# genetronhealth/uvc

Measured on AMD Instinct MI355X. Metric: pileup positions scored/sec at 300x depth, higher is better.
Workload: dtype int32

## Files before the change

### uvc_amd/csrc/uvc_device.h

```cpp
#ifndef UVC_DEVICE_H
#define UVC_DEVICE_H

#include <hip/hip_runtime.h>
#include <stddef.h>
#include <stdint.h>
#include "uvcgpu.h"
#include "uvc_rules.h"
#include "uvc_planes.h"

#define SQR_QUAL_DIV 32
#define MAX_INSERT_SIZE 2000
#define MAX_STR_N_BASES 100
#define UVC_MAXEV 8
#define UVC_DIGEST_MAX_VOTES (1 << 22)

enum { C_MATCH = 0, C_INS = 1, C_DEL = 2, C_REF_SKIP = 3, C_SOFT_CLIP = 4, C_HARD_CLIP = 5, C_PAD = 6, C_EQUAL = 7, C_DIFF = 8 };

struct AlnRec {
    int32_t pos, rend, mpos, isize;
    int32_t flag, mapq, dflag, l_qseq;
    int64_t seq_off;
    int64_t qbase;
    int64_t cigar_off;
    int64_t table_off;
// ... 50 lines not shown
static_assert(sizeof(Item) == 16, "Item");

struct MisItem { int32_t rank, epos, symval; };

struct FragUnit { int32_t beg, end, fi, flags, pos0, rend0, pos1, rend1, qb0, qb1, nogap0, nogap1; };
enum { UVC_FSUM_LCNT = 0 , UVC_FSUM_LTA = 5, UVC_FSUM_LTB, UVC_FSUM_LSING, UVC_FSUM_LMQ, UVC_FSUM_BDP, UVC_FSUM_BTA, UVC_FSUM_BTB, UVC_FSUM_BMQ, UVC_FSUM_N };
struct FragFast {
    int32_t beg, end, fi, flags;
    int32_t pos0, rend0, pos1, rend1;
    int32_t qb0, qb1, nogap0, nogap1;
    int32_t sq, n_cov, n_near, pad_;
    int32_t bpos0, brend0, bqb0, sp0;
    int32_t bpos1, brend1, bqb1, sp1;
};
enum { FF_GENERIC = 1,
       FF_STRAND = 2, FF_SINGLETON = 4, FF_NALN_SHIFT = 3, FF_NALN_MASK = 0xF,
       FF_RUNS_B = 0x100,
       FF_LINK_PER_POS = 0x200,
       FF_NOT_REGISTER = FF_GENERIC | FF_RUNS_B,
       FF_FULL = FF_RUNS_B | FF_LINK_PER_POS,
       FF_NOT_IN_SUMS = FF_GENERIC | FF_FULL };
#define FF_W(field) ((int)(offsetof(FragFast, field) / 4))
static_assert(sizeof(FragFast) == 96, "k_frag fetches a fragment record as six 16-byte words per lane");
static_assert(sizeof(FragUnit) == 48 && offsetof(FragFast, sq) == sizeof(FragUnit), "FragUnit is the first 12 words of FragFast");
static_assert(FF_W(flags) == 3 && offsetof(FragUnit, flags) == offsetof(FragFast, flags) && offsetof(FragUnit, nogap1) == offsetof(FragFast, nogap1), "k_frag_sums reads flags as .w of a record's first int4");

struct AlnGap {
    int32_t epos, sym;
    int32_t len, qpos;
    int32_t weight, aln;
    int32_t mark, pad_;
};
struct GapRow { int32_t x, sym, len, ev; int64_t seq_off; int32_t cnt[8]; };
struct GapWork {
    AlnGap *ev; int32_t n_ev;
    unsigned long long *ckey, *ckey_s, *cval, *cval_s;
    unsigned long long *ikey, *ikey_s, *ival, *ival_s;
    int32_t inc_cap; int32_t *n_inc;
    GapRow *rows; int32_t *n_rows; uint8_t *seq; unsigned long long *seq_len; int64_t seq_cap;
    int32_t *maj;
    void *sort_tmp; size_t sort_tmp_bytes;
};

struct Contrib { uint8_t bsym_p1 , lmask ; uint16_t bval; uint16_t lval[8]; uint16_t pad_[2]; };
static_assert(sizeof(Contrib) == 24, "Contrib rows are zero-filled as bytes and indexed as 24-byte records");

struct HapWork { int32_t *cand, *cand_off, *cand_cap; int32_t *n_cand; unsigned long long *total; int32_t *events; };

struct DevParams { UvcParams P; };

struct RegionDev {
    int32_t beg, end; int64_t npos;
    const uint8_t *refsym;
    int32_t *rtr;
    const int64_t *baq;
    int32_t *prep32; int64_t *prep64; int32_t *thres;
    int32_t *seg32; int64_t *seg64; int32_t *vq; int32_t *bqsum;
    int32_t *frag; int32_t *fam; int32_t *faminfo32; int64_t *faminfo64; int32_t *duplex;
    int32_t *bucket;
    const uint8_t *bases; const uint8_t *quals; const uint32_t *cigars;
    const uint16_t *bq; uint32_t bq_bytes;
    AlnRec *alns; int32_t n_alns;
    int32_t n_fast;
    int32_t p2_off[5];
    FastRec *frec2; int32_t n_fast2; int32_t max_p2_span;
    const int32_t *complex_ids; int32_t n_complex;
    FragRec *frags; int32_t n_frags;
    int32_t *frag_nmut; int32_t *frag_mut;
    const int32_t *sweep_frags; int32_t n_sweep;
    int32_t *overflow_frags; int32_t *n_overflow;
    const int32_t *frag_sorted;
    const int32_t *frag_rank;
    int32_t frag_off[3];
    FragFast *ffast;
    FragUnit *ffast_u;
    int32_t *win; int32_t nwin;
    int32_t *fsum;
    FsRec *fss; int32_t n_fs;
    const int32_t *generic_fs; int32_t n_generic_fs; int64_t n_generic_work;
    const int32_t *generic_sorted; int32_t max_unit_span;
    uint8_t *p5flag;
    uint8_t *dirty; int32_t ndblk;
    uint32_t *occ;
    uint32_t *fam_digest;
    Contrib *table;
    int32_t *ir_list;
    Item *items; int32_t *item_cnt;
    MisItem *mis; int32_t *mis_cnt; int32_t mis_cap;
    unsigned long long *mis_total;
    int32_t max_frag_span;
    int32_t any_amplicon;
    int32_t frag32;
    int32_t max_frag_depth;
    int32_t *err;
    GapWork gap;
};

#define DEV __device__ __forceinline__

DEV int ff_naln(int flags) { return (flags >> FF_NALN_SHIFT) & FF_NALN_MASK; }
template <int WORDS>
DEV void load_words(const void *rec, bool valid, int (&c)[WORDS]) {
    static_assert(WORDS % 4 == 0, "whole 16-byte words");
    if (valid) {
        const int4 *q4 = (const int4 *)rec;
#pragma unroll
        for (int i = 0; i < WORDS / 4; i++) { const int4 t = q4[i]; c[4 * i] = t.x; c[4 * i + 1] = t.y; c[4 * i + 2] = t.z; c[4 * i + 3] = t.w; }
    } else {
#pragma unroll
        for (int i = 0; i < WORDS; i++) c[i] = 0;
    }
}
DEV int64_t lmin(int64_t a, int64_t b) { return a < b ? a : b; }
DEV int64_t lmax(int64_t a, int64_t b) { return a > b ? a : b; }
DEV int64_t nnminus(int64_t a, int64_t b) { return a > b ? a - b : 0; }
DEV int ibetween(int v, int a, int b) { return imin(imax(a, v), b); }
DEV bool is_ins(int s) { return s == UVC_LINK_I3P || s == UVC_LINK_I2 || s == UVC_LINK_I1; }
DEV bool is_del(int s) { return s == UVC_LINK_D3P || s == UVC_LINK_D2 || s == UVC_LINK_D1; }
DEV bool is_subst(int s) { return s <= UVC_BASE_NN; }
DEV bool symbols_mutated(int ref, int alt) {
    if (alt <= UVC_BASE_NN) return ref != alt && ref < UVC_BASE_N && alt < UVC_BASE_N;
    return alt != UVC_LINK_M && alt != UVC_LINK_NN;
}
DEV int cig_op(uint32_t c) { return (int)(c & 0xF); }
DEV int cig_len(uint32_t c) { return (int)(c >> 4); }
DEV bool cig_aligned(int op) { return op == C_MATCH || op == C_EQUAL || op == C_DIFF; }
DEV bool cig_query(int op) { return op == C_MATCH || op == C_EQUAL || op == C_DIFF || op == C_INS || op == C_SOFT_CLIP; }
DEV bool cig_ref(int op) { return op == C_MATCH || op == C_EQUAL || op == C_DIFF || op == C_DEL || op == C_REF_SKIP; }

#define P32(R, f, x) ((R).prep32[(size_t)(f) * (R).npos + (x)])
#define P64(R, f, x) ((R).prep64[(size_t)(f) * (R).npos + (x)])
#define TH(R, f, x) ((R).thres[(size_t)(f) * (R).npos + (x)])
#define S32(R, f, s, x) ((R).seg32[((size_t)(f) * NSYM + (s)) * (R).npos + (x)])
#define S64(R, f, s, x) ((R).seg64[((size_t)(f) * NSYM + (s)) * (R).npos + (x)])
#define VQP(R, f, s, x) ((R).vq[((size_t)(f) * NSYM + (s)) * (R).npos + (x)])
#define BQS(R, s, x) ((R).bqsum[(size_t)(s) * (R).npos + (x)])
#define FRP(R, st, f, s, x) ((R).frag[(((size_t)(st) * UVC_NFRAG + (f)) * NSYM + (s)) * (R).npos + (x)])
#define FAP(R, st, f, s, x) ((R).fam[(((size_t)(st) * UVC_NFAM + (f)) * NSYM + (s)) * (R).npos + (x)])
#define FIP(R, f, s, x) ((R).faminfo32[((size_t)(f) * NSYM + (s)) * (R).npos + (x)])
#define FI64P(R, f, s, x) ((R).faminfo64[((size_t)(f) * NSYM + (s)) * (R).npos + (x)])
#define DUP(R, f, s, x) ((R).duplex[((size_t)(f) * NSYM + (s)) * (R).npos + (x)])
#define BKP(R, st, s, b, x) ((R).bucket[((((size_t)(st) * NSYM + (s)) * NBUCKETS) + (b)) * (R).npos + (x)])
#define RTRP(R, f, x) ((R).rtr[(size_t)(f) * (R).npos + (x)])
#define BAQ1(R, p) ((R).baq[(p) - (R).beg])
#define BAQ2(R, p) ((R).baq[(R).npos + (p) - (R).beg])

DEV int cov_PREP32(const RegionDev &R, int plane, int64_t x) { return P32(R, plane, x); }
DEV int cov_FRAG(const RegionDev &R, int plane, int64_t x) {
    int v = 0;
#pragma unroll
    for (int sd = 0; sd < 2; sd++)
#pragma unroll
        for (int s = UVC_BASE_A; s <= UVC_BASE_NN; s++) v += FRP(R, sd, plane, s, x);
    return v;
}
DEV int cov_FAM(const RegionDev &R, int plane, int64_t x) {
    int v = 0;
#pragma unroll
    for (int sd = 0; sd < 2; sd++)
#pragma unroll
        for (int s = UVC_BASE_A; s <= UVC_BASE_NN; s++) v += FAP(R, sd, plane, s, x);
    return v;
}
DEV int cov_DUPLEX(const RegionDev &R, int plane, int64_t x) {
    int v = 0;
#pragma unroll
// ... 86 lines not shown
```

### uvc_amd/csrc/uvc_host.cpp

```cpp
#include "uvc_launch.h"
#include "uvc_host.h"
#include "uvc_alloc.h"
#include "uvc_prep.h"
#include "uvc_rtr.h"
#include "uvc_hap.h"
#include "uvc_cpus.h"

#include <algorithm>
#include <array>
#include <chrono>
#include <cmath>
#include <cstring>
#include <memory>
#include <numeric>
#include <string>
#include <thread>
#include <vector>

static thread_local std::string g_err;
static int fail(int code, const std::string &msg) { g_err = msg; return code; }
template <class F> static int guarded(const char *what, F &&f) {
    try {
        const int rc = f();
        const hipError_t stale = hipGetLastError();
        if (stale != hipSuccess && getenv("UVCGPU_DEBUG")) fprintf(stderr, "[uvcgpu] %s (rc %d) left HIP error: %s\n", what, rc, hipGetErrorString(stale));
        return rc;
    }
    catch (const std::bad_alloc &) { return fail(UVCGPU_ENOMEM, std::string(what) + ": out of host memory"); }
    catch (const std::exception &e) { return fail(UVCGPU_EDEVICE, std::string(what) + ": " + e.what()); }
}
extern "C" int uvcgpu_set_error(int code, const char *msg) { return fail(code, msg ? msg : ""); }
#define HIP_OK(call) do { hipError_t e_ = (call); if (e_ != hipSuccess) return fail(UVCGPU_EDEVICE, std::string(#call) + ": " + hipGetErrorString(e_)); } while (0)

struct uvcgpu_score_stream;
struct uvcgpu_region;
static void quiesce(const uvcgpu_region *r);
template <class T, bool HOST = false> struct Buf {
    const uvcgpu_region *r; T *p = nullptr; size_t cap = 0;
    explicit Buf(const uvcgpu_region *r_) : r(r_) {}
    Buf(const Buf &) = delete; Buf &operator=(const Buf &) = delete;
    ~Buf() { release(); }
    operator T *() const { return p; }
    static hipError_t raw_alloc(void **q, size_t bytes) { return HOST ? hipHostMalloc(q, bytes, hipHostMallocDefault) : uvc_dev_malloc(q, bytes); }
    static hipError_t raw_free(void *q) { return HOST ? hipHostFree(q) : uvc_dev_free(q); }
    void release() { if (p) { quiesce(r); (void)raw_free(p); } p = nullptr; cap = 0; }
    hipError_t fit(size_t need, size_t slack = 0, size_t keep_max = 0, size_t unit = sizeof(T), size_t *bytes = nullptr) {
        if (cap >= need && !(keep_max && cap > keep_max)) return hipSuccess;
        release();
        const size_t want = (need + slack) * unit;
        if (bytes) *bytes = want;
        const hipError_t e = raw_alloc((void **)&p, want);
        if (e != hipSuccess) { (void)hipGetLastError(); p = nullptr; return e; }
        cap = need + slack;
        return hipSuccess;
    }
};
struct Pool {
    const uvcgpu_region *r; std::vector<void *> blocks; hipError_t last = hipSuccess;
    explicit Pool(const uvcgpu_region *r_) : r(r_) {}
    Pool(const Pool &) = delete; Pool &operator=(const Pool &) = delete;
    ~Pool() { clear(); }
    void *get(size_t bytes) { void *q = nullptr; last = uvc_dev_malloc(&q, bytes); if (last != hipSuccess) return nullptr; blocks.push_back(q); return q; }
    template <class T> bool get(T **out, size_t count) { *out = (T *)get(count * sizeof(T)); return *out != nullptr; }
    void clear() { if (!blocks.empty()) quiesce(r); for (void *q : blocks) (void)uvc_dev_free(q); blocks.clear(); }
};

struct uvcgpu_region {
    UvcParams P;
    int32_t tid, beg, end;
    int64_t npos;
    std::string refstring;
    std::vector<int32_t> h_rtr; bool h_rtr_valid = false;
    UvcRtrWork rw; Buf<char> d_rtrwork{this}; bool thr_ready = false;
    Buf<char, true> h_ref{this};
    hipStream_t stream = nullptr;
    std::array<hipStream_t *, 3> streams() { return { { &stream, &side, &side3 } }; }
    std::array<hipEvent_t *, 6> events() { return { { &e_fork, &e_join, &e_fork2, &e_join3, &e_stat, &e_alleles } }; }
    hipStream_t side = nullptr, side3 = nullptr; hipEvent_t e_fork = nullptr, e_join = nullptr, e_fork2 = nullptr, e_join3 = nullptr, e_stat = nullptr, e_alleles = nullptr;
    Buf<uint8_t> d_refsym{this}; Buf<int32_t> d_rtr{this}, d_rtr0{this}, d_fsum{this}, d_win{this}; Buf<int64_t> d_baq{this};
    Buf<char> d_state{this}; SlabLayout L = {};
    Buf<int32_t> d_err{this};
    int64_t npos_cap = 0;
    bool buckets_clean = false;
    Pool owned{this};
    RegionDev R;
    int32_t *d_dup_units = nullptr; int64_t *d_dup_off = nullptr; int n_dup = 0; int64_t n_dup_work = 0;
    bool has_reads = false, accumulated = false;
    bool reads_given = false;
    Buf<uint8_t> d_dirty{this}; Buf<ZeroPlane> d_zero_planes{this}; int64_t zero_planes_npos = 0;
    int64_t dirty_npos = 0;
    bool state_released = false, state_zeroed = false;
    int64_t last_scored = 0, last_returned = 0;
    size_t zeroed_bytes = 0;
    RawReads W;
    int32_t *d_p2[4] = { nullptr, nullptr, nullptr, nullptr };
    int64_t n_bases = 0;
    UvcProf prof;
    Buf<char> d_score_scratch{this};
    Buf<int32_t> d_score_fields{this}; int64_t *d_score_count = nullptr;
    Buf<uint8_t, true> h_stage{this};
    Buf<int32_t> d_score_kept{this};
    Buf<char> d_report{this}; Buf<char, true> h_report{this};
    uvcgpu_score_stream *ss = nullptr;
    bool gap_ready = false;
    std::vector<UvcGapRow> gap_rows; std::vector<uint8_t> gap_seq;
    std::vector<UvcIndelAllele> gap_alleles; std::vector<int32_t> gap_allele_row;
    Buf<UvcIndelAllele> d_gap_alleles{this}; Buf<int32_t> d_gap_allele_row{this}; Buf<UvcGapRow> d_gap_rows{this}; Buf<uint8_t> d_gap_seq{this};
    bool hap_ready = false;
    std::vector<UvcHapLinkHost> hap[3];
};

static bool stream_is_open(const uvcgpu_region *r);
static void stream_destroy(uvcgpu_region *r);
static void quiesce(const uvcgpu_region *r) { for (hipStream_t s : { r->stream, r->side, r->side3 }) if (s) (void)hipStreamSynchronize(s); }
static int planes_guard(const uvcgpu_region *r, const char *call) {
    if (!r->accumulated) return fail(UVCGPU_ESTATE, std::string(call) + " before accumulate");
    if (r->state_released) return fail(UVCGPU_ESTATE, "the planes were released by the last score (UvcScoreRequest::release_state)");
    return 0;
}

namespace {
template <class T> int dev_alloc(uvcgpu_region *r, size_t count, T **out, bool zero = false) {
    const size_t n = std::max<size_t>(count, 1);
    if (!r->owned.get(out, n)) return fail(UVCGPU_ENOMEM, std::string("hipMalloc: ") + hipGetErrorString(r->owned.last));
    if (zero && hipMemsetAsync(*out, 0, n * sizeof(T), r->stream) != hipSuccess) return fail(UVCGPU_EDEVICE, "hipMemsetAsync");
    return 0;
}
void free_reads(uvcgpu_region *r) { r->owned.clear(); r->has_reads = false; r->reads_given = false; r->accumulated = false; }
}

extern "C" {

const char *uvcgpu_last_error(void) { return g_err.c_str(); }
const char *uvcgpu_version(void) { return "uvcgpu 0.1 (gfx950)"; }

int uvcgpu_init(int device_id) {
    int n = 0;
    if (hipGetDeviceCount(&n) != hipSuccess || n <= 0) return fail(UVCGPU_EDEVICE, "no HIP device: libuvcgpu has no CPU fallback");
    HIP_OK(hipSetDevice(device_id));
    hipDeviceProp_t prop;
    HIP_OK(hipGetDeviceProperties(&prop, device_id));
    if (std::string(prop.gcnArchName).find("gfx950") == std::string::npos) return fail(UVCGPU_EDEVICE, std::string("device is ") + prop.gcnArchName + ", this library is built for gfx950 only");
    return 0;
}

int uvcgpu_device_memory(int64_t *free_bytes, int64_t *total_bytes) {
    size_t fr = 0, tot = 0;
    HIP_OK(hipMemGetInfo(&fr, &tot));
    if (free_bytes) *free_bytes = (int64_t)fr;
    if (total_bytes) *total_bytes = (int64_t)tot;
    return 0;
}

int uvcgpu_device_count(void) { int n = 0; if (hipGetDeviceCount(&n) != hipSuccess) { (void)hipGetLastError(); return 0; } return n; }

void uvcgpu_params_default(UvcParams *p) {
    memset(p, 0, sizeof(*p));
    p->struct_size = (int32_t)sizeof(UvcParams);
#define UVC_PI(name, dflt) p->name = (int32_t)(dflt);
#define UVC_PD(name, dflt) p->name = (double)(dflt);
#include "uvc_params.def"
#undef UVC_PI
#undef UVC_PD
}

static void platform_deltas(UvcParams *p, int32_t platform) {
    auto dec = [](int32_t &a, int32_t b) { a = a - std::min(a, b); };
    if (platform == UVC_PLATFORM_IONTORRENT) {
        p->bq_phred_added_misma += 8;
        dec(p->fam_thres_highBQ_snv, 30); dec(p->fam_thres_highBQ_indel, 30); dec(p->bias_thres_PFBQ1, 30); dec(p->bias_thres_PFBQ2, 30); dec(p->bias_thres_highBQ, 13);
    } else if (platform == UVC_PLATFORM_ILLUMINA) {
        p->syserr_minABQ_pcr_snv += 200; p->syserr_minABQ_pcr_indel += 100; p->syserr_minABQ_cap_snv += 200; p->syserr_minABQ_cap_indel += 100;
    }
}

void uvcgpu_params_apply_platform(UvcParams *p, int32_t platform, int32_t central_readlen, int32_t max_mapq) {
    p->inferred_sequencing_platform = platform;
    if (0 == p->central_readlen) p->central_readlen = central_readlen;
    p->inferred_maxMQ = std::max(p->inferred_maxMQ, max_mapq);
    platform_deltas(p, platform);
}

int uvcgpu_params_apply_platform_ex(UvcParams *p, int32_t sequencing_platform, int32_t inferred, int32_t central_readlen, int32_t max_mapq) {
    if (!p || sequencing_platform < UVC_PLATFORM_AUTO || sequencing_platform > UVC_PLATFORM_OTHER) return fail(UVCGPU_EINVAL, "sequencing platform outside 0..3");
    if (sequencing_platform == UVC_PLATFORM_ILLUMINA || sequencing_platform == UVC_PLATFORM_IONTORRENT) {
        p->inferred_sequencing_platform = sequencing_platform;
        platform_deltas(p, sequencing_platform);
    } else if (sequencing_platform == UVC_PLATFORM_AUTO) {
        uvcgpu_params_apply_platform(p, inferred, central_readlen, max_mapq);
    } else {
        p->inferred_sequencing_platform = inferred;
        if (0 == p->central_readlen) p->central_readlen = central_readlen;
        p->inferred_maxMQ = std::max(p->inferred_maxMQ, max_mapq);
    }
    return 0;
}

static int configure_region(uvcgpu_region *r, int32_t tid, int32_t beg, int32_t end, const char *refseq) {
    r->tid = tid; r->beg = beg; r->end = end + 1; r->npos = (int64_t)end - beg + 1;
    r->refstring.assign(refseq, (size_t)(end - beg));
    r->accumulated = false; r->gap_ready = false; r->hap_ready = false; r->state_released = false;
    r->h_rtr_valid = false;
    r->L = slab_layout(r->npos);
    r->state_zeroed = r->state_zeroed && r->npos <= r->npos_cap && r->L.total <= r->zeroed_bytes;
    r->buckets_clean = r->state_zeroed;
    const int vmax = r->P.indel_vntr_repeatsize_max, smax = r->P.indel_str_repeatsize_max, bqm = r->P.indel_BQ_max;
    const size_t n_rtr = (size_t)UVC_NRTR * r->npos, n = (size_t)r->npos;
    if (r->npos > r->npos_cap) {
        r->npos_cap = 0; r->dirty_npos = 0; r->thr_ready = false;
        size_t scan_tmp = 0;
        const size_t work_bytes = uvc_rtr_work_bytes(r->npos, vmax, smax, bqm, &scan_tmp);
        if (r->d_refsym.fit(n + 1) != hipSuccess || r->d_rtr.fit(n_rtr) != hipSuccess || r->d_rtr0.fit(n_rtr) != hipSuccess || r->d_fsum.fit(2 * UVC_FSUM_N * n) != hipSuccess
            || r->d_win.fit(16 * (size_t)((r->npos + 63) / 64)) != hipSuccess || r->d_baq.fit(2 * n) != hipSuccess || r->d_state.fit(r->L.total) != hipSuccess || r->d_rtrwork.fit(work_bytes) != hipSuccess
            || r->d_dirty.fit((size_t)3 * NSYM * (size_t)((r->npos >> UVC_DIRTY_SHIFT) + 2)) != hipSuccess) return fail(UVCGPU_ENOMEM, "hipMalloc(region planes) failed");
        uvc_rtr_bind(&r->rw, r->d_rtrwork, r->npos, vmax, smax, bqm, scan_tmp);
        r->npos_cap = r->npos;
    }
    if (!r->thr_ready) {
        std::vector<int32_t> thr((size_t)smax * bqm);
        uvc_rtr_thresholds(&r->P, thr.data());
        HIP_OK(hipMemcpy(r->rw.thr, thr.data(), sizeof(int32_t) * thr.size(), hipMemcpyHostToDevice));
        r->thr_ready = true;
    }
    const size_t n_ref = (size_t)(end - beg);
    if (r->h_ref.fit(n_ref) != hipSuccess) return fail(UVCGPU_ENOMEM, "hipHostMalloc(reference staging) failed");
    memcpy(r->h_ref, refseq, n_ref);
    HIP_OK(hipMemcpyAsync(r->rw.refchar, r->h_ref, n_ref, hipMemcpyHostToDevice, r->stream));
    {
        const int e = uvc_launch_region_tracks(&r->rw, &r->P, r->npos, r->d_refsym, r->d_rtr0, r->d_baq, r->stream);
        if (e) return fail(UVCGPU_EDEVICE, std::string("side-array kernels: ") + hipGetErrorString((hipError_t)e));
    }
    RegionDev &R = r->R;
    memset(&R, 0, sizeof(R));
    R.beg = r->beg; R.end = r->end; R.npos = r->npos; R.refsym = r->d_refsym; R.rtr = r->d_rtr; R.baq = r->d_baq; R.fsum = r->d_fsum; R.win = r->d_win; R.nwin = (int32_t)((r->npos + 63) / 64);
    char *b = r->d_state;
#define X(g, m) R.m = (decltype(R.m))(b + r->L.off[UVC_F_##g]);
    UVC_SLAB_MEMBERS(X)
#undef X
    R.bucket = (int32_t *)(b + r->L.bucket_off); R.p5flag = (uint8_t *)(b + r->L.p5flag_off); R.occ = (uint32_t *)(b + r->L.occ_off);
    R.dirty = r->d_dirty; R.ndblk = (int32_t)((r->npos + ((int64_t)1 << UVC_DIRTY_SHIFT) - 1) >> UVC_DIRTY_SHIFT);
    R.err = r->d_err;
    HIP_OK(hipMemsetAsync(R.err, 0, 4, r->stream));
    return 0;
}

static int uvcgpu_region_create_impl(uvcgpu_region_t **out, const UvcParams *params, int32_t tid, int32_t beg, int32_t end, const char *refseq) {
    if (!out || !params || !refseq || end <= beg) return fail(UVCGPU_EINVAL, "bad argument");
    if (const int rc = uvcgpu_params_check(params)) return rc;
    uvcgpu_region *r = new uvcgpu_region();
    memset(&r->prof, 0, sizeof(r->prof));
    memset(&r->R, 0, sizeof(r->R));
    r->P = *params;
    const bool one_stream = (getenv("UVCGPU_ONE_STREAM") != nullptr);
    for (hipStream_t *s : r->streams()) {
        const bool main = (s == &r->stream);
        if (!main && one_stream) break;
        if (hipStreamCreateWithFlags(s, hipStreamNonBlocking) != hipSuccess) { uvcgpu_region_destroy(r); return fail(UVCGPU_EDEVICE, main ? "hipStreamCreate failed (no GPU?)" : "hipStreamCreate / hipEventCreate failed"); }
    }
    if (!one_stream) for (hipEvent_t *e : r->events()) if (hipEventCreateWithFlags(e, hipEventDisableTiming) != hipSuccess) { uvcgpu_region_destroy(r); return fail(UVCGPU_EDEVICE, "hipStreamCreate / hipEventCreate failed"); }
    if (r->d_err.fit(1) != hipSuccess) { uvcgpu_region_destroy(r); return fail(UVCGPU_ENOMEM, "hipMalloc failed"); }
    const int rc = configure_region(r, tid, beg, end, refseq);
    if (rc) { uvcgpu_region_destroy(r); return rc; }
    *out = r;
    return 0;
}

static int uvcgpu_region_reset_impl(uvcgpu_region_t *r, int32_t tid, int32_t beg, int32_t end, const char *refseq) {
    if (!r || !refseq || end <= beg) return fail(UVCGPU_EINVAL, "bad argument");
    if (stream_is_open(r)) return fail(UVCGPU_ESTATE, "reset while a score stream is open");
    HIP_OK(hipStreamSynchronize(r->stream));
    if (r->side) HIP_OK(hipStreamSynchronize(r->side));
    if (r->side3) HIP_OK(hipStreamSynchronize(r->side3));
    free_reads(r);
    return configure_region(r, tid, beg, end, refseq);
}

static void *prep_alloc(void *ctx, size_t bytes, int zero) {
    uvcgpu_region *r = (uvcgpu_region *)ctx;
    char *p = nullptr;
    if (dev_alloc(r, bytes, &p, zero != 0)) return nullptr;
    return p;
}
static int set_reads_on_device(uvcgpu_region_t *r, const UvcReadSoA *d, bool timing, std::chrono::steady_clock::time_point t_prev) {
    auto lap = [&](const char *what) { if (!timing) return; hipStreamSynchronize(r->stream); const auto t = std::chrono::steady_clock::now();
                                       fprintf(stderr, "[uvcgpu set_reads] %-28s %8.2f ms\n", what, std::chrono::duration<double, std::milli>(t - t_prev).count()); t_prev = t; };
    const int64_t n = d->n_reads;
    if (r->npos >= ((int64_t)1 << 29)) return fail(UVCGPU_EUNSUPPORTED, "region longer than 2^29");
    if (d->n_bases >= ((int64_t)1 << 31)) return fail(UVCGPU_EUNSUPPORTED, "more than 2^31 read bases in one region: split the region");
    if (!d->bases && !d->bases4 && d->n_bases > 0) return fail(UVCGPU_EINVAL, "neither bases nor bases4");
    UvcReadSoA dd = *d;
    int32_t *d_bad = nullptr; uint16_t *bq_done = nullptr;
    if (!d->seq_off || !d->cigar_off || !d->bases) {
        int rc0;
        int64_t *so = nullptr, *co = nullptr, *b4o = nullptr; uint8_t *ub = nullptr; char *tmp = nullptr;
        const size_t tb = uvc_prep_compact_tmp_bytes(n);
        if ((rc0 = dev_alloc(r, tb, &tmp)) || (rc0 = dev_alloc(r, 2, &d_bad, true))) return rc0;
        if (!d->seq_off && (rc0 = dev_alloc(r, (size_t)n, &so))) return rc0;
        if (!d->cigar_off && (rc0 = dev_alloc(r, (size_t)n, &co))) return rc0;
        if (!d->bases && ((rc0 = dev_alloc(r, (size_t)n, &b4o)) || (rc0 = dev_alloc(r, (size_t)std::max<int64_t>(d->n_bases, 1), &ub)) || (rc0 = dev_alloc(r, (size_t)std::max<int64_t>(d->n_bases, 1), &bq_done)))) return rc0;
        const int e = uvc_prep_compact(d->l_qseq, d->n_cigar, n, d->n_bases, d->bases ? nullptr : d->bases4, d->n_bases4_bytes, d->quals, so, d->seq_off, co, b4o, ub, bq_done, d_bad, tmp, tb, r->stream);
        if (e) return fail(UVCGPU_EDEVICE, std::string("offset scans: ") + hipGetErrorString((hipError_t)e));
        if (so) dd.seq_off = so;
        if (co) dd.cigar_off = co;
        if (ub) dd.bases = ub;
        d = &dd;
    }
    UvcPrepIn in; memset(&in, 0, sizeof(in));
    in.n_reads = n; in.n_bases = d->n_bases; in.n_cigar_ops = d->n_cigar_ops; in.n_fams = d->n_fams;
    in.pos = d->pos; in.mpos = d->mpos; in.isize = d->isize; in.nm = d->nm; in.l_qseq = d->l_qseq; in.n_cigar = d->n_cigar; in.frag_id = d->frag_id; in.fam_id = d->fam_id;
    in.flag = d->flag; in.mapq = d->mapq; in.fam_strand = d->fam_strand; in.fam_dflag = d->fam_dflag; in.seq_off = d->seq_off; in.cigar_off = d->cigar_off; in.cigars = d->cigars;
    uint16_t *bq_packed = bq_done;
    if (!bq_packed) {
        int rc1;
        if ((rc1 = dev_alloc(r, (size_t)std::max<int64_t>(d->n_bases, 1), &bq_packed))) return rc1;
        if (!d_bad && (rc1 = dev_alloc(r, 2, &d_bad, true))) return rc1;
        uvc_launch_pack_bq(d->bases, d->quals, bq_packed, d->n_bases, d_bad, r->stream);
    }
    in.quals = d->quals; in.zero_qual = d_bad + 1;
    UvcPrepOut o; char msg[256];
    int rc = uvc_prep_reads(&in, &r->P, r->beg, r->end, r->npos, prep_alloc, r, r->stream, &o, msg, (int)sizeof(msg));
    if (rc) return fail(rc, msg);
    lap("nesting + CIGAR facts (device)");
    RegionDev &R = r->R;
// ... 107 lines not shown
    const int64_t n = in->n_reads;
    if (n == 0) { r->reads_given = true; return 0; }
    if (n > INT32_MAX / 2) return fail(UVCGPU_EUNSUPPORTED, "more than 2^30 reads in one region");
    if (in->n_bases < 0 || in->n_cigar_ops < 0) return fail(UVCGPU_EINVAL, "bad reads");
    UvcReadSoA d = *in;
    int rc;
    hipStream_t small_stream = (r->side ? r->side : r->stream);
    auto up_on = [&](hipStream_t st, const void *src, size_t bytes, void **out) -> int {
        char *q = nullptr;
        int rc2 = dev_alloc(r, bytes, &q);
        if (rc2) return rc2;
        if (bytes && hipMemcpyAsync(q, src, bytes, hipMemcpyHostToDevice, st) != hipSuccess) return fail(UVCGPU_EDEVICE, "hipMemcpyAsync(H2D)");
        *out = q;
        return 0;
    };
#define UP(field, T, count) { void *q; if ((rc = up_on(small_stream, in->field, sizeof(T) * (size_t)(count), &q))) return rc; d.field = (const T *)q; }
#define UPBIG(field, T, count) { void *q; if ((rc = up_on(r->stream, in->field, sizeof(T) * (size_t)(count), &q))) return rc; d.field = (const T *)q; }
    if (in->bases) UPBIG(bases, uint8_t, in->n_bases)
    else if (in->bases4) { if (in->n_bases4_bytes < 0) return fail(UVCGPU_EINVAL, "bad reads"); UPBIG(bases4, uint8_t, in->n_bases4_bytes) }
    UPBIG(quals, uint8_t, in->n_bases)
    UP(pos, int32_t, n) UP(mpos, int32_t, n) UP(isize, int32_t, n) UP(flag, uint16_t, n) UP(mapq, uint8_t, n) UP(nm, int32_t, n) UP(l_qseq, int32_t, n)
    UP(n_cigar, int32_t, n) UP(frag_id, int32_t, n) UP(fam_id, int32_t, n) UP(fam_strand, uint8_t, n)
    if (in->seq_off) UP(seq_off, int64_t, n)
    if (in->cigar_off) UP(cigar_off, int64_t, n)
    UP(cigars, uint32_t, in->n_cigar_ops) UP(fam_dflag, uint8_t, in->n_fams)
    if (small_stream != r->stream) {
        if (hipEventRecord(r->e_fork2, small_stream) != hipSuccess || hipStreamWaitEvent(r->stream, r->e_fork2, 0) != hipSuccess) return fail(UVCGPU_EDEVICE, "hipEventRecord / hipStreamWaitEvent");
    }
#undef UPBIG
#undef UP
    if (timing) { hipStreamSynchronize(r->stream); const auto t = std::chrono::steady_clock::now(); fprintf(stderr, "[uvcgpu set_reads] %-28s %8.2f ms\n", "H2D of the columns", std::chrono::duration<double, std::milli>(t - t_prev).count()); t_prev = t; }
    return set_reads_on_device(r, &d, timing, t_prev);
}

static int uvcgpu_region_set_reads_device_impl(uvcgpu_region_t *r, const UvcReadSoA *in) {
    if (!r || !in) return fail(UVCGPU_EINVAL, "bad reads");
    if (stream_is_open(r)) return fail(UVCGPU_ESTATE, "set_reads while a score stream is open");
    if (in->struct_size != (int32_t)sizeof(UvcReadSoA)) return fail(UVCGPU_EINVAL, "UvcReadSoA::struct_size mismatch (set it to sizeof(UvcReadSoA))");
    if (in->n_reads < 0 || in->n_fams < 0 || in->n_bases < 0 || in->n_cigar_ops < 0) return fail(UVCGPU_EINVAL, "bad reads");
    const bool timing = (getenv("UVCGPU_TIMING") != nullptr);
    free_reads(r);
    if (in->n_reads == 0) { r->reads_given = true; return 0; }
    if (in->n_reads > INT32_MAX / 2) return fail(UVCGPU_EUNSUPPORTED, "more than 2^30 reads in one region");
    return set_reads_on_device(r, in, timing, std::chrono::steady_clock::now());
}

static int uvcgpu_region_correct_bq_impl(uvcgpu_region_t *r) {
    if (!r) return fail(UVCGPU_EINVAL, "null region");
    if (!r->has_reads) return fail(UVCGPU_ENOREADS, "no reads");
    uvc_launch_correct_bq(&r->R, r->P.assay_sequencing_BQ_max, r->P.assay_sequencing_BQ_inc, r->stream);
    uvc_launch_pack_bq(r->R.bases, r->R.quals, (uint16_t *)r->R.bq, r->n_bases, nullptr, r->stream);
    const int zthr = uvc_prep_zero_value_qual(&r->P);
    int32_t *d_n_joined = nullptr;
    if (zthr > 0 || (zthr == 0 && (r->P.assay_sequencing_BQ_inc < 0 || r->P.assay_sequencing_BQ_max <= 0))) {
        int rc = dev_alloc(r, 1, &d_n_joined, true);
        if (rc) return rc;
        uvc_prep_requalify(r->R.quals, r->W.seq_off, r->W.l_qseq, &r->P, r->R.n_frags, (FragRec *)r->R.frags, (int32_t *)r->R.sweep_frags, r->R.n_sweep, d_n_joined, r->stream);
    }
    HIP_OK(hipMemsetAsync(r->R.mis_total, 0, sizeof(unsigned long long), r->stream));
    uvc_launch_prelude(&r->R, &r->W, &r->P, r->stream);
    uvc_launch_build_p2list(&r->R, r->W.fast_rank, r->d_p2[0], r->d_p2[1], r->d_p2[2], r->d_p2[3], r->stream);
    HIP_OK(hipGetLastError());
    if (d_n_joined) {
        HIP_OK(hipStreamSynchronize(r->stream));
        int32_t n_joined = 0;
        HIP_OK(hipMemcpy(&n_joined, d_n_joined, sizeof(n_joined), hipMemcpyDeviceToHost));
        if (getenv("UVCGPU_TIMING")) fprintf(stderr, "[uvcgpu correct_bq] fragments looked at again: %d joined the sweep list (%d)\n", n_joined, r->R.n_sweep + n_joined);
        r->R.n_sweep += n_joined;
    } else HIP_OK(hipStreamSynchronize(r->stream));
    r->accumulated = false;
    return 0;
}

int uvcgpu_region_read_quals(uvcgpu_region_t *r, uint8_t *dst, int64_t n) {
    if (!r || !dst) return fail(UVCGPU_EINVAL, "null argument");
    if (!r->has_reads) return fail(UVCGPU_ENOREADS, "no reads");
    if (n != r->n_bases) return fail(UVCGPU_EINVAL, "n must equal UvcReadSoA::n_bases");
    HIP_OK(hipStreamSynchronize(r->stream));
    if (n > 0) HIP_OK(hipMemcpy(dst, r->R.quals, (size_t)n, hipMemcpyDeviceToHost));
    return 0;
}

static int zero_state(uvcgpu_region *r, hipStream_t s) {
    const size_t n_dirty = (size_t)3 * NSYM * (size_t)r->R.ndblk;
    const bool selective = (r->dirty_npos == r->npos && !getenv("UVCGPU_FILL_ALL"));
    r->dirty_npos = 0;
    if (selective) {
        if (r->zero_planes_npos != r->npos) {
            ZeroPlane v[UVC_N_ZERO_PLANES];
            zero_plane_rows(r->L, r->npos, v);
            r->zero_planes_npos = 0;
            const hipError_t e = r->d_zero_planes.fit(UVC_N_ZERO_PLANES);
            if (e != hipSuccess) return fail(UVCGPU_EDEVICE, std::string("hipMalloc(zero-fill table): ") + hipGetErrorString(e));
            HIP_OK(hipMemcpy(r->d_zero_planes, v, sizeof(v), hipMemcpyHostToDevice));
            r->zero_planes_npos = r->npos;
        }
        uvc_launch_zero_state(r->d_state, r->d_zero_planes, UVC_N_ZERO_PLANES, r->d_dirty, r->R.ndblk, r->npos, s);
        if (hipGetLastError() != hipSuccess) return fail(UVCGPU_EDEVICE, "zero fill of the planes failed");
        if (!r->buckets_clean) HIP_OK(hipMemsetAsync(r->d_state + r->L.bucket_off, 0, r->L.total - r->L.bucket_off, s));
    } else {
        HIP_OK(hipMemsetAsync(r->d_state, 0, r->buckets_clean ? r->L.bucket_off : r->L.total, s));
    }
    HIP_OK(hipMemsetAsync(r->d_dirty, 0, n_dirty, s));
    return 0;
}

static int uvcgpu_region_accumulate_impl(uvcgpu_region_t *r) {
    if (!r) return fail(UVCGPU_EINVAL, "null region");
    if (stream_is_open(r)) return fail(UVCGPU_ESTATE, "accumulate while a score stream is open");
    if (!r->has_reads) return fail(UVCGPU_ENOREADS, "no reads");
    if (r->state_zeroed) { r->dirty_npos = 0; HIP_OK(hipStreamWaitEvent(r->stream, r->e_join, 0)); }
    else { const int rcz = zero_state(r, r->stream); if (rcz) return rcz; }
    r->state_zeroed = false; r->state_released = false;
    r->buckets_clean = false;
    HIP_OK(hipMemcpyAsync(r->d_rtr, r->d_rtr0, (size_t)4 * UVC_NRTR * r->npos, hipMemcpyDeviceToDevice, r->stream));
    HIP_OK(hipMemsetAsync(r->R.frag_nmut, 0, sizeof(int32_t) * (size_t)r->R.n_frags, r->stream));
    HIP_OK(hipMemsetAsync(r->R.n_overflow, 0, sizeof(int32_t), r->stream));
    HIP_OK(hipMemsetAsync(r->R.mis_cnt, 0, sizeof(int32_t), r->stream));
    if (r->R.n_complex) {
    }
    const int half = (int)std::round((10.0 / std::log(10.0)) * std::log(r->P.indel_del_to_ins_err_ratio)) / 2;
    const UvcAccStreams st = { r->stream, r->side, r->side3, r->e_fork, r->e_join, r->e_fork2, r->e_join3, r->e_stat, r->e_alleles };
    uvc_launch_accumulate(&r->R, &r->P, half, r->d_dup_units, r->n_dup, r->d_dup_off, r->n_dup_work, &st, &r->prof);
    HIP_OK(hipGetLastError());
    r->buckets_clean = (r->P.inferred_is_vcf_generated != 0);
    r->dirty_npos = r->npos;
    r->accumulated = true; r->gap_ready = false; r->hap_ready = false;
    return 0;
}

int uvcgpu_region_check_presence(uvcgpu_region_t *r, int64_t *n_violations) {
    if (!r || !n_violations) return fail(UVCGPU_EINVAL, "bad argument");
    if (planes_guard(r, "check_presence")) return fail(UVCGPU_ESTATE, "check_presence needs the planes of an accumulate");
    Pool tmp(r);
    unsigned long long *d = nullptr, h = 0;
    if (!tmp.get(&d, 1)) return fail(UVCGPU_EDEVICE, std::string("hipMalloc(violation count): ") + hipGetErrorString(tmp.last));
    int rc = 0;
    if (hipMemsetAsync(d, 0, 8, r->stream) != hipSuccess) rc = fail(UVCGPU_EDEVICE, "hipMemsetAsync");
    if (!rc) { uvc_launch_check_presence(&r->R, d, r->stream); uvc_launch_check_dirty(&r->R, d, r->stream); if (hipMemcpyAsync(&h, d, 8, hipMemcpyDeviceToHost, r->stream) != hipSuccess || hipStreamSynchronize(r->stream) != hipSuccess) rc = fail(UVCGPU_EDEVICE, "check_presence"); }
    *n_violations = (int64_t)h;
    return rc;
}

int uvcgpu_region_set_profiling(uvcgpu_region_t *r, int on) { if (!r) return fail(UVCGPU_EINVAL, "null region"); r->prof.on = on ? 1 : 0; return 0; }
int uvcgpu_region_kernel_times(uvcgpu_region_t *r, char *names, int names_bytes, float *ms, int capacity) {
    if (!r || !names || !ms) return fail(UVCGPU_EINVAL, "bad argument");
    HIP_OK(hipStreamSynchronize(r->stream));
    std::string all;
    int n = 0;
    for (int i = 0; i < r->prof.n && n < capacity; i++, n++) {
        float t = 0;
        HIP_OK(hipEventElapsedTime(&t, r->prof.ev[i][0], r->prof.ev[i][1]));
        ms[n] = t; all += r->prof.name[i]; all += ";";
    }
    if ((int)all.size() + 1 > names_bytes) return fail(UVCGPU_EINVAL, "names buffer too small");
    memcpy(names, all.c_str(), all.size() + 1);
    return n;
}

int uvcgpu_region_last_score_counts(const uvcgpu_region_t *r, int64_t *scored, int64_t *returned) {
    if (!r) return fail(UVCGPU_EINVAL, "null region");
    if (scored) *scored = r->last_scored;
    if (returned) *returned = r->last_returned;
    return 0;
}

int uvcgpu_region_sync(uvcgpu_region_t *r) {
    if (!r) return fail(UVCGPU_EINVAL, "null region");
    HIP_OK(hipStreamSynchronize(r->stream));
    int32_t e = 0;
    HIP_OK(hipMemcpy(&e, r->R.err, 4, hipMemcpyDeviceToHost));
    if (e) return fail(e, "a kernel flagged an unsupported read shape (a CIGAR op the reference itself throws on, process_cigar main_conversion.hpp:902-916)");
    return 0;
}

int64_t uvcgpu_region_field_bytes(const uvcgpu_region_t *r, int32_t g) {
    if (!r || g < 0 || g >= UVC_NUM_FIELD_GROUPS) return -1;
    if (uvc_group_in_slab(g) && !r->accumulated) return -1;
    return (int64_t)uvc_group_bytes(g, r->npos);
}

static int uvcgpu_region_fetch_impl(uvcgpu_region_t *r, int32_t g, void *dst, int64_t dst_bytes) {
    if (!r || !dst || g < 0 || g >= UVC_NUM_FIELD_GROUPS) return fail(UVCGPU_EINVAL, "bad argument");
    if (uvc_group_in_slab(g)) { const int rcg = planes_guard(r, "fetch"); if (rcg) return rcg; }
    if ((int64_t)uvc_group_bytes(g, r->npos) != dst_bytes) return fail(UVCGPU_EINVAL, "bad destination size");
    int rc = uvcgpu_region_sync(r);
    if (rc) return rc;
    const void *src = (g == UVC_F_RTR) ? (const void *)(r->accumulated ? r->d_rtr : r->d_rtr0)  : (g == UVC_F_BAQ) ? (const void *)r->d_baq : (const void *)(r->d_state + r->L.off[g]);
    HIP_OK(hipMemcpy(dst, src, (size_t)dst_bytes, hipMemcpyDeviceToHost));
    return 0;
}

int32_t uvcgpu_region_column_base(int32_t g) { return (g < 0 || g >= UVC_NUM_FIELD_GROUPS) ? -1 : uvc_group_first_column(g); }
int32_t uvcgpu_region_n_columns(void) { return UVC_N_COLUMNS; }
static int uvcgpu_region_fetch_columns_impl(uvcgpu_region_t *r, const int32_t *refpos, int64_t n, int64_t *dst) {
    if (!r || n < 0 || (n > 0 && (!refpos || !dst))) return fail(UVCGPU_EINVAL, "bad argument");
    { const int rcg = planes_guard(r, "fetch"); if (rcg) return rcg; }
    if (n == 0) return 0;
    int rc = uvcgpu_region_sync(r);
    if (rc) return rc;
    const int32_t ncol = UVC_N_COLUMNS;
    const char *base[UVC_NUM_FIELD_GROUPS]; int32_t first[UVC_NUM_FIELD_GROUPS + 1], elem[UVC_NUM_FIELD_GROUPS];
    for (int g = 0; g <= UVC_NUM_FIELD_GROUPS; g++) first[g] = uvc_columns_before(g);
    for (int g = 0; g < UVC_NUM_FIELD_GROUPS; g++) { elem[g] = uvc_group_elem(g); base[g] = r->d_state + r->L.off[g]; }
    std::vector<int32_t> xs((size_t)n);
    for (int64_t i = 0; i < n; i++) xs[(size_t)i] = refpos[i] - r->beg;
    Pool tmp(r);
    int32_t *d_xs = nullptr; long long *d_out = nullptr;
    if (!tmp.get(&d_xs, (size_t)n)) return fail(UVCGPU_ENOMEM, "hipMalloc(column positions) failed");
    if (!tmp.get(&d_out, (size_t)n * ncol)) return fail(UVCGPU_ENOMEM, "hipMalloc(columns) failed");
    hipError_t e = hipMemcpyAsync(d_xs, xs.data(), sizeof(int32_t) * (size_t)n, hipMemcpyHostToDevice, r->stream);
    if (e == hipSuccess) { uvc_launch_gather_columns(base, first, elem, r->npos, d_xs, n, d_out, r->stream); e = hipGetLastError(); }
    if (e == hipSuccess) e = hipMemcpyAsync(dst, d_out, sizeof(long long) * (size_t)n * ncol, hipMemcpyDeviceToHost, r->stream);
    if (e == hipSuccess) e = hipStreamSynchronize(r->stream);
    if (e != hipSuccess) return fail(UVCGPU_EDEVICE, hipGetErrorString(e));
    return 0;
}
int uvcgpu_region_block_stats_(uvcgpu_region_t *r, int32_t refpos_beg, int32_t refpos_end, int32_t *dst) {
    if (!r || !dst || refpos_end < refpos_beg) return fail(UVCGPU_EINVAL, "bad argument");
    { const int rcg = planes_guard(r, "fetch"); if (rcg) return rcg; }
    const int64_t n = (int64_t)refpos_end - refpos_beg;
    if (n == 0) return 0;
    int rc = uvcgpu_region_sync(r);
    if (rc) return rc;
    Pool tmp(r);
    int32_t *d = nullptr;
    if (!tmp.get(&d, 10 * (size_t)n)) return fail(UVCGPU_ENOMEM, "hipMalloc(block stats) failed");
    uvc_launch_block_stats(&r->R, &r->P, (int64_t)refpos_beg - r->beg, n, d, r->stream);
    hipError_t e = hipGetLastError();
    if (e == hipSuccess) e = hipMemcpyAsync(dst, d, sizeof(int32_t) * 10 * (size_t)n, hipMemcpyDeviceToHost, r->stream);
    if (e == hipSuccess) e = hipStreamSynchronize(r->stream);
    if (e != hipSuccess) return fail(UVCGPU_EDEVICE, hipGetErrorString(e));
    return 0;
}
int uvcgpu_region_block_stats_windows_(uvcgpu_region_t *r, const int32_t *win, int64_t n_win, int32_t *dst) {
    if (!r || !win || !dst || n_win < 0 || n_win > INT32_MAX) return fail(UVCGPU_EINVAL, "bad argument");
    { const int rcg = planes_guard(r, "fetch"); if (rcg) return rcg; }
    std::vector<long long> tab((size_t)(2 * n_win));
    int64_t n = 0;
    for (int64_t k = 0; k < n_win; k++) {
        if (win[2 * k + 1] <= win[2 * k]) return fail(UVCGPU_EINVAL, "block statistics: empty window");
        tab[(size_t)(2 * k)] = (long long)win[2 * k] - r->beg; tab[(size_t)(2 * k + 1)] = n; n += (int64_t)win[2 * k + 1] - win[2 * k];
    }
    if (n == 0) return 0;
    int rc = uvcgpu_region_sync(r);
    if (rc) return rc;
    Pool tmp(r);
    long long *d_tab = nullptr; int32_t *d = nullptr;
    if (!tmp.get(&d_tab, tab.size()) || !tmp.get(&d, 10 * (size_t)n)) return fail(UVCGPU_ENOMEM, "hipMalloc(block stats) failed");
    hipError_t e = hipMemcpyAsync(d_tab, tab.data(), sizeof(long long) * tab.size(), hipMemcpyHostToDevice, r->stream);
    if (e == hipSuccess) { uvc_launch_block_stats_windows(&r->R, &r->P, d_tab, (int)n_win, n, d, r->stream); e = hipGetLastError(); }
    if (e == hipSuccess) e = hipMemcpyAsync(dst, d, sizeof(int32_t) * 10 * (size_t)n, hipMemcpyDeviceToHost, r->stream);
    const hipError_t e2 = hipStreamSynchronize(r->stream);
    if (e != hipSuccess || e2 != hipSuccess) return fail(UVCGPU_EDEVICE, hipGetErrorString(e != hipSuccess ? e : e2));
    return 0;
}
int uvcgpu_pin_host_buffer(void *p, int64_t bytes) {
    if (!p || bytes <= 0) return fail(UVCGPU_EINVAL, "bad argument");
    hipError_t e = hipHostRegister(p, (size_t)bytes, hipHostRegisterDefault);
    if (e != hipSuccess) { (void)hipGetLastError(); return fail(UVCGPU_EDEVICE, std::string("hipHostRegister: ") + hipGetErrorString(e)); }
    return 0;
}
int uvcgpu_host_alloc(void **p, int64_t bytes) {
    if (!p || bytes <= 0) return fail(UVCGPU_EINVAL, "bad argument");
    *p = nullptr;
    hipError_t e = Buf<char, true>::raw_alloc(p, (size_t)bytes);
    if (e != hipSuccess) { (void)hipGetLastError(); *p = nullptr; return fail(UVCGPU_ENOMEM, std::string("hipHostMalloc: ") + hipGetErrorString(e)); }
    return 0;
}
int uvcgpu_host_free(void *p) {
    if (!p) return 0;
    hipError_t e = Buf<char, true>::raw_free(p);
    if (e != hipSuccess) { (void)hipGetLastError(); if (getenv("UVCGPU_DEBUG")) fprintf(stderr, "[uvcgpu] hipHostFree: %s\n", hipGetErrorString(e)); return fail(UVCGPU_EDEVICE, std::string("hipHostFree: ") + hipGetErrorString(e)); }
    return 0;
}
int uvcgpu_unpin_host_buffer(void *p) {
    if (!p) return 0;
    hipError_t e = hipHostUnregister(p);
    if (e != hipSuccess) { (void)hipGetLastError(); return fail(UVCGPU_EDEVICE, std::string("hipHostUnregister: ") + hipGetErrorString(e)); }
    return 0;
}

const char *uvcgpu_region_refseq(const uvcgpu_region_t *r, int32_t *beg, int32_t *end) { if (beg) *beg = r->beg; if (end) *end = r->end - 1; return r->refstring.c_str(); }
const int32_t *uvcgpu_region_repeat_tracks(const uvcgpu_region_t *cr, int64_t *npos) {
    uvcgpu_region_t *r = const_cast<uvcgpu_region_t *>(cr);
    if (npos) *npos = r->npos;
    if (!r->h_rtr_valid) {
        r->h_rtr.resize((size_t)3 * r->npos);
        if (hipMemcpyAsync(r->h_rtr.data(), r->d_rtr0, sizeof(int32_t) * r->h_rtr.size(), hipMemcpyDeviceToHost, r->stream) != hipSuccess || hipStreamSynchronize(r->stream) != hipSuccess) { (void)hipGetLastError(); return nullptr; }
        r->h_rtr_valid = true;
    }
    return r->h_rtr.data();
}
const UvcParams *uvcgpu_region_params(const uvcgpu_region_t *r) { return &r->P; }
// ... 138 lines not shown
        events.resize(at + (size_t)c.total);
        HIP_OK(hipMemcpyAsync(events.data() + at, H.events, 4 * (size_t)c.total, hipMemcpyDeviceToHost, r->stream));
        HIP_OK(hipStreamSynchronize(r->stream));
        lap(units ? "events of units + D2H" : "events of fragments + D2H", (long long)c.total);
    }
    { const int rc = uvcgpu_region_sync(r); if (rc) return rc; }
    uvc_hap_build(events.data(), (int64_t)events.size(), r->beg, r->npos, r->P.phasing_haplotype_max_count, r->P.phasing_haplotype_min_ad, r->P.phasing_haplotype_max_detail_cnt, r->hap);
    lap("maps + links (host)", (long long)(r->hap[0].size() + r->hap[1].size() + r->hap[2].size()));
    r->hap_ready = true;
    return 0;
}
const std::vector<UvcHapLinkHost> *uvcgpu_region_hap_(uvcgpu_region_t *r) { return hap_tables(r) ? nullptr : r->hap; }

static int uvcgpu_region_hap_links_impl(uvcgpu_region_t *r, UvcHapLink *links, int64_t link_capacity, int64_t *n_links, int32_t *muts, int64_t mut_capacity, int64_t *n_mut_ints) {
    if (!r) return fail(UVCGPU_EINVAL, "null region");
    int rc = hap_tables(r);
    if (rc) return rc;
    int64_t nl = 0, nm = 0;
    for (int w = 0; w < 3; w++) for (const UvcHapLinkHost &h : r->hap[w]) { nl++; nm += 2 * (int64_t)h.form.size(); }
    if (n_links) *n_links = nl;
    if (n_mut_ints) *n_mut_ints = nm;
    if (nl > link_capacity || nm > mut_capacity || (nl && !links) || (nm && !muts)) return fail(UVCGPU_ENOMEM, "haplotype link capacity too small");
    int64_t li = 0, mi = 0;
    for (int w = 0; w < 3; w++) for (const UvcHapLinkHost &h : r->hap[w]) {
        UvcHapLink &o = links[li++];
        o.which = w; o.n_muts = (int32_t)h.form.size(); o.mut_off = mi; o.fr_cnt[0] = h.fr[0]; o.fr_cnt[1] = h.fr[1]; o.other_cnt[0] = h.other[0]; o.other_cnt[1] = h.other[1];
        for (const auto &ps : h.form) { muts[mi++] = ps.first; muts[mi++] = ps.second; }
    }
    return 0;
}

int64_t uvcgpu_region_score_size(const uvcgpu_region_t *r, const UvcScoreRequest *req) {
    if (!r) return -1;
    const int64_t np = (req && req->pos_beg >= 0) ? (req->pos_end - req->pos_beg) : r->npos;
    return NSYM * (np + 1) + (req ? req->n_indel_alleles + req->n_tumor_keys + 16 * std::max<int64_t>(req->n_force_sites, 0) : 0) + (int64_t)r->gap_alleles.size();
}
int64_t uvcgpu_region_score_ranges_size(const uvcgpu_region_t *r, const UvcScoreRequest *req, const UvcScoreRange *ranges, int64_t n_ranges) {
    if (!r || !ranges || n_ranges < 0) return -1;
    int64_t np = 0;
    for (int64_t k = 0; k < n_ranges; k++) np += std::max<int64_t>((int64_t)ranges[k].pos_end - ranges[k].pos_beg, 0);
    return NSYM * (np + 1) + (req ? req->n_indel_alleles + req->n_tumor_keys + 16 * std::max<int64_t>(req->n_force_sites, 0) : 0) + (int64_t)r->gap_alleles.size();
}

static int stage_upload(uvcgpu_region_t *r, void *dst, const void *src, size_t bytes, size_t &at, size_t total) {
    if (r->h_stage.fit(total, total / 2 + 4096) != hipSuccess) return fail(UVCGPU_ENOMEM, "hipHostMalloc(staging)");
    memcpy(r->h_stage + at, src, bytes);
    if (hipMemcpyAsync(dst, r->h_stage + at, bytes, hipMemcpyHostToDevice, r->stream) != hipSuccess) return fail(UVCGPU_EDEVICE, "hipMemcpyAsync(staging)");
    at += (bytes + 63) & ~(size_t)63;
    return 0;
}

struct ScorePrep {
    UvcScoreRequest rq; std::vector<UvcScoreRangeDev> rtab; int64_t npos_scored = 0;
    std::unique_ptr<Pool> tmp;
    UvcScoreIn in = {};
};
static int score_prepare(uvcgpu_region_t *r, const UvcScoreRequest *req, const UvcScoreRange *ranges, int64_t n_ranges, ScorePrep &p) {
    { const int rcg = planes_guard(r, "score"); if (rcg) return rcg; }
    if (stream_is_open(r)) return fail(UVCGPU_ESTATE, "a score stream is open on this handle (uvcgpu_score_stream_end closes it)");
    p.tmp.reset(new Pool(r));
    UvcScoreRequest &rq = p.rq; memset(&rq, 0, sizeof(rq)); rq.pos_beg = -1;
    if (req) rq = *req;
    std::vector<UvcScoreRangeDev> &rtab = p.rtab;
    int64_t &npos_scored = p.npos_scored;
    if (ranges) {
        if (n_ranges < 1 || n_ranges > INT32_MAX) return fail(UVCGPU_EINVAL, "score_ranges: n_ranges must be at least 1");
        if (rq.pos_beg != -1 || rq.base_at_pos_beg != 0 || rq.region_beg != 0) return fail(UVCGPU_EINVAL, "score_ranges: the request's pos_beg must be -1, its base_at_pos_beg and region_beg 0 (the ranges carry them)");
        rtab.resize((size_t)n_ranges);
        for (int64_t k = 0; k < n_ranges; k++) {
            const UvcScoreRange &q = ranges[k];
            if (q.pos_beg < r->beg + (q.base_at_pos_beg ? 1 : 0) || q.pos_end > r->end - 1 || q.pos_end < q.pos_beg)
                return fail(UVCGPU_EINVAL, "score_ranges: range " + std::to_string(k) + " [" + std::to_string(q.pos_beg) + ", " + std::to_string(q.pos_end) + ") is outside the region");
            if (k > 0 && q.pos_beg < ranges[k - 1].pos_end)
                return fail(UVCGPU_EINVAL, "score_ranges: range " + std::to_string(k) + " begins at " + std::to_string(q.pos_beg) + ", in front of the end " + std::to_string(ranges[k - 1].pos_end) + " of range " + std::to_string(k - 1) + " (ranges must be sorted and disjoint)");
            rtab[(size_t)k] = UvcScoreRangeDev{ q.pos_beg, q.pos_end, (int32_t)npos_scored, q.base_at_pos_beg ? 1 : 0 };
            npos_scored += (int64_t)q.pos_end - q.pos_beg;
        }
        rq.pos_beg = ranges[0].pos_beg; rq.pos_end = ranges[n_ranges - 1].pos_end;
    } else {
        if (rq.pos_beg < 0) { rq.pos_beg = r->beg + 1; rq.pos_end = r->end - 1; }
        if (rq.pos_beg < r->beg + (rq.base_at_pos_beg ? 1 : 0) || rq.pos_end > r->end - 1 || rq.pos_end < rq.pos_beg) return fail(UVCGPU_EINVAL, "score range outside the region");
        npos_scored = (int64_t)rq.pos_end - rq.pos_beg;
    }
    { int rc0 = gap_tables(r); if (rc0) return rc0; }
    UvcIndelAllele *d_al = nullptr; int32_t *d_al_row = nullptr; UvcTumorKey *d_tk = nullptr; int32_t *d_fs = nullptr; UvcScoreRangeDev *d_rg = nullptr;
    auto no_room = [&] { return fail(UVCGPU_EDEVICE, std::string("hipMalloc(score request): ") + hipGetErrorString(p.tmp->last)); };
    std::vector<UvcIndelAllele> merged; std::vector<int32_t> merged_row;
    const UvcIndelAllele *use_al = r->d_gap_alleles; const int32_t *use_row = r->d_gap_allele_row; int64_t n_al = (int64_t)r->gap_alleles.size();
    size_t stage_at = 0;
    const size_t stage_total = (sizeof(UvcIndelAllele) + sizeof(int32_t)) * (size_t)(r->gap_alleles.size() + (size_t)std::max<int64_t>(rq.n_indel_alleles, 0)) + sizeof(UvcTumorKey) * (size_t)std::max<int64_t>(rq.n_tumor_keys, 0)
                              + sizeof(int32_t) * (size_t)std::max<int64_t>(rq.n_force_sites, 0) + sizeof(UvcScoreRangeDev) * rtab.size() + 320;
    if (rq.n_indel_alleles > 0) {
        auto less = [](const UvcIndelAllele &a, const UvcIndelAllele &b) { return a.refpos < b.refpos || (a.refpos == b.refpos && a.symbol < b.symbol); };
        for (int64_t q = 1; q < rq.n_indel_alleles; q++) if (less(rq.indel_alleles[q], rq.indel_alleles[q - 1])) return fail(UVCGPU_EINVAL, "indel_alleles must be sorted by (refpos, symbol)");
        size_t i = 0; int64_t j = 0;
        while (i < r->gap_alleles.size() || j < rq.n_indel_alleles) {
            const bool take_own = (j >= rq.n_indel_alleles) || (i < r->gap_alleles.size() && less(r->gap_alleles[i], rq.indel_alleles[j]));
            if (take_own) { merged.push_back(r->gap_alleles[i]); merged_row.push_back(r->gap_allele_row[i]); i++; continue; }
            const UvcIndelAllele key = rq.indel_alleles[j];
            while (i < r->gap_alleles.size() && !less(key, r->gap_alleles[i])) i++;
            while (j < rq.n_indel_alleles && !less(key, rq.indel_alleles[j])) { merged.push_back(rq.indel_alleles[j]); merged_row.push_back(-1); j++; }
        }
        n_al = (int64_t)merged.size();
        if (!p.tmp->get(&d_al, (size_t)n_al) || !p.tmp->get(&d_al_row, (size_t)n_al)) return no_room();
        { int rc1 = stage_upload(r, d_al, merged.data(), sizeof(UvcIndelAllele) * (size_t)n_al, stage_at, stage_total); if (rc1) return rc1; }
        { int rc1 = stage_upload(r, d_al_row, merged_row.data(), sizeof(int32_t) * (size_t)n_al, stage_at, stage_total); if (rc1) return rc1; }
        use_al = d_al; use_row = d_al_row;
    }
    if (r->P.tumor_vcf_is_provided && rq.n_tumor_keys > 0) {
        for (int64_t q = 1; q < rq.n_tumor_keys; q++) {
            const UvcTumorKey &a = rq.tumor_keys[q - 1], &b = rq.tumor_keys[q];
            if (a.refpos > b.refpos || (a.refpos == b.refpos && a.symbol > b.symbol)) return fail(UVCGPU_EINVAL, "tumor_keys must be sorted by (refpos, symbol)");
        }
        if (!p.tmp->get(&d_tk, (size_t)rq.n_tumor_keys)) return no_room();
        { int rc1 = stage_upload(r, d_tk, rq.tumor_keys, sizeof(UvcTumorKey) * (size_t)rq.n_tumor_keys, stage_at, stage_total); if (rc1) return rc1; }
    }
    if (rq.n_force_sites < 0 || (rq.n_force_sites > 0 && !rq.force_sites)) return fail(UVCGPU_EINVAL, "force_sites: bad count or NULL array");
    if (rq.n_force_sites > 0) {
        if (r->P.tumor_vcf_is_provided) return fail(UVCGPU_EINVAL, "force_sites cannot go with tumor_vcf_is_provided (the normal sample's gate is the rescue set)");
        for (int64_t q = 1; q < rq.n_force_sites; q++) if (rq.force_sites[q] < rq.force_sites[q - 1]) return fail(UVCGPU_EINVAL, "force_sites must be sorted ascending");
        if (!p.tmp->get(&d_fs, (size_t)rq.n_force_sites)) return no_room();
        { int rc1 = stage_upload(r, d_fs, rq.force_sites, sizeof(int32_t) * (size_t)rq.n_force_sites, stage_at, stage_total); if (rc1) return rc1; }
    }
    if (!rtab.empty()) {
        if (!p.tmp->get(&d_rg, rtab.size())) return no_room();
        { int rc1 = stage_upload(r, d_rg, rtab.data(), sizeof(UvcScoreRangeDev) * rtab.size(), stage_at, stage_total); if (rc1) return rc1; }
    }
    p.in = UvcScoreIn{ &r->R, &r->P, &rq, use_al, use_row, n_al, r->d_gap_rows, r->d_gap_seq, d_tk, nullptr, d_fs, d_rg, (int64_t)rtab.size(), npos_scored };
    return 0;
}
extern "C++" template <class B>
static int fit_buffer(B &b, size_t need, size_t slack, size_t keep_max, size_t unit, int err, const std::string &what) {
    size_t bytes = 0;
    return b.fit(need, slack, keep_max, unit, &bytes) == hipSuccess ? 0 : fail(err, what + " (" + std::to_string(bytes) + " bytes)");
}
static const size_t SCORE_RECORD_BYTES = sizeof(int32_t) * UVC_NUM_SCORE_FIELDS;
static bool queue_release_state(uvcgpu_region *r, bool stream_already_ordered) {
    if (!stream_already_ordered && (hipEventRecord(r->e_fork, r->stream) != hipSuccess || hipStreamWaitEvent(r->side, r->e_fork, 0) != hipSuccess)) return false;
    if (zero_state(r, r->side) != 0 || hipEventRecord(r->e_join, r->side) != hipSuccess) return false;
    r->state_released = true; r->state_zeroed = true; r->zeroed_bytes = r->L.total; r->dirty_npos = r->npos;
    return true;
}
static int uvcgpu_region_score_impl(uvcgpu_region_t *r, const UvcScoreRequest *req, const UvcScoreRange *ranges, int64_t n_ranges, UvcScoreOut *out) {
    if (!r || !out || !out->fields) return fail(UVCGPU_EINVAL, "bad argument");
    ScorePrep prep;
    { const int rc0 = score_prepare(r, req, ranges, n_ranges, prep); if (rc0) return rc0; }
    const UvcScoreRequest &rq = prep.rq; const int64_t npos_scored = prep.npos_scored;
    const bool kept_only = (rq.kept_only != 0);
    int64_t cap = std::max<int64_t>(out->capacity, 1);
    if (kept_only) cap = std::max<int64_t>(std::max<int64_t>(cap, (int64_t)r->d_score_fields.cap), npos_scored / 8 + 4096);
    int rc = 0;
    int64_t cnt[2] = { 0, 0 };
    for (int attempt = 0; attempt < 2 && !rc; attempt++) {
        if ((rc = fit_buffer(r->d_score_fields, (size_t)cap, 0, 0, SCORE_RECORD_BYTES, UVCGPU_EDEVICE, "score: hipMalloc of the records"))) break;
        if (kept_only && (rc = fit_buffer(r->d_score_kept, r->d_score_fields.cap, 0, r->d_score_fields.cap, SCORE_RECORD_BYTES, UVCGPU_EDEVICE, "score: hipMalloc of the kept records"))) break;
        const size_t need = uvc_score_scratch_bytes(npos_scored, (int64_t)r->d_score_fields.cap);
        if ((rc = fit_buffer(r->d_score_scratch, need, need / 8, 0, 1, UVCGPU_EDEVICE, "score: hipMalloc of the scratch"))) break;
        r->d_score_count = (int64_t *)r->d_score_scratch.p;
        HIP_OK(hipMemsetAsync(r->d_score_scratch, 0, uvc_score_scratch_zero_bytes(npos_scored, (int64_t)r->d_score_fields.cap), r->stream));
        const int pi = uvc_prof_begin(&r->prof, "k_score_all", r->stream);
        prep.in.scratch = r->d_score_scratch;
        rc = uvc_launch_score(&prep.in, r->d_score_fields, (int64_t)r->d_score_fields.cap, kept_only ? r->d_score_kept : nullptr, r->stream);
        if (rc) rc = fail(rc, "score: the force-output mask could not be cleared");
        uvc_prof_end(&r->prof, pi, r->stream);
        if (!rc && hipGetLastError() != hipSuccess) rc = fail(UVCGPU_EDEVICE, "score kernel launch failed");
        if (!rc) rc = uvcgpu_region_sync(r);
// ... 629 lines not shown
```

### uvc_amd/csrc/uvc_kernels_acc.hip

```cpp
#include "uvc_launch.h"
#include "uvc_collectives.h"
#include <stdlib.h>
#include <string.h>

DEV int wave_uniform(int v) { return __builtin_amdgcn_readfirstlane(v); }

DEV int xcd_block() {
    const int nb = gridDim.x, b = blockIdx.x, q = nb >> 3, r = nb & 7, k = b & 7, i = b >> 3;
    return k * q + (k < r ? k : r) + i;
}

DEV int bcast(int v, int j) { return __builtin_amdgcn_readlane(v, j); }
#ifdef UVC_FRAG_COARSE
#define COARSE_T(v) unsigned long long v; asm volatile("s_memtime %0\n\ts_waitcnt lgkmcnt(0)" : "=s"(v) :: "memory");
#else
#define COARSE_T(v)
#endif
DEV __amdgpu_buffer_rsrc_t bq_rsrc(const RegionDev &R) { return __builtin_amdgcn_make_buffer_rsrc((void *)R.bq, 0, (int)R.bq_bytes, 0x00020000); }
DEV int bq_load(__amdgpu_buffer_rsrc_t rs, int idx) { return (int)__builtin_amdgcn_raw_buffer_load_b16(rs, idx << 1, 0, 0); }
#define WIN_LISTS 8
DEV int win_lo(const RegionDev &R, int list, int w) { return R.win[((size_t)list * 2) * R.nwin + w]; }
DEV int win_hi(const RegionDev &R, int list, int w) { return R.win[((size_t)list * 2 + 1) * R.nwin + w]; }
__global__ void __launch_bounds__(256) k_win_index(RegionDev R, int list_beg, int list_end) {
    const int64_t t = (int64_t)blockIdx.x * blockDim.x + threadIdx.x;
    const int64_t per_list = 2 * (int64_t)R.nwin;
    if (t >= per_list * (list_end - list_beg)) return;
    const int list = list_beg + (int)(t / per_list), which = (int)((t % per_list) / R.nwin), w = (int)(t % R.nwin);
    const char *base; int stride, lo, hi, span;
    if (list <= 4) { base = (const char *)&R.frec2[0].pos; stride = sizeof(FastRec); lo = R.p2_off[list - 1]; hi = R.p2_off[list]; span = R.max_p2_span; }
    else if (list <= 6) { base = (const char *)&R.ffast[0].beg; stride = sizeof(FragFast); lo = R.frag_off[list - 5]; hi = R.frag_off[list - 4]; span = R.max_frag_span; }
    else { base = nullptr; stride = 0; lo = 0; hi = R.n_generic_fs; span = R.max_unit_span; }
    const int w0 = R.beg + 64 * w, key = (which == 0 ? w0 - span + 1 : w0 + 64);
    if (list <= 6) { while (lo < hi) { const int mid = (lo + hi) >> 1; if (*(const int32_t *)(base + (size_t)mid * stride) < key) lo = mid + 1; else hi = mid; } }
    else { while (lo < hi) { const int mid = (lo + hi) >> 1; if (R.fss[R.generic_sorted[mid]].beg < key) lo = mid + 1; else hi = mid; } }
    R.win[((size_t)list * 2 + which) * R.nwin + w] = lo;
}

struct SegAcc {
    int s[UVC_NSEG32];
    long long l[UVC_NSEG64];
    int lp[UVC_NSEG64];
    int a1BQf, a1BQr, a2BQf, a2BQr, bq;
    DEV void zero() { for (int i = 0; i < UVC_NSEG32; i++) s[i] = 0; for (int i = 0; i < UVC_NSEG64; i++) { l[i] = 0; lp[i] = 0; } a1BQf = a1BQr = a2BQf = a2BQr = bq = 0; }
    DEV void fold() { for (int i = 0; i < UVC_NSEG64; i++) { l[i] += (long long)lp[i]; lp[i] = 0; } }
};

DEV void seg_flush(const RegionDev &R, const SegAcc &A, int sym, int64_t x) {
    mark_sym(R, sym, x);
#pragma unroll
    for (int f = 0; f < UVC_NSEG32; f++) if (A.s[f]) atomicAdd(&S32(R, f, sym, x), A.s[f]);
#pragma unroll
    for (int f = 0; f < UVC_NSEG64; f++) if (A.l[f]) add64(&S64(R, f, sym, x), A.l[f]);
    if (A.a1BQf) atomicAdd(&VQP(R, UVC_VQ_a1BQf, sym, x), A.a1BQf);
    if (A.a1BQr) atomicAdd(&VQP(R, UVC_VQ_a1BQr, sym, x), A.a1BQr);
    if (A.a2BQf) atomicAdd(&VQP(R, UVC_VQ_a2BQf, sym, x), A.a2BQf);
    if (A.a2BQr) atomicAdd(&VQP(R, UVC_VQ_a2BQr, sym, x), A.a2BQr);
    if (A.bq) atomicAdd(&BQS(R, sym, x), A.bq);
}

DEV void seg_store(const RegionDev &R, const SegAcc &A, int sym, int64_t x) {
#pragma unroll
    for (int f = 0; f < UVC_NSEG32; f++) if (A.s[f]) S32(R, f, sym, x) = A.s[f];
#pragma unroll
    for (int f = 0; f < UVC_NSEG64; f++) if (A.l[f]) S64(R, f, sym, x) = A.l[f];
    if (A.a1BQf) VQP(R, UVC_VQ_a1BQf, sym, x) = A.a1BQf;
    if (A.a1BQr) VQP(R, UVC_VQ_a1BQr, sym, x) = A.a1BQr;
    if (A.a2BQf) VQP(R, UVC_VQ_a2BQf, sym, x) = A.a2BQf;
    if (A.a2BQr) VQP(R, UVC_VQ_a2BQr, sym, x) = A.a2BQr;
    if (A.bq) BQS(R, sym, x) = A.bq;
}

struct PosThres { int t[UVC_NTHRES]; };

struct SegRead {
    int pos, rend, flag, mapq, isize, frag_pos_L, frag_pos_R, xm1500, clip_cnt, dflag;
    long long baq_pos, baq_last, baq2_last;
};

DEV SegRead make_segread(const RegionDev &R, const AlnRec &a) {
    SegRead r;
    r.pos = a.pos; r.rend = a.rend; r.flag = a.flag; r.mapq = a.mapq; r.isize = a.isize;
    r.frag_pos_L = imin(a.pos, a.mpos); r.frag_pos_R = r.frag_pos_L + abs(a.isize);
    r.xm1500 = a.xm1500; r.clip_cnt = a.clip_cnt; r.dflag = a.dflag;
    r.baq_pos = a.baq_pos; r.baq_last = a.baq_last; r.baq2_last = a.baq2_last;
    return r;
}

DEV void bidir(int &LP1, int &LP2, int &RP1, int &RP2, long long &LPL, long long &RPL, int L1, int L2, int R1, int R2, long long nl, long long nr, bool tier2, int n_indel) {
    if (nl + n_indel >= L1) LP1 += 1;
    if ((nl + n_indel >= L2) && tier2) LP2 += 1;
    if (nr >= R1) RP1 += 1;
    if ((nr >= R2) && tier2) RP2 += 1;
    LPL += nl; RPL += nr;
}

template <bool isGap>
DEV void segbias(SegAcc &A, const UvcParams &P, const SegRead &r, const PosThres &T, int rpos, long long baq_p, long long baq2_p,
                 int bq, int bm1500, int cigar_op, int indel_len, int dist_to_interfering_indel) {
    const bool amplicon = is_assay_amplicon(r.dflag, P);
    const bool normal_filter_primers = normal_filters_primers(P);
    const bool is_assay_UMI = (r.dflag & UVC_DFLAG_UMI);
    const int seg_l_baq1 = (int)(baq_p - r.baq_pos + 1);
    const int _seg_r_baq = (int)(r.baq_last - baq_p + 1);
    const int seg_r_baq1 = (isGap ? (int)lmin((long long)_seg_r_baq, r.baq2_last - baq2_p + 7) : _seg_r_baq);
    const int seg_l_nbases = rpos - r.pos + 1;
    const int seg_r_nbases = r.rend - rpos;
    const bool is_high_readlen = (P.central_readlen >= P.microadjust_median_readlen_thres);
    const int seg_l_baq = (is_high_readlen ? seg_l_baq1 : imax(seg_l_baq1, seg_l_nbases * P.microadjust_BAQ_per_base_x1024 / 1024));
    const int seg_r_baq = (is_high_readlen ? seg_r_baq1 : imax(seg_r_baq1, seg_r_nbases * P.microadjust_BAQ_per_base_x1024 / 1024));
    const int frag_l_nbases2 = ((r.isize != 0) ? imin(rpos - r.frag_pos_L + 1, MAX_INSERT_SIZE) : MAX_INSERT_SIZE);
    const int frag_r_nbases2 = ((r.isize != 0) ? imin(r.frag_pos_R - rpos, MAX_INSERT_SIZE) : MAX_INSERT_SIZE);
    const bool is_normal = ((r.isize != 0) || (0 == (r.flag & 0x1)));
    const bool isrc = (r.flag & 0x10) != 0;
    const bool strand = ((r.flag & 0x81) == 0x81) ? ((r.flag & 0x20) != 0) : ((r.flag & 0x10) != 0);

    if (isrc) { A.a1BQr += bq; A.a2BQr += bq * bq / SQR_QUAL_DIV; } else { A.a1BQf += bq; A.a2BQf += bq * bq / SQR_QUAL_DIV; }
    A.s[UVC_S_aMQs] += r.mapq;
    A.s[UVC_S_aDPff] += (!strand && !isrc); A.s[UVC_S_aDPfr] += (!strand && isrc);
    A.s[UVC_S_aDPrf] += (strand && !isrc);  A.s[UVC_S_aDPrr] += (strand && isrc);
    if (imin(dist_to_interfering_indel, imin(seg_l_nbases, seg_r_nbases)) >= P.bias_thres_interfering_indel) A.s[UVC_S_aP3] += 1;
    if (0 == r.clip_cnt) A.s[UVC_S_aNC] += 1;
    if (isrc) A.l[UVC_S64_aLIT] += ((r.isize != 0) ? frag_l_nbases2 : 0);
    else      A.l[UVC_S64_aRIT] += ((r.isize != 0) ? frag_r_nbases2 : 0);

    const int _LPxT = T.t[UVC_T_aLPxT], RPxT = T.t[UVC_T_aRPxT];
    const int LPxT = (isGap ? _LPxT : imin(_LPxT, RPxT));
    const bool is_far_from_edge = (seg_l_nbases + ((C_INS == cigar_op) ? (int)nnminus(indel_len, P.microadjust_nobias_pos_indel_maxlen) : 0) >= LPxT) && (seg_r_nbases >= RPxT);
    const int thres_highBAQ = P.bias_thres_highBAQ + (isGap ? 0 : 3);
    const bool is_unaffected_by_edge = (seg_l_baq >= thres_highBAQ && seg_r_baq >= thres_highBAQ);
    const int min_dist2iend = ((r.flag & 0x1) ? imin(frag_l_nbases2, frag_r_nbases2) : (isrc ? seg_r_nbases : seg_l_nbases));
    if (is_far_from_edge && is_unaffected_by_edge && (min_dist2iend > P.primerlen2 || !amplicon)) A.s[UVC_S_aP1] += 1;
    if (is_assay_UMI || !amplicon) A.s[UVC_S_aP2] += 1;

    int ampfact2 = 100;
    if (bq < P.bias_thres_PFBQ1) ampfact2 = 100 * (bq * bq) / (P.bias_thres_PFBQ1 * P.bias_thres_PFBQ1);
    A.s[UVC_S_aPF1] += (isGap ? imin(100, ampfact2) : (100 * ampfact2 / 100));
    ampfact2 = 100;
    if (bq < P.bias_thres_PFBQ2) ampfact2 = 100 * (bq * bq) / (P.bias_thres_PFBQ2 * P.bias_thres_PFBQ2);
    A.s[UVC_S_aPF2] += (isGap ? imin(100, ampfact2) : (100 * ampfact2 / 100));
    if (!isGap) {
        A.s[UVC_S_a2XM2] += (r.xm1500 > 20 ? (100 * (20 * 20) / (r.xm1500 * r.xm1500)) : 100);
        A.s[UVC_S_a2BM2] += (bm1500 > 20 ? (100 * (20 * 20) / (bm1500 * bm1500)) : 100);
    }
    if (((!isGap) && bq >= P.bias_thres_highBQ) || (isGap && dist_to_interfering_indel >= P.bias_thres_interfering_indel)) {
        const bool tier2 = (isGap || bq >= P.bias_thres_highBQ);
        if (is_far_from_edge) {
            long long LPL = 0, RPL = 0;
            bidir(A.s[UVC_S_aLP1], A.s[UVC_S_aLP2], A.s[UVC_S_aRP1], A.s[UVC_S_aRP2], LPL, RPL,
                  T.t[UVC_T_aLP1t], T.t[UVC_T_aLP2t], T.t[UVC_T_aRP1t], T.t[UVC_T_aRP2t], seg_l_nbases, seg_r_nbases, tier2, indel_len);
            A.s[UVC_S_aLPL] += (int)LPL; A.s[UVC_S_aRPL] += (int)RPL;
        }
        if (is_unaffected_by_edge) {
// ... 785 lines not shown
    const double ins_r = ceil(sqrt((double)(P64(R, UVC_P_a_near_ins_r_pow2len, x) / imax(ins_dp, 1))));
    const double del_r = ceil(sqrt((double)(P64(R, UVC_P_a_near_del_r_pow2len, x) / imax(del_dp, 1))));
    const int dnv_border = ((UVC_PLATFORM_IONTORRENT == P.inferred_sequencing_platform && (P32(R, UVC_P_a_dnv_dp, x) * 2 > P32(R, UVC_P_a_snv_dp, x))) ? 10 : 0);
    TH(R, UVC_T_aLPxT, x) = (int)(fmax(ins_l, fmax(del_l, (double)dnv_border)) + P.bias_thres_aLPxT_add);
    TH(R, UVC_T_aRPxT, x) = (int)(fmax(ins_r, fmax(del_r, (double)dnv_border)) + P.bias_thres_aLPxT_add);
    int ip = RTRP(R, UVC_RTR_indelphred, x);
    if (ins_dp * P.indel_del_to_ins_err_ratio < del_dp) ip += half_ratio_phred;
    if (del_dp * P.indel_del_to_ins_err_ratio < ins_dp) ip -= half_ratio_phred;
    const int pc_inc1 = (int)(3 * 100 * imax(1, ins_dp + del_dp) / (imax(1, P32(R, UVC_P_a_near_ins_inv100len, x) + P32(R, UVC_P_a_near_del_inv100len, x)))) - 3;
    ip += ibetween(pc_inc1, 0, 6);
    RTRP(R, UVC_RTR_indelphred, x) = imax(ip, 0);
    const int p1T = (is_normal ? P.bias_thres_aLRI1NT_perc : P.bias_thres_aLRI1T_perc), p1t = (is_normal ? P.bias_thres_aLRI1Nt_perc : P.bias_thres_aLRI1t_perc);
    const long long LI = P64(R, UVC_P_a_LI, x), RI = P64(R, UVC_P_a_RI, x);
    TH(R, UVC_T_aLI1T, x) = (int)(LI * p1T / (segLIDP * 100) + P.bias_thres_aLRI1T_add);
    TH(R, UVC_T_aLI2T, x) = (int)(LI * P.bias_thres_aLRI2T_perc / (segLIDP * 100) + P.bias_thres_aLRI2T_add);
    TH(R, UVC_T_aLI1t, x) = (int)(LI * p1t / (segLIDP * 100));
    TH(R, UVC_T_aLI2t, x) = (int)(LI * P.bias_thres_aLRI2t_perc / (segLIDP * 100));
    TH(R, UVC_T_aRI1T, x) = (int)(RI * p1T / (segRIDP * 100) + P.bias_thres_aLRI1T_add);
    TH(R, UVC_T_aRI2T, x) = (int)(RI * P.bias_thres_aLRI2T_perc / (segRIDP * 100) + P.bias_thres_aLRI2T_add);
    TH(R, UVC_T_aRI1t, x) = (int)(RI * p1t / (segRIDP * 100));
    TH(R, UVC_T_aRI2t, x) = (int)(RI * P.bias_thres_aLRI2t_perc / (segRIDP * 100));
    const int pP1 = (is_normal ? P.bias_thres_aLRP1Nt_avgmul_perc : P.bias_thres_aLRP1t_avgmul_perc), pP2 = P.bias_thres_aLRP2t_avgmul_perc;
    const int pB1 = (is_normal ? P.bias_thres_aLRB1Nt_avgmul_perc : P.bias_thres_aLRB1t_avgmul_perc), pB2 = P.bias_thres_aLRB2t_avgmul_perc;
    const int hb = P32(R, UVC_P_a_highBQ_dp, x);
    const long long den = imax(1, hb * 100);
    const long long lds = P32(R, UVC_P_a_l_dist_sum, x), rds = P32(R, UVC_P_a_r_dist_sum, x);
    TH(R, UVC_T_aLP1t, x) = (int)nnminus(lds * pP1 / den, P.bias_thres_aLRP1t_minus);
    TH(R, UVC_T_aLP2t, x) = (int)nnminus(lds * pP2 / den, P.bias_thres_aLRP2t_minus);
    TH(R, UVC_T_aRP1t, x) = (int)nnminus(rds * pP1 / den, P.bias_thres_aLRP1t_minus);
    TH(R, UVC_T_aRP2t, x) = (int)nnminus(rds * pP2 / den, P.bias_thres_aLRP2t_minus);
    const long long pdel = P64(R, UVC_P_a_delBAQ_sum, x) / imax(1, hb);
    const long long lb = P64(R, UVC_P_a_l_BAQ_sum, x), rb = P64(R, UVC_P_a_r_BAQ_sum, x);
    TH(R, UVC_T_aLB1t, x) = (int)nnminus(lb * pB1 / den, P.bias_thres_aLRB1t_minus + pdel);
    TH(R, UVC_T_aLB2t, x) = (int)nnminus(lb * pB2 / den, P.bias_thres_aLRB2t_minus);
    TH(R, UVC_T_aRB1t, x) = (int)nnminus(rb * pB1 / den, P.bias_thres_aLRB1t_minus + pdel);
    TH(R, UVC_T_aRB2t, x) = (int)nnminus(rb * pB2 / den, P.bias_thres_aLRB2t_minus);
}

DEV int simple_link_value(const RegionDev &R, const UvcParams &P, const AlnRec &a, int p, const uint8_t *quals_qbase, bool proton) {
    const int64_t x = p - R.beg;
    const int noindel = imin(RTRP(R, UVC_RTR_indelphred, x - 1), RTRP(R, UVC_RTR_indelphred, x));
    const int qfromBQ2 = (proton ? imin((int)quals_qbase[p - 1], (int)quals_qbase[p]) : 80);
    return (int)nnminus(imin(qfromBQ2, noindel), a.nogap_penal) + 1;
}
DEV int simple_base_value(const UvcParams &P, const AlnRec &a, int p, const uint8_t *quals_qbase, bool proton) {
    const int q = quals_qbase[p];
    if (proton) {
        const int i2 = p - a.pos, len = a.rend - a.pos;
        if ((0 == i2) || (len - 1 == i2)) {
            const bool next_gap = (len - 1 == i2), prev_gap = (0 == i2);
            const bool isrc2 = (0 != i2);
            const int qpos = (int)(p - a.pos) + a.lclip_q;
            int prev_base_phred = 1;
            if (isrc2 && (qpos + 1 < a.l_qseq)) prev_base_phred = quals_qbase[p + 1];
            if ((!isrc2) && (qpos > 0)) prev_base_phred = quals_qbase[p - 1];
            int adj = 100;
            if (next_gap) adj = imin(adj, (a.rclip_oplen > 0 ? a.rclip_oplen : 100));
            if (prev_gap) adj = imin(adj, (a.lclip_oplen > 0 ? a.lclip_oplen : 100));
            if (adj < 3) return imin(q, prev_base_phred) + imin(P.bq_phred_added_misma, P.bq_phred_added_indel);
            return imin(q, prev_base_phred) + P.bq_phred_added_misma;
        }
    }
    return base_value(q, P);
}

DEV void mis_apply(const RegionDev &R, const UvcParams &P, const MisItem &it) {
    const int64_t x = it.epos - R.beg;
    const int sym = it.symval & 0xFF, inc = it.symval >> 8;
    if ((unsigned)it.rank >= (unsigned)R.n_alns || x < 0 || x >= R.npos || sym > UVC_BASE_NN) { atomicExch(R.err, UVCGPU_EDEVICE); return; }
    const AlnRec &a = R.alns[it.rank];
    const SegRead sr = make_segread(R, a);
    PosThres T;
    load_thres(R, T, x);
    SegAcc A; A.zero();
    A.bq = inc;
    segbias<false>(A, P, sr, T, it.epos, R.baq[x], R.baq[R.npos + x], inc, a.bm1500[sym], C_MATCH, 0, 10000);
    seg_flush(R, A, sym, x);
}

#ifndef P2_AHEAD
#define P2_AHEAD 2
#endif
#define MISQ_CAP 192
#define P2_RED_SLOTS (UVC_NSEG32 + 2 * UVC_NSEG64 + 5)
DEV unsigned long long *red64(int (*red)[64], int f) { return (unsigned long long *)&red[UVC_NSEG32 + 2 * f][0]; }
template <bool DO_L, bool DO_B, bool PLAIN, bool SPLIT = false>
DEV void p2_fast_body(const RegionDev &R, const UvcParams &P, int *amp1, int *amp2, MisItem (*misq)[DO_B ? MISQ_CAP : 1], int (*red)[64] = nullptr) {
    COARSE_T(ct0)
    {
        for (int v = (int)threadIdx.x - AMP_LO; v < 256; v += 256) {
            const int d1 = P.bias_thres_PFBQ1 * P.bias_thres_PFBQ1, d2 = P.bias_thres_PFBQ2 * P.bias_thres_PFBQ2;
            amp1[v + AMP_LO] = ((v < P.bias_thres_PFBQ1 && d1) ? 100 * (v * v) / d1 : 100);
            amp2[v + AMP_LO] = ((v < P.bias_thres_PFBQ2 && d2) ? 100 * (v * v) / d2 : 100);
        }
    }
    __syncthreads();
    const int lane = threadIdx.x & 63;
    const int wave = SPLIT ? wave_uniform((int)xcd_block()) : wave_uniform((int)((xcd_block() * blockDim.x + threadIdx.x) >> 6));
    const int64_t x0 = (int64_t)wave * 64;
    if (x0 >= R.npos) return;
    if (SPLIT) { for (int i2 = threadIdx.x; i2 < P2_RED_SLOTS * 64; i2 += 256) (&red[0][0])[i2] = 0; __syncthreads(); }
    const int w0 = R.beg + (int)x0;
    const int p = w0 + lane;
    const int64_t x = x0 + lane;
    const bool valid = x < R.npos;
    const bool proton = (PLAIN ? false : (UVC_PLATFORM_IONTORRENT == P.inferred_sequencing_platform));
    const bool normal_filter_primers = normal_filters_primers(P);
    const int my_ref = valid ? R.refsym[x] : 0;
    PosThres T;
    long long baq_p = 0, baq2_p = 0;
    if (valid) { load_thres(R, T, x); baq_p = R.baq[x]; baq2_p = R.baq[R.npos + x]; }
    else { for (int f = 0; f < UVC_NTHRES; f++) T.t[f] = 0; }
    SegAcc Aref, Alink;
    Aref.zero(); Alink.zero();
    int noindel80 = 80;
    if (DO_L && valid && x > 0) noindel80 = imin(80, imin(RTRP(R, UVC_RTR_indelphred, x - 1), RTRP(R, UVC_RTR_indelphred, x)));
    MisItem *myq = misq[DO_B ? (threadIdx.x >> 6) : 0];
    int nq = 0;
    auto flush_queue = [&]() {
        int base = 0;
        if (lane == 0) base = atomicAdd(R.mis_cnt, nq);
        base = wave_uniform(base);
        for (int i = lane; i < nq; i += 64) {
            if (base + i < R.mis_cap) R.mis[base + i] = myq[i];
            else atomicExch(R.err, UVCGPU_EDEVICE);
        }
        nq = 0;
    };
    const __amdgpu_buffer_rsrc_t rs = bq_rsrc(R);
    auto run_list = [&](auto IS, auto ST, int cls) {
    constexpr bool ISRC = decltype(IS)::value, STRAND = decltype(ST)::value;
    const int lo = wave_uniform(win_lo(R, 1 + cls, (int)(x0 >> 6))), hi = wave_uniform(win_hi(R, 1 + cls, (int)(x0 >> 6)));
    for (int k0 = lo + (SPLIT ? 64 * (int)(threadIdx.x >> 6) : 0); k0 < hi; k0 += (SPLIT ? 256 : 64)) {
        int c[16];
        if (DO_B) load_words(R.frec2 + (k0 + lane), k0 + lane < hi, c);
        const int n = imin(64, hi - k0);
        auto fetch = [&](int j) { return bq_load(rs, bcast(c[FR_W(qb_lo)], j) + p); };
        auto one = [&](auto K, int bqn) {
            const int sym = bq_sym(bqn), q = bq_qual(bqn);
            const int apos = K(FR_W(pos)), rend = K(FR_W(rend));
            if (rend <= w0) return;
            const int fmd = K(FR_W(fmd));
            const int ext = K(FR_W(ext));
            SegRead sr;
            sr.pos = apos - (ext & 0xFFFF); sr.rend = rend + (int)((unsigned)ext >> 16); sr.flag = fmd & 0xFFFF; sr.mapq = (fmd >> 16) & 0xFF; sr.dflag = (fmd >> 24) & 0xFF;
            sr.isize = K(FR_W(isize));
            const int mpos = K(FR_W(mpos));
            sr.frag_pos_L = imin(sr.pos, mpos); sr.frag_pos_R = sr.frag_pos_L + abs(sr.isize);
            sr.xm1500 = K(FR_W(xm1500));
            const int bm4c = K(FR_W(bm4c));
            sr.clip_cnt = (bm4c >> 16) & 0xF;
            const int nogap = (int)(short)(bm4c & 0xFFFF);
            sr.baq_pos = K(FR_W(baq_pos)); sr.baq_last = K(FR_W(baq_last)); sr.baq2_last = K(FR_W(baq2_last));
            const bool amplicon = (PLAIN ? false : is_assay_amplicon(sr.dflag, P));
            bool gate = true;
            if (amplicon && !normal_filter_primers) {
                constexpr bool isrc = ISRC;
                const int ibeg = ((sr.isize != 0) ? (sr.frag_pos_L + P.primerlen) : ((isrc && (0x0 == (0x1 & sr.flag))) ? 0 : (sr.pos + P.primerlen)));
                const int iend = ((sr.isize != 0) ? (int)nnminus(sr.frag_pos_L + abs(sr.isize), P.primerlen) : ((isrc && (0x0 == (0x1 & sr.flag))) ? (int)nnminus(sr.rend, P.primerlen) : INT32_MAX));
                gate = (ibeg <= p && p < iend);
            }
            const bool cover = (valid & (p >= apos) & (p < rend) & gate);
            const bool hasL = DO_L && (p > apos), hasB = DO_B && (sym == my_ref);
            int inc = 0, incL = 0;
            if (proton) {
                if (cover) {
                    const AlnRec &a = R.alns[K(FR_W(aln))];
                    if (DO_B) inc = simple_base_value(P, a, p, R.quals + a.qbase, true);
                    if (DO_L) incL = (p > apos ? simple_link_value(R, P, a, p, R.quals + a.qbase, true) : 0);
                }
            } else { inc = base_value(q, P); incL = (int)nnminus(noindel80, nogap) + 1; }
            const wmask mm = DO_B ? BAL(cover && !hasB) : 0ull;
            if (DO_B && mm) {
                if (nq > MISQ_CAP - 64) flush_queue();
                if (cover && !hasB) { MisItem it; it.rank = K(FR_W(aln)); it.epos = p; it.symval = sym | (inc << 8); myq[nq + (int)__builtin_popcountll(mm & ((1ull << lane) - 1ull))] = it; }
                nq += (int)__builtin_popcountll(mm);
            }
            constexpr bool ONE_SIDE = (DO_B != DO_L);
            if (!ONE_SIDE ? cover : (DO_B ? (cover & hasB) : (cover & hasL))) {
                const int bmv = K(FR_W(bmv)), xbv = K(FR_W(xbv));
                const int bm_inc = (sym < 4 ? ((bmv >> (8 * sym)) & 0xFF) : (xbv & 0xFF)), xm_inc = (xbv >> 8) & 0xFF;
                segbias_simple<ISRC, STRAND, PLAIN>(Alink, Aref, P, sr, T, p, baq_p, baq2_p, ONE_SIDE ? DO_L : hasL, ONE_SIDE ? DO_B : hasB, incL, inc, xm_inc, bm_inc, amp1, amp2);
            }
        };
        if (DO_B) {
            int r0 = fetch(0), r1 = (1 < n ? fetch(1) : 0);
#if P2_AHEAD == 4
            int r2 = (2 < n ? fetch(2) : 0), r3 = (3 < n ? fetch(3) : 0);
            for (int j = 0; j < n; j += 4) {
                { const int v = r0; if (j + 4 < n) r0 = fetch(j + 4); one([&](int i) { return bcast(c[i], j); }, v); }
                if (j + 1 < n) { const int v = r1; if (j + 5 < n) r1 = fetch(j + 5); one([&](int i) { return bcast(c[i], j + 1); }, v); }
                if (j + 2 < n) { const int v = r2; if (j + 6 < n) r2 = fetch(j + 6); one([&](int i) { return bcast(c[i], j + 2); }, v); }
                if (j + 3 < n) { const int v = r3; if (j + 7 < n) r3 = fetch(j + 7); one([&](int i) { return bcast(c[i], j + 3); }, v); }
            }
#else
#ifdef UVC_P2_BASE_VECREC
            for (int j = 0; j < n; j += 2) {
                { const int v = r0; if (j + 2 < n) r0 = fetch(j + 2); one([&](int i) { return bcast(c[i], j); }, v); }
                if (j + 1 < n) { const int v = r1; if (j + 3 < n) r1 = fetch(j + 3); one([&](int i) { return bcast(c[i], j + 1); }, v); }
            }
#else
            typedef int v4i_ __attribute__((ext_vector_type(4)));
            typedef __attribute__((address_space(4))) const v4i_ *crec4;
            v4i_ a0, a1, a2, a3;
            const int kb = wave_uniform(k0), nb = wave_uniform(n);
            { crec4 q = (crec4)(R.frec2 + kb); a0 = q[0]; a1 = q[1]; a2 = q[2]; a3 = q[3]; }
            for (int j = 0; j < nb; j += 2) {
                { const int v = r0; if (j + 2 < nb) r0 = fetch(j + 2);
                  const v4i_ c0 = a0, c1 = a1, c2 = a2, c3 = a3;
                  if (j + 1 < nb) { crec4 q = (crec4)(R.frec2 + (kb + j + 1)); a0 = q[0]; a1 = q[1]; a2 = q[2]; a3 = q[3]; }
                  one([&](int i) { const v4i_ w = (i < 4 ? c0 : i < 8 ? c1 : i < 12 ? c2 : c3); return (int)w[i & 3]; }, v); }
                if (j + 1 < nb) { const int v = r1; if (j + 3 < nb) r1 = fetch(j + 3);
                  const v4i_ c0 = a0, c1 = a1, c2 = a2, c3 = a3;
                  if (j + 2 < nb) { crec4 q = (crec4)(R.frec2 + (kb + j + 2)); a0 = q[0]; a1 = q[1]; a2 = q[2]; a3 = q[3]; }
                  one([&](int i) { const v4i_ w = (i < 4 ? c0 : i < 8 ? c1 : i < 12 ? c2 : c3); return (int)w[i & 3]; }, v); }
            }
#endif
#endif
        } else {
            typedef int v4i_ __attribute__((ext_vector_type(4)));
            typedef __attribute__((address_space(4))) const v4i_ *crec4;
            v4i_ a0, a1, a2, a3;
            const int kb = wave_uniform(k0), nb = wave_uniform(n);
            { crec4 q = (crec4)(R.frec2 + kb); a0 = q[0]; a1 = q[1]; a2 = q[2]; a3 = q[3]; }
            for (int j = 0; j < nb; j++) {
                const v4i_ c0 = a0, c1 = a1, c2 = a2, c3 = a3;
                if (j + 1 < nb) { crec4 q = (crec4)(R.frec2 + (kb + j + 1)); a0 = q[0]; a1 = q[1]; a2 = q[2]; a3 = q[3]; }
                one([&](int i) { const v4i_ w = (i < 4 ? c0 : i < 8 ? c1 : i < 12 ? c2 : c3); return (int)w[i & 3]; }, 0);
            }
        }
        if (DO_B) Aref.fold();
        if (DO_L) Alink.fold();
    }
    };
    COARSE_T(ct1)
    run_list(std::false_type{}, std::false_type{}, 0);
    run_list(std::true_type{}, std::false_type{}, 1);
    run_list(std::false_type{}, std::true_type{}, 2);
    run_list(std::true_type{}, std::true_type{}, 3);
    if (DO_B && nq > 0) flush_queue();
    COARSE_T(ct2)
    if (SPLIT) {
        const SegAcc &A = (DO_B ? Aref : Alink);
#pragma unroll
        for (int f = 0; f < UVC_NSEG32; f++) if (A.s[f]) atomicAdd(&red[f][lane], A.s[f]);
#pragma unroll
        for (int f = 0; f < UVC_NSEG64; f++) if (A.l[f]) atomicAdd(&red64(red, f)[lane], (unsigned long long)A.l[f]);
        if (A.a1BQf) atomicAdd(&red[UVC_NSEG32 + 2 * UVC_NSEG64 + 0][lane], A.a1BQf);
        if (A.a1BQr) atomicAdd(&red[UVC_NSEG32 + 2 * UVC_NSEG64 + 1][lane], A.a1BQr);
        if (A.a2BQf) atomicAdd(&red[UVC_NSEG32 + 2 * UVC_NSEG64 + 2][lane], A.a2BQf);
        if (A.a2BQr) atomicAdd(&red[UVC_NSEG32 + 2 * UVC_NSEG64 + 3][lane], A.a2BQr);
        if (A.bq) atomicAdd(&red[UVC_NSEG32 + 2 * UVC_NSEG64 + 4][lane], A.bq);
        __syncthreads();
        if (!valid) return;
        const int sym = (DO_B ? my_ref : UVC_LINK_M), wv = (int)(threadIdx.x >> 6);
        for (int f = wv; f < UVC_NSEG32; f += 4) { const int v = red[f][lane]; if (v) S32(R, f, sym, x) = v; }
        for (int f = wv; f < UVC_NSEG64; f += 4) { const long long v = (long long)red64(red, f)[lane]; if (v) S64(R, f, sym, x) = v; }
        if (wv == 0) {
            const int b0 = UVC_NSEG32 + 2 * UVC_NSEG64;
            if (red[b0][lane]) VQP(R, UVC_VQ_a1BQf, sym, x) = red[b0][lane];
            if (red[b0 + 1][lane]) VQP(R, UVC_VQ_a1BQr, sym, x) = red[b0 + 1][lane];
            if (red[b0 + 2][lane]) VQP(R, UVC_VQ_a2BQf, sym, x) = red[b0 + 2][lane];
            if (red[b0 + 3][lane]) VQP(R, UVC_VQ_a2BQr, sym, x) = red[b0 + 3][lane];
            if (red[b0 + 4][lane]) BQS(R, sym, x) = red[b0 + 4][lane];
        }
        return;
    }
    if (!valid) return;
    if (DO_B) seg_store(R, Aref, my_ref, x);
    if (DO_L) seg_store(R, Alink, UVC_LINK_M, x);
#ifdef UVC_FRAG_COARSE
    asm volatile("s_waitcnt vmcnt(0)" ::: "memory");
    COARSE_T(ct3)
    if (lane == 0 && (wave % 2999) == 7) printf("coarse p2<%d,%d> wave %d prologue %llu lists %llu epilogue %llu\n", (int)DO_L, (int)DO_B, wave, ct1 - ct0, ct2 - ct1, ct3 - ct2);
#endif
}
template <bool DO_L, bool DO_B, bool PLAIN>
__global__ void __launch_bounds__(256) __attribute__((amdgpu_waves_per_eu(5))) k_p2_fast(RegionDev R, UvcParams P) {
    __shared__ int amp1[256 + AMP_LO], amp2[256 + AMP_LO];
    __shared__ MisItem misq[DO_B ? 4 : 1][DO_B ? MISQ_CAP : 1];
    p2_fast_body<DO_L, DO_B, PLAIN>(R, P, amp1, amp2, misq);
}
template <bool DO_L, bool DO_B, bool PLAIN>
__global__ void __launch_bounds__(256) __attribute__((amdgpu_waves_per_eu(4))) k_p2_fast_split(RegionDev R, UvcParams P) {
    __shared__ int amp1[256 + AMP_LO], amp2[256 + AMP_LO];
    __shared__ MisItem misq[DO_B ? 4 : 1][DO_B ? MISQ_CAP : 1];
    __shared__ __attribute__((aligned(8))) int red[P2_RED_SLOTS][64];
    p2_fast_body<DO_L, DO_B, PLAIN, true>(R, P, amp1, amp2, misq, red);
}

__global__ void __launch_bounds__(256) k_p2_mism(RegionDev R, UvcParams P) {
    const int n = imin(*R.mis_cnt, R.mis_cap);
    for (int t = blockIdx.x * blockDim.x + threadIdx.x; t < n; t += gridDim.x * blockDim.x) mis_apply(R, P, R.mis[t]);
}

DEV int indel_len_rusize_phred_dev(int indel_len, int repeatunit_size) {
    const int t[19] = { 0, 0, 3, 5, 6, 7, 8, 8, 9, 10, 10, 10, 11, 11, 11, 12, 12, 12, 13 };
    if (0 == (indel_len % repeatunit_size)) return t[imin(indel_len / repeatunit_size, 18)];
    return t[imin(indel_len, 18)];
}
DEV int indel_phred_dev(double ampfact, int rs, int rn) {
    const int region_size = rs * rn;
    const double num_slips = (region_size > 64 ? (double)(region_size - 8) : log1p(exp((double)region_size - (double)8))) * ampfact / ((double)(rs * rs));
    const double pr = (1.0 - 2.220446049250313e-16) / (num_slips + 1.0);
    return (int)floor(-10 * log(pr) / log(10.0));
}
DEV bool more_STR(int rulen1, int rc1, int rulen2, int rc2, int strmax) {
    if (rulen2 * rc2 == 0) return true;
    if (rulen1 > strmax || rulen2 > strmax) return (rulen1 < rulen2 || (rulen1 == rulen2 && rc1 > rc2));
    int rank1 = (rc1 <= 1 ? (-rc1 * rulen1) : ((rc1 - 1) * rulen1));
    int rank2 = (rc2 <= 1 ? (-rc2 * rulen1) : ((rc2 - 1) * rulen2));
    if (0 == rc1 || 0 == rulen1) rank1 = -100;
    if (0 == rc2 || 0 == rulen2) rank2 = -100;
    return rank1 > rank2;
}
DEV int ref_to_phredvalue_dev(int &n_units, int &max_rn, int &rs_at_max, const RegionDev &R, const UvcParams &P, int refidx, int max_phred, double ampfact, int oplen, int op) {
    const int n = (int)R.npos - 1;
    max_rn = 0; rs_at_max = 0;
    for (int rs = 1; rs <= P.indel_str_repeatsize_max; rs++) {
        int q = refidx;
        while (q + rs < n && R.refsym[q] == R.refsym[q + rs]) q++;
        const int rn = (q - refidx) / rs + 1;
        if (more_STR(rs, rn, rs_at_max, max_rn, P.indel_str_repeatsize_max)) { max_rn = rn; rs_at_max = rs; }
    }
    if (oplen == rs_at_max && op == C_DEL) ampfact *= P.indel_del_to_ins_err_ratio;
    const int decphred = indel_phred_dev(ampfact, rs_at_max, max_rn);
    if (rs_at_max * (max_rn - 1) >= 6 - 1) n_units = ((0 == oplen % rs_at_max) ? (oplen / rs_at_max) : ((1 == oplen) ? 1 : 0));
    else n_units = 1 + (oplen / 6);
    return max_phred - imin(max_phred, decphred) + indel_len_rusize_phred_dev(oplen, rs_at_max);
}
DEV int proton_cigarlen2phred(int cigarlen) { const int t[13] = { 0, 0, 9, 14, 18, 21, 23, 25, 27, 29, 30, 31, 32 }; return t[imin(cigarlen, 12)]; }

DEV void table_put(const RegionDev &R, Contrib *row, int sym, int v) {
    const uint16_t vv = (uint16_t)imin(imax(v, 0), 65535);
    if (sym <= UVC_BASE_NN) {
        if (row->bsym_p1 == 0 || row->bsym_p1 == sym + 1) { row->bval = (row->bsym_p1 == sym + 1) ? (uint16_t)imax((int)row->bval, (int)vv) : vv; row->bsym_p1 = (uint8_t)(sym + 1); }
        else atomicExch(R.err, UVCGPU_EDEVICE);
        return;
    }
    const int k = sym - UVC_LINK_M;
    if (row->lmask & (1 << k)) row->lval[k] = (uint16_t)imax((int)row->lval[k], (int)vv);
    else { row->lmask = (uint8_t)(row->lmask | (1 << k)); row->lval[k] = vv; }
}

template <bool BIAS>
__global__ void __launch_bounds__(64) k_p2_slow(RegionDev R, UvcParams P) {
    const int t = blockIdx.x * blockDim.x + threadIdx.x;
    if (t >= R.n_complex) return;
    const AlnRec a = R.alns[R.complex_ids[t]];
    const uint32_t *cigar = R.cigars + a.cigar_off;
    const uint8_t *bases = R.bases + a.seq_off, *quals = R.quals + a.seq_off;
    const bool proton = (UVC_PLATFORM_IONTORRENT == P.inferred_sequencing_platform);
    const int off = R.beg, rend = a.rend, n_cigar = a.n_cigar;
// ... 1989 lines not shown
    if (R->n_alns) hipLaunchKernelGGL(k_correct_bq, dim3((unsigned)((R->n_alns + 255) / 256)), dim3(256), 0, s, *R, bq_max, bq_inc);
}

__global__ void __launch_bounds__(256) k_pack_bq1(const uint8_t *bases, const uint8_t *quals, uint16_t *bq, int64_t n, int32_t *bad) {
    int any = 0, zero = 0;
    for (int64_t i = (int64_t)blockIdx.x * blockDim.x + threadIdx.x; i < n; i += (int64_t)gridDim.x * blockDim.x) {
        bq[i] = (uint16_t)(bases[i] | (quals[i] << 8));
        any |= (bases[i] > 4); zero |= (quals[i] == 0);
    }
    if (bad && __any(any) && (threadIdx.x & 63) == 0) *bad = 2;
    if (bad && __any(zero) && (threadIdx.x & 63) == 0) bad[1] = 1;
}
__global__ void __launch_bounds__(256) k_pack_bq(const uint8_t *bases, const uint8_t *quals, uint16_t *bq, int64_t n, int32_t *bad) {
    const int64_t n8 = n >> 3;
    unsigned long long over = 0, zero = 0;
    for (int64_t i = (int64_t)blockIdx.x * blockDim.x + threadIdx.x; i < n8; i += (int64_t)gridDim.x * blockDim.x) {
        const unsigned long long b = ((const unsigned long long *)bases)[i], q = ((const unsigned long long *)quals)[i];
        over |= (b & 0xF8F8F8F8F8F8F8F8ull) | (b & 0x0404040404040404ull & (((b | (b >> 1)) & 0x0101010101010101ull) << 2));
        zero |= (q - 0x0101010101010101ull) & ~q & 0x8080808080808080ull;
        uint4 o;
        o.x = (uint32_t)((b & 0xFF) | ((q & 0xFF) << 8) | (((b >> 8) & 0xFF) << 16) | (((q >> 8) & 0xFF) << 24));
        o.y = (uint32_t)(((b >> 16) & 0xFF) | (((q >> 16) & 0xFF) << 8) | (((b >> 24) & 0xFF) << 16) | (((q >> 24) & 0xFF) << 24));
        o.z = (uint32_t)(((b >> 32) & 0xFF) | (((q >> 32) & 0xFF) << 8) | (((b >> 40) & 0xFF) << 16) | (((q >> 40) & 0xFF) << 24));
        o.w = (uint32_t)(((b >> 48) & 0xFF) | (((q >> 48) & 0xFF) << 8) | (((b >> 56) & 0xFF) << 16) | (((q >> 56) & 0xFF) << 24));
        ((uint4 *)bq)[i] = o;
    }
    if (blockIdx.x == 0) for (int64_t i = (n8 << 3) + threadIdx.x; i < n; i += blockDim.x) { bq[i] = (uint16_t)(bases[i] | (quals[i] << 8)); over |= (bases[i] > 4); zero |= (quals[i] == 0); }
    if (bad && __any(over != 0) && (threadIdx.x & 63) == 0) *bad = 2;
    if (bad && __any(zero != 0) && (threadIdx.x & 63) == 0) bad[1] = 1;
}
extern "C" void uvc_launch_pack_bq(const uint8_t *bases, const uint8_t *quals, uint16_t *bq, int64_t n, int32_t *bad, hipStream_t s) {
    if (n <= 0) return;
    const bool aligned = !(((uintptr_t)bases | (uintptr_t)quals) & 7) && !((uintptr_t)bq & 15);
    if (getenv("UVCGPU_TIMING")) fprintf(stderr, "[uvcgpu pack_bq] %s\n", aligned ? "k_pack_bq" : "k_pack_bq1");
    if (aligned) hipLaunchKernelGGL(k_pack_bq, dim3((unsigned)std::min<int64_t>(((n >> 3) + 255) / 256 + 1, 16384)), dim3(256), 0, s, bases, quals, bq, n, bad);
    else hipLaunchKernelGGL(k_pack_bq1, dim3((unsigned)std::min<int64_t>((n + 255) / 256, 65536)), dim3(256), 0, s, bases, quals, bq, n, bad);
}
extern "C" void uvc_launch_build_p2list(const RegionDev *R, const int32_t *fast_rank, const int32_t *aln, const int32_t *cbeg, const int32_t *cend, const int32_t *qb, hipStream_t s) {
    if (R->n_fast2) hipLaunchKernelGGL(k_build_p2list, dim3(nblk(R->n_fast2, 256)), dim3(256), 0, s, *R, fast_rank, aln, cbeg, cend, qb);
}
extern "C" void uvc_launch_prelude(const RegionDev *R, const RawReads *W, const UvcParams *P, hipStream_t s) {
    if (R->n_alns && R->n_fast) hipLaunchKernelGGL(k_aln_bm, dim3(imin_h((int)nblk(R->n_alns, 256), 16384)), dim3(256), 0, s, *R, *W);
    if (R->n_alns) hipLaunchKernelGGL(k_aln_prelude, dim3(nblk(R->n_alns, 256)), dim3(256), 0, s, *R, *W, *P);
}
#define TIMED2(prof, kname, ...) do { hipStream_t s = s2; TIMED(prof, kname, __VA_ARGS__); } while (0)
#define TIMED3(prof, kname, ...) do { hipStream_t s = s3; TIMED(prof, kname, __VA_ARGS__); } while (0)
__global__ void __launch_bounds__(256) k_zero_state(char *slab, const ZeroPlane *planes, const uint8_t *dirty, int ndblk, int64_t npos) {
    const ZeroPlane zp = planes[blockIdx.x];
    const int b = (int)blockIdx.y;
    if (zp.fam >= 0 && !dirty[((size_t)zp.fam * NSYM + zp.sym) * ndblk + b]) return;
    const int64_t x0 = (int64_t)b << UVC_DIRTY_SHIFT, x1 = (x0 + ((int64_t)1 << UVC_DIRTY_SHIFT) < npos ? x0 + ((int64_t)1 << UVC_DIRTY_SHIFT) : npos);
    char *p0 = slab + zp.off + x0 * zp.elem, *p1 = slab + zp.off + x1 * zp.elem;
    char *a0 = (char *)(((uintptr_t)p0 + 15) & ~(uintptr_t)15), *a1 = (char *)((uintptr_t)p1 & ~(uintptr_t)15);
    if (a0 >= a1) { for (char *q = p0 + threadIdx.x; q < p1; q += 256) *q = 0; return; }
    for (char *q = p0 + threadIdx.x; q < a0; q += 256) *q = 0;
    const uint4 z = make_uint4(0u, 0u, 0u, 0u);
    for (uint4 *q = (uint4 *)a0 + threadIdx.x; q < (uint4 *)a1; q += 256) *q = z;
    for (char *q = a1 + threadIdx.x; q < p1; q += 256) *q = 0;
}
extern "C" void uvc_launch_zero_state(char *slab, const ZeroPlane *planes, int n_planes, uint8_t *dirty, int ndblk, int64_t npos, hipStream_t s) {
    if (n_planes <= 0 || ndblk <= 0) return;
    hipLaunchKernelGGL(k_zero_state, dim3((unsigned)n_planes, (unsigned)ndblk), dim3(256), 0, s, slab, planes, dirty, ndblk, npos);
}
__global__ void __launch_bounds__(256) k_check_dirty(RegionDev R, unsigned long long *n_bad) {
    const int64_t x = (int64_t)blockIdx.x * blockDim.x + threadIdx.x;
    const int s = (int)blockIdx.y;
    if (x >= R.npos) return;
    const int b = (int)(x >> UVC_DIRTY_SHIFT);
    long long any[UVC_N_DIRTY_FAMILIES] = { 0, 0, 0 };
#define X(g, m) { constexpr int fill = UVC_GROUPS[UVC_F_##g].fill; \
                  if (fill >= 0) for (int pl = 0; pl < uvc_group_sym_planes(UVC_F_##g); pl++) any[fill >= 0 ? fill : 0] |= R.m[((size_t)pl * NSYM + s) * R.npos + x]; }
    UVC_SLAB_MEMBERS(X)
#undef X
    int bad = 0;
    for (int fam = 0; fam < UVC_N_DIRTY_FAMILIES; fam++)
        if (any[fam] && !(fam == UVC_FILL_CORE && sym_always_filled(s)) && !R.dirty[((size_t)fam * NSYM + s) * R.ndblk + b]) bad++;
    if (bad) atomicAdd(n_bad, (unsigned long long)bad);
}
extern "C" void uvc_launch_check_dirty(const RegionDev *R, unsigned long long *d_n_bad, hipStream_t s) {
    hipLaunchKernelGGL(k_check_dirty, dim3((unsigned)((R->npos + 255) / 256), NSYM), dim3(256), 0, s, *R, d_n_bad);
}

struct AccForms { bool vcf, proton, split_windows, p2_plain, frag_plain, h16, fam, digest, duplex; int n_gen; };
static AccForms acc_forms(const RegionDev *R, const UvcParams *P, int n_dup) {
    AccForms F;
    F.vcf = (P->inferred_is_vcf_generated != 0);
    F.proton = (UVC_PLATFORM_IONTORRENT == P->inferred_sequencing_platform);
    const char *sp_env = getenv("UVCGPU_SPLIT");
    const long long per_window = (long long)R->n_fast2 * (R->max_p2_span + 64) / (R->npos > 0 ? R->npos : 1);
    F.split_windows = sp_env ? (atoi(sp_env) != 0) : (R->nwin < 4 * 1024 && per_window >= 1024);
    F.p2_plain = !F.proton && !R->any_amplicon && !(P->primerlen > 0 && !(0x2 & P->primer_flag)) && (P->central_readlen >= P->microadjust_median_readlen_thres);
    F.frag_plain = F.vcf && !F.proton && !(0x1 & P->fam_flag) && !(P->microadjust_padded_deletion_flag & 0x1);
    F.h16 = (R->max_frag_depth < 65536) && !R->frag32;
    F.fam = (R->n_generic_fs > 0);
    F.digest = (R->fam_digest != nullptr);
    F.duplex = F.fam && F.vcf && n_dup;
    F.n_gen = F.proton ? R->n_frags : R->n_sweep;
    return F;
}
static void print_forms(const AccForms &F) {
    fprintf(stderr, "[uvcgpu accumulate] forms prep=%s p2=%s%s frag=%s,%s,%s family=%s duplex=%s frag_generic=%s\n",
            !F.vcf ? "none" : F.split_windows ? "split" : "wave",
            !F.vcf ? "none" : F.split_windows ? "split" : "wave", !F.vcf ? "" : F.p2_plain ? ",plain" : ",generic",
            F.h16 ? "h16" : "b32", (F.split_windows && F.h16) ? "split" : "wave", F.frag_plain ? "plain" : "generic",
            !F.fam ? "none" : F.digest ? "digest" : "generic",
            !F.duplex ? "none" : F.digest ? "digest" : "generic",
            !F.n_gen ? "none" : F.proton ? "all" : "sweep");
}
static bool prep_scan_wanted() {
    const char *e = getenv("UVCGPU_PREP");
    return !(e && !strcmp(e, "window"));
}
static bool prep_scan_exact(const RegionDev *R, const UvcParams *P) {
    const long long m_str = llabs((long long)(int32_t)((uint32_t)P->indel_str_phred_per_region * 10u)) + 1;
    const long long m_non = llabs((long long)(int32_t)((uint32_t)P->indel_nonSTR_phred_per_base * 10u));
    const long long m = (m_str > m_non ? m_str : m_non);
    return ((long long)R->max_p2_span + PSCAN_TILE) * m / 10 + 2 < (1LL << 30);
}
template <bool DO_L, bool DO_B>
static void launch_p2_fast(const char *kname, const AccForms &F, const RegionDev *R, const UvcParams *P, unsigned nwin, UvcProf *prof, hipStream_t s) {
    if (F.split_windows && F.p2_plain) TIMED(prof, kname, hipLaunchKernelGGL((k_p2_fast_split<DO_L, DO_B, true>), dim3(R->nwin), dim3(256), 0, s, *R, *P));
    else if (F.split_windows) TIMED(prof, kname, hipLaunchKernelGGL((k_p2_fast_split<DO_L, DO_B, false>), dim3(R->nwin), dim3(256), 0, s, *R, *P));
    else if (F.p2_plain) TIMED(prof, kname, hipLaunchKernelGGL((k_p2_fast<DO_L, DO_B, true>), dim3(nwin), dim3(256), 0, s, *R, *P));
    else TIMED(prof, kname, hipLaunchKernelGGL((k_p2_fast<DO_L, DO_B, false>), dim3(nwin), dim3(256), 0, s, *R, *P));
}

extern "C" void uvc_launch_accumulate(const RegionDev *R, const UvcParams *P, int half_ratio_phred, const int32_t *dup_units, int n_dup, const int64_t *dup_off, int64_t n_dup_work,
                                      const UvcAccStreams *st, UvcProf *prof) {
    const hipStream_t s = st->s, side = st->side, side3 = st->side3;
    const hipEvent_t e_fork = st->e_fork, e_join = st->e_join, e_fork2 = st->e_fork2, e_join3 = st->e_join3, e_stat = st->e_stat, e_alleles = st->e_alleles;
    const unsigned nwin = nblk(R->npos, 256);
    const AccForms F = acc_forms(R, P, n_dup);
    if (getenv("UVCGPU_TIMING")) print_forms(F);
    if (prof) prof->n = 0;
    hipStream_t s2 = (side ? side : s);
    hipStream_t s3 = ((side && side3) ? side3 : s2);
    {
        const int64_t n = 2 * (int64_t)R->nwin * 4;
        TIMED(prof, "k_win_index", hipLaunchKernelGGL(k_win_index, dim3(nblk(n, 256)), dim3(256), 0, s, *R, 1, 5));
        if (R->n_generic_fs) hipLaunchKernelGGL(k_win_index, dim3(nblk(2 * (int64_t)R->nwin, 256)), dim3(256), 0, s, *R, 7, 8);
    }
    if (P->inferred_is_vcf_generated && R->n_fast) TIMED(prof, "k_prep_sums", hipLaunchKernelGGL(k_prep_sums, dim3(nblk(R->npos, PSUM_TILE)), dim3(256), 0, s, *R, *P));
    if (P->inferred_is_vcf_generated) {
        if (side && R->n_complex) { hipEventRecord(e_fork, s); hipStreamWaitEvent(s2, e_fork, 0); }
        if (R->n_complex) TIMED2(prof, "k_prep_slow", hipLaunchKernelGGL(k_prep_slow, dim3(R->n_complex), dim3(64), 0, s, *R, *P));
        if (side && R->n_complex) hipEventRecord(e_join, s2);
        const bool scan = !F.split_windows && prep_scan_wanted() && prep_scan_exact(R, P);
        if (getenv("UVCGPU_TIMING")) fprintf(stderr, "[uvcgpu accumulate] prep kernel %s\n", F.split_windows ? "k_prep_fast<true>" : scan ? "k_prep_scan" : "k_prep_fast<false>");
        if (F.split_windows) TIMED(prof, "k_prep_fast", hipLaunchKernelGGL(k_prep_fast<true>, dim3(R->nwin), dim3(256), 0, s, *R, *P));
        else if (scan) TIMED(prof, "k_prep_scan", hipLaunchKernelGGL(k_prep_scan, dim3(nblk(R->npos, PSCAN_TILE)), dim3(256), 0, s, *R, *P));
        else TIMED(prof, "k_prep_fast", hipLaunchKernelGGL(k_prep_fast<false>, dim3(nwin), dim3(256), 0, s, *R, *P));
        if (side && R->n_complex) hipStreamWaitEvent(s, e_join, 0);
    }
    if (P->inferred_is_vcf_generated) TIMED(prof, "k_thres", hipLaunchKernelGGL(k_thres, dim3(nblk(R->npos, 256)), dim3(256), 0, s, *R, *P, half_ratio_phred));
    if (side) { hipEventRecord(e_fork, s); hipStreamWaitEvent(s2, e_fork, 0); if (s3 != s2) hipStreamWaitEvent(s3, e_fork, 0); }
    if (P->inferred_is_vcf_generated && R->n_complex) TIMED2(prof, "k_p2_slow_walk", hipLaunchKernelGGL(k_p2_slow<true>, dim3(nblk(R->n_complex, 64)), dim3(64), 0, s, *R, *P));
    if (R->n_complex) TIMED3(prof, "k_p2_slow_table", hipLaunchKernelGGL(k_p2_slow<false>, dim3(nblk(R->n_complex, 64)), dim3(64), 0, s, *R, *P));
    TIMED3(prof, "k_fragstat_fast", hipLaunchKernelGGL(k_fragstat_fast, dim3(nblk(R->n_frags, 256)), dim3(256), 0, s, *R, *P));
    TIMED3(prof, "k_win_index_frag", hipLaunchKernelGGL(k_win_index, dim3(nblk(2 * (int64_t)R->nwin * 2, 256)), dim3(256), 0, s, *R, 5, 7));
    if (R->n_sweep) TIMED3(prof, "k_fragstat_sweep", hipLaunchKernelGGL(k_fragstat_sweep, dim3(R->n_sweep), dim3(64), 0, s, *R, *P, R->sweep_frags, (const int32_t *)nullptr, R->n_sweep));
    TIMED3(prof, "k_fragstat_overflow", hipLaunchKernelGGL(k_fragstat_sweep, dim3(imin_h(R->n_frags, 65535)), dim3(64), 0, s, *R, *P, (const int32_t *)R->overflow_frags, (const int32_t *)R->n_overflow, 0));
    if (UVC_PLATFORM_IONTORRENT != P->inferred_sequencing_platform)
        TIMED3(prof, "k_frag_sums", hipLaunchKernelGGL(k_frag_sums, dim3(nblk(R->npos, FSUM_TILE), 2), dim3(256), 0, s, *R, *P));
    if (P->inferred_is_vcf_generated) {
        launch_p2_fast<false, true>("k_p2_fast_base", F, R, P, nwin, prof, s);
        if (side) { hipEventRecord(e_fork2, s); hipStreamWaitEvent(s2, e_fork2, 0); }
        TIMED2(prof, "k_p2_mism", hipLaunchKernelGGL(k_p2_mism, dim3(2048), dim3(256), 0, s, *R, *P));
        launch_p2_fast<true, false>("k_p2_fast_link", F, R, P, nwin, prof, s);
    }
    if (side) {
        hipEventRecord(e_join, s2); hipStreamWaitEvent(s, e_join, 0);
        if (s3 != s2) { hipEventRecord(e_join3, s3); hipStreamWaitEvent(s, e_join3, 0); hipStreamWaitEvent(s2, e_join3, 0); }
    }
    const GapWork &G = R->gap;
    hipMemsetAsync(G.n_inc, 0, 16, s2);
    if (P->inferred_is_vcf_generated && G.n_ev > 0) {
        TIMED2(prof, "k_gap", {
            hipLaunchKernelGGL(k_gap_keys, dim3(nblk(G.n_ev, 256)), dim3(256), 0, s, *R);
            uvc_gap_sort(G.sort_tmp, G.sort_tmp_bytes, G.ckey, G.ckey_s, G.cval, G.cval_s, (size_t)G.n_ev, 58, s);
            hipMemsetAsync(G.ikey, 0xFF, sizeof(unsigned long long) * (size_t)G.inc_cap, s);
            hipLaunchKernelGGL(k_gap_alleles, dim3(nblk(G.n_ev, 64)), dim3(64), 0, s, *R, *P);
            if (side) hipEventRecord(e_alleles, s);
            uvc_gap_sort(G.sort_tmp, G.sort_tmp_bytes, G.ikey, G.ikey_s, G.ival, G.ival_s, (size_t)G.inc_cap, 64, s);
            hipLaunchKernelGGL(k_gap_rows, dim3(nblk(G.inc_cap, 256)), dim3(256), 0, s, *R);
            hipLaunchKernelGGL(k_gap_rows_add, dim3(nblk(G.inc_cap, 256)), dim3(256), 0, s, *R);
            hipLaunchKernelGGL(k_gap_rows_fin, dim3(nblk(G.n_ev, 256)), dim3(256), 0, s, *R);
        });
    }
    if (side && !(P->inferred_is_vcf_generated && G.n_ev > 0)) hipEventRecord(e_alleles, s2);
    if (R->n_generic_fs) TIMED3(prof, "k_fam_stat", hipLaunchKernelGGL(k_fam_stat, dim3(nblk(R->n_generic_fs, 64)), dim3(64), 0, s, *R, *P));
    if (side) { hipEventRecord(e_stat, s3); hipEventRecord(e_fork2, s2); }
    if (P->inferred_is_vcf_generated && R->n_complex) TIMED(prof, "k_p2_items", hipLaunchKernelGGL(k_p2_items, dim3(R->n_complex), dim3(64), 0, s, *R, *P));
    {
        if (F.n_gen) TIMED(prof, "k_frag_generic", hipLaunchKernelGGL(k_frag_generic, dim3(imin_h(F.n_gen, 1 << 20), imin_h((R->max_frag_span + 63) / 64, 16)), dim3(64), 0, s, *R, *P, F.proton ? (const int32_t *)nullptr : R->sweep_frags, F.n_gen));
    }
    {
        const bool plain = F.frag_plain;
        if (F.split_windows && F.h16 && plain) TIMED(prof, "k_frag", hipLaunchKernelGGL(k_frag16_split<true>, dim3(R->nwin), dim3(256), 0, s, *R, *P));
        else if (F.split_windows && F.h16) TIMED(prof, "k_frag", hipLaunchKernelGGL(k_frag16_split<false>, dim3(R->nwin), dim3(256), 0, s, *R, *P));
        else if (plain && F.h16) TIMED(prof, "k_frag", hipLaunchKernelGGL(k_frag16<true>, dim3(nwin), dim3(256), 0, s, *R, *P));
        else if (plain) TIMED(prof, "k_frag", hipLaunchKernelGGL(k_frag<true>, dim3(nwin), dim3(256), 0, s, *R, *P));
        else if (F.h16) TIMED(prof, "k_frag", hipLaunchKernelGGL(k_frag16<false>, dim3(nwin), dim3(256), 0, s, *R, *P));
        else TIMED(prof, "k_frag", hipLaunchKernelGGL(k_frag<false>, dim3(nwin), dim3(256), 0, s, *R, *P));
    }
    if (R->n_generic_fs) {
        if (side) { hipStreamWaitEvent(s, e_stat, 0); hipStreamWaitEvent(s, e_alleles, 0); }
        if (F.digest) TIMED(prof, "k_fam_p4", { hipLaunchKernelGGL(k_fam_p4d, dim3(nblk(R->npos, 64)), dim3(256), 0, s, *R, *P);
                                               hipLaunchKernelGGL(k_fam_p4d_rest, dim3(R->n_generic_fs), dim3(64), 0, s, *R, *P); });
        else TIMED(prof, "k_fam_p4", hipLaunchKernelGGL(k_fam_p4, dim3(nblk(R->n_generic_work, 256)), dim3(256), 0, s, *R, *P));
        if (P->inferred_is_vcf_generated) {
            if (F.digest) TIMED(prof, "k_fam_p5", hipLaunchKernelGGL(k_fam_p5d, dim3(nblk(R->npos, 64)), dim3(256), 0, s, *R, *P));
            else TIMED(prof, "k_fam_p5", hipLaunchKernelGGL(k_fam_p5, dim3(nblk(R->n_generic_work, 256)), dim3(256), 0, s, *R, *P));
            if (F.duplex && F.digest) TIMED(prof, "k_duplex", hipLaunchKernelGGL(k_duplex_d, dim3(n_dup), dim3(64), 0, s, *R, dup_units, n_dup, dup_off, n_dup_work));
            else if (F.duplex) TIMED(prof, "k_duplex", hipLaunchKernelGGL(k_duplex, dim3(nblk(n_dup_work, 256)), dim3(256), 0, s, *R, *P, dup_units, n_dup, dup_off, n_dup_work));
        }
    }
    if (P->inferred_is_vcf_generated) TIMED(prof, "k_p5b", hipLaunchKernelGGL(k_p5b, dim3(nblk(R->npos * 2, 256)), dim3(256), 0, s, *R, *P));
    if (side) hipStreamWaitEvent(s, e_fork2, 0);
}

__global__ void __launch_bounds__(256) k_math_probe_acc(int op, long long n, const double *in, int n_in, double *out, int n_out) {
    __shared__ double p2p_s[128];
    const bool with_table = (op == UVC_PROBE_phred2prob_tab);
    if (with_table) { for (int i = threadIdx.x; i < 128; i += 256) p2p_s[i] = phred2prob(i); __syncthreads(); }
    const long long i = (long long)blockIdx.x * blockDim.x + threadIdx.x;
    if (i >= n) return;
    const int v = (int)in[i * n_in];
    out[i * n_out] = (op == UVC_PROBE_proton_cigarlen2phred) ? (double)proton_cigarlen2phred(cig_len((uint32_t)v << 4)) :
                     phred2prob_tab(with_table ? p2p_s : nullptr, v);
}
extern "C" int uvc_launch_math_probe_acc(int op, int64_t n, const double *in, int n_in, double *out, int n_out, hipStream_t s) {
    if (op < UVC_PROBE_proton_cigarlen2phred || op >= UVC_PROBE_END || n < 1 || n > (1LL << 32) || n_in < 1 || n_out < 1 || !in || !out) return -1;
    hipLaunchKernelGGL(k_math_probe_acc, dim3((unsigned)((n + 255) / 256)), dim3(256), 0, s, op, (long long)n, in, n_in, out, n_out);
    return 0;
}
```

### uvc_amd/csrc/uvc_kernels_score.hip

```cpp
#include <algorithm>
#include "uvc_launch.h"
#include "uvc_score_rows.h"
#include "uvc_collectives.h"

#define DBL_EPS 2.220446049250313e-16
#define FLT_EPS 1.1920928955078125e-07

DEV double dmin(double a, double b) { return a < b ? a : b; }
DEV double dmax(double a, double b) { return a > b ? a : b; }
DEV double dbetween(double v, double a, double b) { return dmin(dmax(a, v), b); }
DEV double nnminus_d(double a, double b) { return a > b ? a - b : 0.0; }
DEV double phred2nat(double x) { return (log(10.0) / 10.0) * x; }
DEV double numstates2phred(double x) { return (10.0 / log(10.0)) * log(x); }
DEV int i32_as_x86(double v) { return (v > -2147483649.0 && v < 2147483648.0) ? (int)v : (int)0x80000000; }
DEV int numstates2deciphred(double x) { return i32_as_x86(round((100.0 / log(10.0)) * log(x))); }
DEV double prob2odds(double p) { return p / (1.0 - p); }
DEV double logit2(double a, double b) { return log(prob2odds((a + DBL_EPS) / (a + b + 2.0 * DBL_EPS))); }

DEV double binom_llr(double prob, double a, double b) {
    prob = (prob + DBL_EPS) / (1.0 + (2.0 * DBL_EPS));
    a += DBL_EPS; b += DBL_EPS;
    const double A = (prob) * (a + b), B = (1.0 - prob) * (a + b);
    if (a > A) return 10.0 / log(10.0) * (a * log(a / A) + b * log(b / B));
    return 0.0;
// ... 263 lines not shown
#pragma unroll
        for (int kk = 0; kk < 8; kk++) bd[kk] = (kk == k ? v : bd[kk]);
    }
    return tot;
}
DEV int gate_count(const RegionDev &R, const UvcParams &P, const ScoreCtx &C, long long g) {
    bool no_base;
    const int zpos = group_zpos(C, g, no_base), st = (int)(g & 1);
    if (no_base && st == UVC_BASE_SYMBOL) return 0;
    const int refpos = (st == UVC_BASE_SYMBOL ? zpos - 1 : zpos);
    const int64_t x = refpos - R.beg;
    const int refsymbol = group_refsymbol(R, zpos, st), nsym = st_count(st);
    int bd[8], totBDP = 0;
    const bool all_out = group_all_out(C, g);
    if (all_out || P.tumor_vcf_is_provided) {
#pragma unroll
        for (int k = 0; k < 8; k++) bd[k] = 0;
    } else {
        const unsigned mask = type_mask(R, st, x, refsymbol);
        if (P.min_altdp_thres > 0 && !(mask & (mask - 1u))) return 0;
        totBDP = masked_bdepths(R, st, x, mask, bd);
    }
    bool pos_rescued = false;
    if (P.tumor_vcf_is_provided && C.n_tkeys) { const long long q = tkey_lower_bound(C, refpos, 0); pos_rescued = (q < C.n_tkeys && C.tkeys[q].refpos == refpos); }
    int n = 0;
#pragma unroll
    for (int k = 0; k < 8; k++) {
        if (k >= nsym) break;
        const int s = st_symbol(st, k);
        if (gate_b(P, s, refsymbol, bd[k], totBDP, all_out, pos_rescued)) { long long first; int src; n += allele_source(C, P.tumor_vcf_is_provided, refpos, s, first, src); }
    }
    return n;
}

__global__ void __launch_bounds__(GS_BLOCK) k_gate_scan(RegionDev R, UvcParams P, ScoreCtx C, Stage S, long long *total_records) {
    __shared__ long long sh_cnt[GATE_TILE + GATE_TILE / 8];
    __shared__ unsigned long long sh_wave[4], sh_prefix;
    __shared__ int sh_tile;
    if (threadIdx.x == 0) sh_tile = (int)atomicAdd(&S.cnt[CNT_ticket1], 1u);
    __syncthreads();
    const int tile = sh_tile;
    const long long ngroups = 2LL * (C.pos_end - C.pos_beg);
    const long long base = (long long)tile * GATE_TILE;
#pragma unroll 1
    for (int i = 0; i < GATE_ITEMS; i++) {
        const int j = i * GS_BLOCK + (int)threadIdx.x;
        const long long g = base + j;
        const long long n = (g < ngroups ? (long long)gate_count(R, P, C, g) : 0LL);
        sh_cnt[j + (j >> 3)] = n | (n > 0 ? (1LL << 32) : 0LL);
    }
    __syncthreads();
    long long v[GATE_ITEMS]; unsigned long long s = 0;
    { const int j0 = (int)threadIdx.x * GATE_ITEMS;
#pragma unroll
      for (int i = 0; i < GATE_ITEMS; i++) { v[i] = sh_cnt[j0 + i + (j0 >> 3)]; s += (unsigned long long)v[i]; } }
    unsigned long long total = 0;
    const unsigned long long excl = block_excl<GS_BLOCK / 64>(s, sh_wave, total);
    if (threadIdx.x < 64) { const unsigned long long p = cs_lookback(S.status1, tile, total, (int)threadIdx.x, R.err); if (threadIdx.x == 0) sh_prefix = p; }
    __syncthreads();
    long long run = (long long)(sh_prefix + excl);
    const long long g0 = base + (long long)threadIdx.x * GATE_ITEMS;
#pragma unroll
    for (int i = 0; i < GATE_ITEMS; i++) {
        const long long g = g0 + i;
        if (g < ngroups) { C.offsets[g] = run; if (PK_FLAGS(v[i])) C.active[PK_FLAGS(run)] = (int)g; }
        run += v[i];
    }
    if (g0 <= ngroups - 1 && ngroups - 1 < g0 + GATE_ITEMS) { C.offsets[ngroups] = (long long)(sh_prefix + total); *total_records = PK_COUNT((long long)(sh_prefix + total)); }
}

__global__ void __launch_bounds__(128) k_enum(RegionDev R, UvcParams P, ScoreCtx C, Stage S) {
    WIN_PROLOGUE
    const long long gi = (long long)blockIdx.x * blockDim.x + threadIdx.x;
    if (gi >= n_active || gi >= S.gcap) return;
    const long long g = C.active[a_base + gi];
    const long long rec0 = PK_COUNT(C.offsets[g]) - r_base, nrec = PK_COUNT(C.offsets[g + 1]) - r_base - rec0;
    if (nrec <= 0 || rec0 + nrec > C.capacity || rec0 + nrec > S.cap) { GR_(nrec, gi) = 0; return; }
    bool no_base_;
    const int zpos = group_zpos(C, g, no_base_), st = (int)(g & 1);
    const int refpos = (st == UVC_BASE_SYMBOL ? zpos - 1 : zpos);
    const int64_t x = refpos - R.beg;
    const int refidx = zpos - R.beg, refsize = (int)R.npos - 1;
    const int refsymbol = group_refsymbol(R, zpos, st), nsym = st_count(st);
    unsigned mask = type_mask(R, st, x, refsymbol);
    int bd[8], cd[8];
    const int totBDP = masked_bdepths(R, st, x, mask, bd);
    const bool all_out = group_all_out(C, g);
#pragma unroll
    for (int k = 0; k < 8; k++) cd[k] = 0;
    for (unsigned m = mask & 0xFFu; m; m &= m - 1u) {
        const int k = __builtin_ctz(m), s = st_symbol_at(st, k);
        const int v = imax(FAP(R, 0, UVC_FAM_cDP1, s, x), FAP(R, 0, UVC_FAM_cDP12, s, x)) + imax(FAP(R, 1, UVC_FAM_cDP1, s, x), FAP(R, 1, UVC_FAM_cDP12, s, x));
#pragma unroll
        for (int kk = 0; kk < 8; kk++) cd[kk] = (kk == k ? v : cd[kk]);
    }
    { const int kr = st_index(st, refsymbol); int rb = 0;
#pragma unroll
      for (int k = 0; k < 8; k++) rb = (k == kr ? bd[k] : rb);
      GR_(refbdp, gi) = rb; }
    { const size_t blk = (size_t)(x >> UVC_DIRTY_SHIFT);
      unsigned fi = 0, du = 0;
#pragma unroll
      for (int k = 0; k < 8; k++) {
          const int s = st_symbol(st, k < nsym ? k : nsym - 1);
          const unsigned f1 = R.dirty[((size_t)NSYM + s) * R.ndblk + blk], f2 = R.dirty[((size_t)2 * NSYM + s) * R.ndblk + blk];
          if ((mask >> k) & 1u) { fi |= f1; du |= f2; }
      }
      if (fi) mask |= GM_FI;
      if (du) mask |= GM_DUP;
      if (R.p5flag[x]) mask |= GM_P5F;
      if (R.p5flag[(size_t)R.npos + x]) mask |= GM_P5R; }
    GR_(x, gi) = (int)x; GR_(zpos, gi) = zpos; GR_(st, gi) = st; GR_(refsym, gi) = refsymbol; GR_(mask, gi) = (int)mask; GR_(rec0, gi) = (int)rec0; GR_(nrec, gi) = (int)nrec;
    const int prev1 = ((refidx >= 2) ? (int)R.refsym[refidx - 2] : UVC_BASE_NN), prev2 = ((refidx >= 3) ? (int)R.refsym[refidx - 3] : UVC_BASE_NN);
    const int next1 = ((refidx < refsize) ? (int)R.refsym[refidx] : UVC_BASE_NN), next2 = ((refidx + 1 < refsize) ? (int)R.refsym[refidx + 1] : UVC_BASE_NN);
    const bool hp1 = (prev1 == refsymbol && next1 == refsymbol), hp2 = (prev2 == refsymbol && next2 == refsymbol);
    GR_(hp, gi) = (hp1 ? (hp2 ? 20 : 10) : 0);
    const int nrtr = (int)R.npos;
    const RtrLite rtr1 = load_rtr(R, imax(refpos - R.beg, 3) - 3), rtr2 = load_rtr(R, imin(refpos - R.beg + 3, nrtr - 1));
    GR_(r1t, gi) = rtr1.tracklen; GR_(r1u, gi) = rtr1.unitlen; GR_(r1a, gi) = rtr1.anyTR_tracklen; GR_(r2t, gi) = rtr2.tracklen; GR_(r2u, gi) = rtr2.unitlen; GR_(r2a, gi) = rtr2.anyTR_tracklen;
    long long rec = rec0;
    bool indel_rec = false;
#pragma unroll
    for (int k = 0; k < 8; k++) {
        if (k >= nsym) break;
        const int s = st_symbol(st, k);
        if (!gate_b(P, s, refsymbol, bd[k], totBDP, all_out, true )) continue;
        long long first; int src;
        const int m = allele_source(C, P.tumor_vcf_is_provided, refpos, s, first, src);
        indel_rec = indel_rec || is_ins(s) || is_del(s);
        for (int ai = 0; ai < m && rec < rec0 + nrec; ai++, rec++) {
            RH_(gi, rec) = (int)gi; RH_(symbol, rec) = s; RH_(src, rec) = src; RH_(idx, rec) = (src ? (int)(first + ai) : -1); RH_(bdepth, rec) = bd[k]; RH_(cdepth, rec) = cd[k];
        }
    }
    int ins_cdepth = 0, del_cdepth = 0, ins1_cdepth = 0, del1_cdepth = 0;
    if (indel_rec) {
        const int64_t xz = zpos - R.beg;
#pragma unroll
        for (int k = 1; k < 7; k++) {
            const int s = st_symbol(UVC_LINK_SYMBOL, k);
            const int cdz = imax(FAP(R, 0, UVC_FAM_cDP1, s, xz), FAP(R, 0, UVC_FAM_cDP12, s, xz)) + imax(FAP(R, 1, UVC_FAM_cDP1, s, xz), FAP(R, 1, UVC_FAM_cDP12, s, xz));
            if (is_ins(s)) { ins_cdepth += cdz; if (UVC_LINK_I1 == s) ins1_cdepth += cdz; } else { del_cdepth += cdz; if (UVC_LINK_D1 == s) del1_cdepth += cdz; }
        }
    }
    GR_(insc, gi) = ins_cdepth; GR_(delc, gi) = del_cdepth; GR_(ins1c, gi) = ins1_cdepth; GR_(del1c, gi) = del1_cdepth;
    int ru_size = 0, repeatnum = 0;
    if (indel_rec) indel_context(R, refidx, P.indel_str_repeatsize_max, ru_size, repeatnum);
    GR_(rusize, gi) = ru_size; GR_(repnum, gi) = repeatnum;
    if (rec != rec0 + nrec) atomicExch(R.err, UVCGPU_EDEVICE);
    atomicMax(&S.cnt[CNT_nvalid], (unsigned)(rec0 + nrec));
}

#define GATHER_PLANES 4
__global__ void __launch_bounds__(256) k_gather(RegionDev R, ScoreCtx C, Stage S) {
    WIN_PROLOGUE
    const long long gi = (long long)blockIdx.x * blockDim.x + threadIdx.x;
    if (gi >= n_active || gi >= S.gcap) return;
    const int nrec = GR_(nrec, gi);
    if (nrec == 0) return;
    const int64_t x = GR_(x, gi);
    const int st = GR_(st, gi), rec0 = GR_(rec0, gi);
    const unsigned mask = (unsigned)GR_(mask, gi);
    const int kf = __builtin_ctz(mask);
    long long c[GATHER_PLANES][8];
#pragma unroll
    for (int q = 0; q < GATHER_PLANES; q++) {
        const int u = (int)blockIdx.y * GATHER_PLANES + q;
// ... 1141 lines not shown
```

### uvc_amd/csrc/uvc_launch.h

```cpp
#ifndef UVC_LAUNCH_H
#define UVC_LAUNCH_H
#include "uvc_device.h"

struct RawReads {
    const int32_t *pos, *endpos, *mpos, *isize, *nm, *l_qseq, *n_cigar, *frag, *fs, *dflag, *kind, *fast_rank;
    const uint16_t *flag; const uint8_t *mapq;
    const int64_t *seq_off, *cigar_off, *table_off, *item_off, *gap_off;
};
static_assert(sizeof(RawReads) == 19 * sizeof(void *), "RawReads is 19 device pointers");
struct UvcProf { int on; int n; const char *name[32]; hipEvent_t ev[32][2]; };
static inline int uvc_prof_begin(UvcProf *p, const char *name, hipStream_t s) {
    if (!p || !p->on || p->n >= 32) return -1;
    const int i = p->n++;
    p->name[i] = name;
    if (!p->ev[i][0]) { hipEventCreate(&p->ev[i][0]); hipEventCreate(&p->ev[i][1]); }
    hipEventRecord(p->ev[i][0], s);
    return i;
}
static inline void uvc_prof_end(UvcProf *p, int i, hipStream_t s) { if (i >= 0) hipEventRecord(p->ev[i][1], s); }
struct UvcScoreRangeDev { int beg, end, first, flags; };
static_assert(sizeof(UvcScoreRangeDev) == 16, "the host uploads the range table as 16-byte rows");
struct UvcChunkDev { long long g0, ng, r0, nr; };
static_assert(sizeof(UvcChunkDev) == 32, "the host reads the chunk table back as 32-byte rows");
struct UvcRangeRow { int x0, first; };
static_assert(sizeof(UvcRangeRow) == 8, "the host uploads the range table as 8-byte rows");
struct UvcRangeCursor { int rid = -1, first = 0, next = 0, x0 = 0; };
DEV void uvc_range_find(UvcRangeCursor &g, const UvcRangeRow *tab, int n_ranges, long long i) {
    if (i >= g.first && i < g.next) return;
    int lo = 0, hi = n_ranges;
    while (hi - lo > 1) { const int mid = (lo + hi) >> 1; if (tab[mid].first <= i) lo = mid; else hi = mid; }
    g.rid = lo; g.first = tab[lo].first; g.x0 = tab[lo].x0; g.next = tab[lo + 1].first;
}
struct UvcUnitSpan { int lo, hi; };
static_assert(sizeof(UvcUnitSpan) == 8, "the host sizes the span scratch as 8-byte rows");
struct UvcFragSpan { int loF, hiF, loR, hiR; };
static_assert(sizeof(UvcFragSpan) == 16, "the host sizes the fragment span scratch as 16-byte rows");

struct UvcScoreIn {
    const RegionDev *R; const UvcParams *P; const UvcScoreRequest *req;
    const UvcIndelAllele *alleles; const int32_t *allele_rows; int64_t n_alleles;
    const UvcGapRow *gap_rows; const uint8_t *gap_seq; const UvcTumorKey *tkeys;
    char *scratch; const int32_t *force_sites;
    const UvcScoreRangeDev *ranges; int64_t n_ranges, n_compact;
};
struct UvcAccStreams { hipStream_t s, side, side3; hipEvent_t e_fork, e_join, e_fork2, e_join3, e_stat, e_alleles; };
#define UVC_SCAN_TILE 256
static inline int64_t uvc_scan_tiles(int64_t n) { return (n + UVC_SCAN_TILE - 1) / UVC_SCAN_TILE; }

extern "C" {
void uvc_launch_correct_bq(const RegionDev *R, int bq_max, int bq_inc, hipStream_t s);
void uvc_launch_pack_bq(const uint8_t *bases, const uint8_t *quals, uint16_t *bq, int64_t n, int32_t *bad, hipStream_t s);
void uvc_launch_build_p2list(const RegionDev *R, const int32_t *fast_rank, const int32_t *aln, const int32_t *cbeg, const int32_t *cend, const int32_t *qb, hipStream_t s);
void uvc_launch_prelude(const RegionDev *R, const RawReads *W, const UvcParams *P, hipStream_t s);
void uvc_launch_zero_state(char *slab, const ZeroPlane *planes, int n_planes, uint8_t *dirty, int ndblk, int64_t npos, hipStream_t s);
void uvc_launch_check_dirty(const RegionDev *R, unsigned long long *d_n_bad, hipStream_t s);
void uvc_launch_accumulate(const RegionDev *R, const UvcParams *P, int half_ratio_phred, const int32_t *dup_units, int n_dup, const int64_t *dup_off, int64_t n_dup_work,
                           const UvcAccStreams *st, UvcProf *prof);
void uvc_launch_hap_cand(const RegionDev *R, const HapWork *H, int units, hipStream_t s);
void uvc_launch_hap_events(const RegionDev *R, const UvcParams *P, const HapWork *H, int units, int n_cand, hipStream_t s);
int uvc_launch_score(const UvcScoreIn *in, int32_t *d_fields, int64_t capacity, int32_t *d_fields_kept, hipStream_t s);
size_t uvc_score_scratch_bytes(int64_t npos_scored, int64_t capacity);
size_t uvc_score_scratch_zero_bytes(int64_t npos_scored, int64_t capacity);
int uvc_launch_score_gate(const UvcScoreIn *in, int64_t chunk_records, int64_t tab_cap, hipStream_t s);
int uvc_launch_score_chunk(const UvcScoreIn *in, char *set, int64_t chunk_records, int with_kept, const UvcChunkDev *win, int64_t win_groups, hipStream_t s);
size_t uvc_score_set_bytes(int64_t chunk_records, int64_t ngroups, int with_kept);
size_t uvc_score_set_bytes_per_record(void);
int32_t *uvc_score_set_fields(char *set, int64_t chunk_records, int64_t ngroups, int kept);
size_t uvc_score_stream_pos_bytes(int64_t npos_scored, int64_t tab_cap);
size_t uvc_score_stream_table_offset(int64_t npos_scored);
void uvc_launch_check_presence(const RegionDev *R, unsigned long long *d_n_bad, hipStream_t s);
void uvc_launch_block_stats(const RegionDev *R, const UvcParams *P, int64_t x0, int64_t n, int32_t *d_out, hipStream_t s);
void uvc_launch_block_stats_windows(const RegionDev *R, const UvcParams *P, const long long *d_win, int n_win, int64_t n, int32_t *d_out, hipStream_t s);
void uvc_launch_block_scan(int *d_a, int n, hipStream_t s);
void uvc_launch_tile_sums(const int32_t *d_in, int64_t n, int chunks, int32_t *d_tile_sums, hipStream_t s);
void uvc_launch_tile_prefix(const int32_t *d_in, int n, int chunks, const int32_t *d_tile_pref, int32_t *d_out, hipStream_t s);
void uvc_launch_sum_fold(const long long *d_parts, int shards, int cells, long long *d_out, hipStream_t s);
void uvc_launch_coverage(const RegionDev *R, const UvcRangeRow *d_tab, int n_ranges, int64_t n_total, const int32_t *thr, int n_thr, long long *d_out, long long *d_scratch, int64_t scratch_rows, hipStream_t s);
const char *uvc_coverage_name(int id);
int64_t uvc_coverage_scratch_rows(int n_ranges, int64_t n_total);
void uvc_launch_errprofile(const RegionDev *R, const UvcRangeRow *d_tab, int n_ranges, int64_t n_total, int min_depth, int max_alt_permille, long long *d_out, long long *d_scratch, hipStream_t s);
const char *uvc_errprofile_level_name(int id);
int64_t uvc_errprofile_scratch_cells(void);
void uvc_launch_famstats(const RegionDev *R, const int32_t *pos, const int32_t *endpos, const int32_t *fs_of, UvcUnitSpan *d_span, const UvcFamilyRange *d_ranges, int n_ranges, long long *d_rows, hipStream_t s);
const char *uvc_famstats_name(int id);
void uvc_launch_fragprofile(const RegionDev *R, const RawReads *W, const UvcFragmentProfileRequest *req, UvcFragSpan *d_fspan, UvcUnitSpan *d_uspan, const UvcFamilyRange *d_ranges, int n_ranges,
                            long long *d_out, long long *d_parts, hipStream_t s);
const char *uvc_fragprofile_name(int id);
int64_t uvc_fragprofile_copies(void);
void uvc_launch_readprofile_depth(const RegionDev *R, const RawReads *W, int64_t n_bases, int min_mapq, int32_t *d_dx, int32_t *d_x, int32_t *d_scratch, hipStream_t s);
void uvc_launch_readprofile_status(const RegionDev *R, const UvcRangeRow *d_tab, int n_ranges, int min_depth, int max_alt_permille, int32_t *d_dx, const int32_t *d_x, uint8_t *d_status,
                                   long long *d_parts, int32_t *d_scratch, hipStream_t s);
void uvc_launch_readprofile_bin(const RegionDev *R, const RawReads *W, int64_t n_bases, int min_mapq, const uint8_t *d_status, long long *d_parts, long long *d_out, const int32_t *d_scratch, hipStream_t s);
const char *uvc_readprofile_class_name(int c);
int64_t uvc_readprofile_copies(void);
int64_t uvc_readprofile_scratch_ints(int64_t n_alns, int64_t npos);
void uvc_launch_sitereads_count(const RegionDev *R, const RawReads *W, const int32_t *d_sites, int n_sites, const UvcSiteReadsRequest *req, int32_t *d_counts, int32_t *d_scratch, hipStream_t s);
void uvc_launch_sitereads_write(const RegionDev *R, const RawReads *W, const int32_t *d_sites, int n_sites, const UvcSiteReadsRequest *req, int32_t *d_scratch, UvcSiteRead *d_rows, hipStream_t s);
int64_t uvc_sitereads_scratch_ints(int64_t n_alns, int64_t n_sites);
int64_t uvc_sitereads_rows_at(int64_t n_alns, int64_t n_sites);
const char *uvc_sitereads_kind_name(int k);
void uvc_launch_clipsites_find(const RegionDev *R, const RawReads *W, const UvcRangeRow *d_tab, int n_ranges, const UvcClipSitesRequest *req, long long *d_totals, int32_t *d_pos,
                               int32_t *d_keys, int64_t key_room, int32_t *d_scratch, hipStream_t s);
void uvc_launch_clipsites_fill(const RegionDev *R, const RawReads *W, const UvcRangeRow *d_tab, int n_ranges, const UvcClipSitesRequest *req, const int32_t *d_pos, const int32_t *d_keys,
                               int n_sites, const int32_t *d_scratch, long long *d_rows, UvcClipRead *d_reads, hipStream_t s);
int64_t uvc_clipsites_pos_ints(int64_t npos);
int64_t uvc_clipsites_scratch_ints(int64_t n_alns, int64_t npos);
int64_t uvc_clipsites_sites_at(int64_t n_alns, int64_t npos);
int64_t uvc_clipsites_reads_at(int64_t n_alns, int64_t npos);
const char *uvc_clipsites_name(int id);
void uvc_launch_callable_count(const RegionDev *R, const UvcRangeRow *d_tab, int n_ranges, int64_t n_total, const UvcCallableRequest *req, unsigned char *d_mask, int *d_blocks, hipStream_t s);
void uvc_launch_callable_emit(const RegionDev *R, const UvcRangeRow *d_tab, int n_ranges, int64_t n_total, const unsigned char *d_mask, const int *d_blocks, UvcCallableRun *d_runs, hipStream_t s);
int64_t uvc_callable_blocks(int64_t n_total);
const char *uvc_callable_name(int bit);
enum UvcProbeOp {
    UVC_PROBE_phred2nat, UVC_PROBE_numstates2phred, UVC_PROBE_numstates2deciphred, UVC_PROBE_prob2odds, UVC_PROBE_logit2,
    UVC_PROBE_binom_llr,
    UVC_PROBE_dp4,
    UVC_PROBE_indel_len_rusize_phred_s,
    UVC_PROBE_indel_phred_s,
    UVC_PROBE_more_STR_s,
    UVC_PROBE_norm_fa, UVC_PROBE_i32_as_x86,
    UVC_PROBE_het_lodq,
    UVC_PROBE_normv_quals,
    UVC_PROBE_normv_quals2,
    UVC_PROBE_symbols_mutated,
    UVC_PROBE_sscs_phred,
    UVC_PROBE_infer_max_qual,
    UVC_PROBE_infer_max_qual_regs,
    UVC_PROBE_infer_max_qual_one,
    UVC_PROBE_infer_max_qual_regs_one,
    UVC_PROBE_proton_cigarlen2phred, UVC_PROBE_phred2prob, UVC_PROBE_phred2prob_tab,
    UVC_PROBE_END
};
int uvc_launch_math_probe(int op, int64_t n, const double *in, int n_in, double *out, int n_out, hipStream_t s);
int uvc_launch_math_probe_acc(int op, int64_t n, const double *in, int n_in, double *out, int n_out, hipStream_t s);
void uvc_launch_msi(const RegionDev *R, const UvcRangeRow *d_tab, int n_ranges, int64_t n_total, const UvcMsiRequest *req, int *d_blocks, int32_t *d_heads, int32_t *d_rows, int64_t room, hipStream_t s);
int64_t uvc_msi_blocks(int64_t n_total);
const char *uvc_msi_name(int id);
size_t uvc_gap_sort_tmp_bytes(size_t n);
int uvc_gap_sort(void *tmp, size_t tmp_bytes, const unsigned long long *kin, unsigned long long *kout, const unsigned long long *vin, unsigned long long *vout, size_t n, int end_bit, hipStream_t s);
// ... 12 lines not shown
```

Measured before the change: 119.2 million.

## Defer LINK_M p2 accumulation to windows with indel occupancy until demanded

Result: faster. 124.5 million (median of 6 runs) (+4.5%).

```diff
diff --git a/uvc_amd/csrc/uvc_device.h b/uvc_amd/csrc/uvc_device.h
--- a/uvc_amd/csrc/uvc_device.h
+++ b/uvc_amd/csrc/uvc_device.h
@@ -156,6 +156,7 @@
     uint8_t *p5flag;
     uint8_t *dirty; int32_t ndblk;
     uint32_t *occ;
+    uint8_t *link_need, *link_done;
     uint32_t *fam_digest;
     Contrib *table;
     int32_t *ir_list;
diff --git a/uvc_amd/csrc/uvc_host.cpp b/uvc_amd/csrc/uvc_host.cpp
--- a/uvc_amd/csrc/uvc_host.cpp
+++ b/uvc_amd/csrc/uvc_host.cpp
@@ -86,6 +86,7 @@
     RegionDev R;
     int32_t *d_dup_units = nullptr; int64_t *d_dup_off = nullptr; int n_dup = 0; int64_t n_dup_work = 0;
     bool has_reads = false, accumulated = false;
+    UvcLinkState link; int link_split = 0;
     bool reads_given = false;
     Buf<uint8_t> d_dirty{this}; Buf<ZeroPlane> d_zero_planes{this}; int64_t zero_planes_npos = 0;
     int64_t dirty_npos = 0;
@@ -119,6 +120,22 @@
     return 0;
 }
 
+static void link_report(const uvcgpu_region *r, const char *scope) {
+    std::vector<uint8_t> done((size_t)r->R.nwin);
+    if (hipStreamSynchronize(r->stream) != hipSuccess || hipMemcpy(done.data(), r->R.link_done, done.size(), hipMemcpyDeviceToHost) != hipSuccess) { (void)hipGetLastError(); return; }
+    long long n = 0;
+    for (uint8_t b : done) n += (b != 0);
+    fprintf(stderr, "[uvcgpu link_complete] scope=%s done=%lld of %d windows\n", scope, n, (int)r->R.nwin);
+}
+static int link_complete(uvcgpu_region *r, int scope, const int32_t *d_xs = nullptr, int64_t n_xs = 0) {
+    if (!r->link.wants(r->accumulated, r->state_released, scope)) return 0;
+    uvc_launch_link_complete(&r->R, &r->P, r->link_split, scope, d_xs, n_xs, nullptr, r->stream);
+    if (hipGetLastError() != hipSuccess) return fail(UVCGPU_EDEVICE, "completion pass of LINK_M: launch failed");
+    r->link.enqueued(scope);
+    if (getenv("UVCGPU_TIMING")) link_report(r, scope == UVC_LINK_ALL ? "all" : "positions");
+    return 0;
+}
+
 namespace {
 template <class T> int dev_alloc(uvcgpu_region *r, size_t count, T **out, bool zero = false) {
     const size_t n = std::max<size_t>(count, 1);
@@ -196,6 +213,7 @@
     return 0;
 }
 
+static size_t dirty_bytes(const RegionDev &R) { return (size_t)3 * NSYM * (size_t)R.ndblk; }
 static int configure_region(uvcgpu_region *r, int32_t tid, int32_t beg, int32_t end, const char *refseq) {
     r->tid = tid; r->beg = beg; r->end = end + 1; r->npos = (int64_t)end - beg + 1;
     r->refstring.assign(refseq, (size_t)(end - beg));
@@ -212,7 +230,7 @@
         const size_t work_bytes = uvc_rtr_work_bytes(r->npos, vmax, smax, bqm, &scan_tmp);
         if (r->d_refsym.fit(n + 1) != hipSuccess || r->d_rtr.fit(n_rtr) != hipSuccess || r->d_rtr0.fit(n_rtr) != hipSuccess || r->d_fsum.fit(2 * UVC_FSUM_N * n) != hipSuccess
             || r->d_win.fit(16 * (size_t)((r->npos + 63) / 64)) != hipSuccess || r->d_baq.fit(2 * n) != hipSuccess || r->d_state.fit(r->L.total) != hipSuccess || r->d_rtrwork.fit(work_bytes) != hipSuccess
-            || r->d_dirty.fit((size_t)3 * NSYM * (size_t)((r->npos >> UVC_DIRTY_SHIFT) + 2)) != hipSuccess) return fail(UVCGPU_ENOMEM, "hipMalloc(region planes) failed");
+            || r->d_dirty.fit(uvc_link_marks_bytes((size_t)3 * NSYM * (size_t)((r->npos >> UVC_DIRTY_SHIFT) + 2), (r->npos + 63) / 64)) != hipSuccess) return fail(UVCGPU_ENOMEM, "hipMalloc(region planes) failed");
         uvc_rtr_bind(&r->rw, r->d_rtrwork, r->npos, vmax, smax, bqm, scan_tmp);
         r->npos_cap = r->npos;
     }
@@ -239,6 +257,8 @@
 #undef X
     R.bucket = (int32_t *)(b + r->L.bucket_off); R.p5flag = (uint8_t *)(b + r->L.p5flag_off); R.occ = (uint32_t *)(b + r->L.occ_off);
     R.dirty = r->d_dirty; R.ndblk = (int32_t)((r->npos + ((int64_t)1 << UVC_DIRTY_SHIFT) - 1) >> UVC_DIRTY_SHIFT);
+    R.link_need = r->d_dirty + uvc_link_marks_off(dirty_bytes(R)); R.link_done = R.link_need + uvc_link_marks_stride(R.nwin);
+    r->link.planes_zeroed();
     R.err = r->d_err;
     HIP_OK(hipMemsetAsync(R.err, 0, 4, r->stream));
     return 0;
@@ -512,7 +532,6 @@
 }
 
 static int zero_state(uvcgpu_region *r, hipStream_t s) {
-    const size_t n_dirty = (size_t)3 * NSYM * (size_t)r->R.ndblk;
     const bool selective = (r->dirty_npos == r->npos && !getenv("UVCGPU_FILL_ALL"));
     r->dirty_npos = 0;
     if (selective) {
@@ -531,7 +550,8 @@
     } else {
         HIP_OK(hipMemsetAsync(r->d_state, 0, r->buckets_clean ? r->L.bucket_off : r->L.total, s));
     }
-    HIP_OK(hipMemsetAsync(r->d_dirty, 0, n_dirty, s));
+    HIP_OK(hipMemsetAsync(r->d_dirty, 0, uvc_link_marks_bytes(dirty_bytes(r->R), r->R.nwin), s));
+    r->link.planes_zeroed();
     return 0;
 }
 
@@ -551,8 +571,13 @@
     }
     const int half = (int)std::round((10.0 / std::log(10.0)) * std::log(r->P.indel_del_to_ins_err_ratio)) / 2;
     const UvcAccStreams st = { r->stream, r->side, r->side3, r->e_fork, r->e_join, r->e_fork2, r->e_join3, r->e_stat, r->e_alleles };
-    uvc_launch_accumulate(&r->R, &r->P, half, r->d_dup_units, r->n_dup, r->d_dup_off, r->n_dup_work, &st, &r->prof);
+    const char *lk_env = getenv("UVCGPU_LINK");
+    const bool link_eager = (lk_env && !strcmp(lk_env, "eager")) || !uvc_acc_p2_plain(&r->R, &r->P);
+    r->link_split = uvc_acc_split_windows(&r->R);
+    uvc_launch_accumulate(&r->R, &r->P, half, r->d_dup_units, r->n_dup, r->d_dup_off, r->n_dup_work, &st, link_eager ? 1 : 0, &r->prof);
     HIP_OK(hipGetLastError());
+    r->link.accumulated(link_eager);
+    if (getenv("UVCGPU_TIMING")) link_report(r, link_eager ? "all" : "indel");
     r->buckets_clean = (r->P.inferred_is_vcf_generated != 0);
     r->dirty_npos = r->npos;
     r->accumulated = true; r->gap_ready = false; r->hap_ready = false;
@@ -614,6 +639,7 @@
     if (!r || !dst || g < 0 || g >= UVC_NUM_FIELD_GROUPS) return fail(UVCGPU_EINVAL, "bad argument");
     if (uvc_group_in_slab(g)) { const int rcg = planes_guard(r, "fetch"); if (rcg) return rcg; }
     if ((int64_t)uvc_group_bytes(g, r->npos) != dst_bytes) return fail(UVCGPU_EINVAL, "bad destination size");
+    { const int rcl = link_complete(r, uvc_link_fetch_scope(g)); if (rcl) return rcl; }
     int rc = uvcgpu_region_sync(r);
     if (rc) return rc;
     const void *src = (g == UVC_F_RTR) ? (const void *)(r->accumulated ? r->d_rtr : r->d_rtr0)  : (g == UVC_F_BAQ) ? (const void *)r->d_baq : (const void *)(r->d_state + r->L.off[g]);
@@ -640,6 +666,7 @@
     if (!tmp.get(&d_xs, (size_t)n)) return fail(UVCGPU_ENOMEM, "hipMalloc(column positions) failed");
     if (!tmp.get(&d_out, (size_t)n * ncol)) return fail(UVCGPU_ENOMEM, "hipMalloc(columns) failed");
     hipError_t e = hipMemcpyAsync(d_xs, xs.data(), sizeof(int32_t) * (size_t)n, hipMemcpyHostToDevice, r->stream);
+    if (e == hipSuccess) { const int rcl = link_complete(r, uvc_link_columns_scope(), d_xs, n); if (rcl) return rcl; }
     if (e == hipSuccess) { uvc_launch_gather_columns(base, first, elem, r->npos, d_xs, n, d_out, r->stream); e = hipGetLastError(); }
     if (e == hipSuccess) e = hipMemcpyAsync(dst, d_out, sizeof(long long) * (size_t)n * ncol, hipMemcpyDeviceToHost, r->stream);
     if (e == hipSuccess) e = hipStreamSynchronize(r->stream);
@@ -944,6 +971,7 @@
         if (rq.pos_beg < r->beg + (rq.base_at_pos_beg ? 1 : 0) || rq.pos_end > r->end - 1 || rq.pos_end < rq.pos_beg) return fail(UVCGPU_EINVAL, "score range outside the region");
         npos_scored = (int64_t)rq.pos_end - rq.pos_beg;
     }
+    { const int rcl = link_complete(r, uvc_link_score_scope(rq.all_out, r->P.should_output_all, r->P.tumor_vcf_is_provided, rq.n_force_sites, r->P.min_altdp_thres)); if (rcl) return rcl; }
     { int rc0 = gap_tables(r); if (rc0) return rc0; }
     UvcIndelAllele *d_al = nullptr; int32_t *d_al_row = nullptr; UvcTumorKey *d_tk = nullptr; int32_t *d_fs = nullptr; UvcScoreRangeDev *d_rg = nullptr;
     auto no_room = [&] { return fail(UVCGPU_EDEVICE, std::string("hipMalloc(score request): ") + hipGetErrorString(p.tmp->last)); };
diff --git a/uvc_amd/csrc/uvc_kernels_acc.hip b/uvc_amd/csrc/uvc_kernels_acc.hip
--- a/uvc_amd/csrc/uvc_kernels_acc.hip
+++ b/uvc_amd/csrc/uvc_kernels_acc.hip
@@ -68,6 +68,20 @@
     if (A.a2BQf) VQP(R, UVC_VQ_a2BQf, sym, x) = A.a2BQf;
     if (A.a2BQr) VQP(R, UVC_VQ_a2BQr, sym, x) = A.a2BQr;
     if (A.bq) BQS(R, sym, x) = A.bq;
+}
+
+DEV constexpr bool seg_is_adp(int f) { return f == UVC_S_aDPff || f == UVC_S_aDPfr || f == UVC_S_aDPrf || f == UVC_S_aDPrr; }
+template <bool WITH5>
+DEV void seg_add_link(const RegionDev &R, const SegAcc &A, int64_t x) {
+    if (WITH5 && A.bq) BQS(R, UVC_LINK_M, x) += A.bq;
+#pragma unroll
+    for (int f = 0; f < UVC_NSEG32; f++) if (A.s[f] && (WITH5 || !seg_is_adp(f))) S32(R, f, UVC_LINK_M, x) += A.s[f];
+#pragma unroll
+    for (int f = 0; f < UVC_NSEG64; f++) if (A.l[f]) S64(R, f, UVC_LINK_M, x) += A.l[f];
+    if (A.a1BQf) VQP(R, UVC_VQ_a1BQf, UVC_LINK_M, x) += A.a1BQf;
+    if (A.a1BQr) VQP(R, UVC_VQ_a1BQr, UVC_LINK_M, x) += A.a1BQr;
+    if (A.a2BQf) VQP(R, UVC_VQ_a2BQf, UVC_LINK_M, x) += A.a2BQf;
+    if (A.a2BQr) VQP(R, UVC_VQ_a2BQr, UVC_LINK_M, x) += A.a2BQr;
 }
 
 struct PosThres { int t[UVC_NTHRES]; };
@@ -1019,11 +1033,16 @@
 #define P2_AHEAD 2
 #endif
 #define MISQ_CAP 192
-#define P2_RED_SLOTS (UVC_NSEG32 + 2 * UVC_NSEG64 + 5)
+#define P2_RED_LINK5 (UVC_NSEG32 + 2 * UVC_NSEG64 + 5)
+#define P2_RED_SLOTS (P2_RED_LINK5 + 5)
 DEV unsigned long long *red64(int (*red)[64], int f) { return (unsigned long long *)&red[UVC_NSEG32 + 2 * f][0]; }
 template <bool DO_L, bool DO_B, bool PLAIN, bool SPLIT = false>
 DEV void p2_fast_body(const RegionDev &R, const UvcParams &P, int *amp1, int *amp2, MisItem (*misq)[DO_B ? MISQ_CAP : 1], int (*red)[64] = nullptr) {
     COARSE_T(ct0)
+    if (DO_L) {
+        if (SPLIT) { const int w = xcd_block(); if (!uvc_link_window_runs(R.link_need[w], R.link_done[w])) return; }
+        else { const int b = xcd_block(); if (!(((const uint32_t *)R.link_need)[b] & ~((const uint32_t *)R.link_done)[b] & 0x01010101u)) return; }
+    }
     {
         for (int v = (int)threadIdx.x - AMP_LO; v < 256; v += 256) {
             const int d1 = P.bias_thres_PFBQ1 * P.bias_thres_PFBQ1, d2 = P.bias_thres_PFBQ2 * P.bias_thres_PFBQ2;
@@ -1036,6 +1055,7 @@
     const int wave = SPLIT ? wave_uniform((int)xcd_block()) : wave_uniform((int)((xcd_block() * blockDim.x + threadIdx.x) >> 6));
     const int64_t x0 = (int64_t)wave * 64;
     if (x0 >= R.npos) return;
+    if (DO_L && !SPLIT && !uvc_link_window_runs(R.link_need[wave], R.link_done[wave])) return;
     if (SPLIT) { for (int i2 = threadIdx.x; i2 < P2_RED_SLOTS * 64; i2 += 256) (&red[0][0])[i2] = 0; __syncthreads(); }
     const int w0 = R.beg + (int)x0;
     const int p = w0 + lane;
@@ -1050,10 +1070,12 @@
     else { for (int f = 0; f < UVC_NTHRES; f++) T.t[f] = 0; }
     SegAcc Aref, Alink;
     Aref.zero(); Alink.zero();
+    constexpr bool L5_BASE = DO_B && PLAIN, L5_LINK = DO_L && !PLAIN;
     int noindel80 = 80;
-    if (DO_L && valid && x > 0) noindel80 = imin(80, imin(RTRP(R, UVC_RTR_indelphred, x - 1), RTRP(R, UVC_RTR_indelphred, x)));
+    if ((DO_L || L5_BASE) && valid && x > 0) noindel80 = imin(80, imin(RTRP(R, UVC_RTR_indelphred, x - 1), RTRP(R, UVC_RTR_indelphred, x)));
     MisItem *myq = misq[DO_B ? (threadIdx.x >> 6) : 0];
     int nq = 0;
+    int l5_bq = 0;
     auto flush_queue = [&]() {
         int base = 0;
         if (lane == 0) base = atomicAdd(R.mis_cnt, nq);
@@ -1068,6 +1090,7 @@
     auto run_list = [&](auto IS, auto ST, int cls) {
     constexpr bool ISRC = decltype(IS)::value, STRAND = decltype(ST)::value;
     const int lo = wave_uniform(win_lo(R, 1 + cls, (int)(x0 >> 6))), hi = wave_uniform(win_hi(R, 1 + cls, (int)(x0 >> 6)));
+    int l5_dp = 0;
     for (int k0 = lo + (SPLIT ? 64 * (int)(threadIdx.x >> 6) : 0); k0 < hi; k0 += (SPLIT ? 256 : 64)) {
         int c[16];
         if (DO_B) load_words(R.frec2 + (k0 + lane), k0 + lane < hi, c);
@@ -1113,6 +1136,7 @@
                 if (cover && !hasB) { MisItem it; it.rank = K(FR_W(aln)); it.epos = p; it.symval = sym | (inc << 8); myq[nq + (int)__builtin_popcountll(mm & ((1ull << lane) - 1ull))] = it; }
                 nq += (int)__builtin_popcountll(mm);
             }
+            if (L5_BASE) { const wmask ml = BAL(cover & (p > apos)); addm(l5_dp, ml); l5_bq += selm(ml, incL); }
             constexpr bool ONE_SIDE = (DO_B != DO_L);
             if (!ONE_SIDE ? cover : (DO_B ? (cover & hasB) : (cover & hasL))) {
                 const int bmv = K(FR_W(bmv)), xbv = K(FR_W(xbv));
@@ -1169,6 +1193,11 @@
         if (DO_B) Aref.fold();
         if (DO_L) Alink.fold();
     }
+    if (L5_BASE && l5_dp) {
+        constexpr int f = (STRAND ? (ISRC ? UVC_S_aDPrr : UVC_S_aDPrf) : (ISRC ? UVC_S_aDPfr : UVC_S_aDPff));
+        if (SPLIT) atomicAdd(&red[P2_RED_LINK5 + cls][lane], l5_dp);
+        else if (valid) S32(R, f, UVC_LINK_M, x) = l5_dp;
+    }
     };
     COARSE_T(ct1)
     run_list(std::false_type{}, std::false_type{}, 0);
@@ -1180,32 +1209,44 @@
     if (SPLIT) {
         const SegAcc &A = (DO_B ? Aref : Alink);
 #pragma unroll
-        for (int f = 0; f < UVC_NSEG32; f++) if (A.s[f]) atomicAdd(&red[f][lane], A.s[f]);
+        for (int f = 0; f < UVC_NSEG32; f++) if (A.s[f] && !(DO_L && !L5_LINK && seg_is_adp(f))) atomicAdd(&red[f][lane], A.s[f]);
 #pragma unroll
         for (int f = 0; f < UVC_NSEG64; f++) if (A.l[f]) atomicAdd(&red64(red, f)[lane], (unsigned long long)A.l[f]);
         if (A.a1BQf) atomicAdd(&red[UVC_NSEG32 + 2 * UVC_NSEG64 + 0][lane], A.a1BQf);
         if (A.a1BQr) atomicAdd(&red[UVC_NSEG32 + 2 * UVC_NSEG64 + 1][lane], A.a1BQr);
         if (A.a2BQf) atomicAdd(&red[UVC_NSEG32 + 2 * UVC_NSEG64 + 2][lane], A.a2BQf);
         if (A.a2BQr) atomicAdd(&red[UVC_NSEG32 + 2 * UVC_NSEG64 + 3][lane], A.a2BQr);
-        if (A.bq) atomicAdd(&red[UVC_NSEG32 + 2 * UVC_NSEG64 + 4][lane], A.bq);
+        if ((DO_B || L5_LINK) && A.bq) atomicAdd(&red[UVC_NSEG32 + 2 * UVC_NSEG64 + 4][lane], A.bq);
+        if (L5_BASE && l5_bq) atomicAdd(&red[P2_RED_LINK5 + 4][lane], l5_bq);
         __syncthreads();
+        if (DO_L && threadIdx.x == 0) R.link_done[xcd_block()] = 1;
         if (!valid) return;
         const int sym = (DO_B ? my_ref : UVC_LINK_M), wv = (int)(threadIdx.x >> 6);
-        for (int f = wv; f < UVC_NSEG32; f += 4) { const int v = red[f][lane]; if (v) S32(R, f, sym, x) = v; }
-        for (int f = wv; f < UVC_NSEG64; f += 4) { const long long v = (long long)red64(red, f)[lane]; if (v) S64(R, f, sym, x) = v; }
+        auto put = [](auto &cell, auto v) { if (DO_L) cell += v; else cell = v; };
+        for (int f = wv; f < UVC_NSEG32; f += 4) { const int v = red[f][lane]; if (v) put(S32(R, f, sym, x), v); }
+        for (int f = wv; f < UVC_NSEG64; f += 4) { const long long v = (long long)red64(red, f)[lane]; if (v) put(S64(R, f, sym, x), v); }
         if (wv == 0) {
             const int b0 = UVC_NSEG32 + 2 * UVC_NSEG64;
-            if (red[b0][lane]) VQP(R, UVC_VQ_a1BQf, sym, x) = red[b0][lane];
-            if (red[b0 + 1][lane]) VQP(R, UVC_VQ_a1BQr, sym, x) = red[b0 + 1][lane];
-            if (red[b0 + 2][lane]) VQP(R, UVC_VQ_a2BQf, sym, x) = red[b0 + 2][lane];
-            if (red[b0 + 3][lane]) VQP(R, UVC_VQ_a2BQr, sym, x) = red[b0 + 3][lane];
-            if (red[b0 + 4][lane]) BQS(R, sym, x) = red[b0 + 4][lane];
+            if (red[b0][lane]) put(VQP(R, UVC_VQ_a1BQf, sym, x), red[b0][lane]);
+            if (red[b0 + 1][lane]) put(VQP(R, UVC_VQ_a1BQr, sym, x), red[b0 + 1][lane]);
+            if (red[b0 + 2][lane]) put(VQP(R, UVC_VQ_a2BQf, sym, x), red[b0 + 2][lane]);
+            if (red[b0 + 3][lane]) put(VQP(R, UVC_VQ_a2BQr, sym, x), red[b0 + 3][lane]);
+            if ((DO_B || L5_LINK) && red[b0 + 4][lane]) put(BQS(R, sym, x), red[b0 + 4][lane]);
+        }
+        if (L5_BASE && wv == 1) {
+            const int l0 = P2_RED_LINK5;
+            if (red[l0][lane]) S32(R, UVC_S_aDPff, UVC_LINK_M, x) = red[l0][lane];
+            if (red[l0 + 1][lane]) S32(R, UVC_S_aDPfr, UVC_LINK_M, x) = red[l0 + 1][lane];
+            if (red[l0 + 2][lane]) S32(R, UVC_S_aDPrf, UVC_LINK_M, x) = red[l0 + 2][lane];
+            if (red[l0 + 3][lane]) S32(R, UVC_S_aDPrr, UVC_LINK_M, x) = red[l0 + 3][lane];
+            if (red[l0 + 4][lane]) BQS(R, UVC_LINK_M, x) = red[l0 + 4][lane];
         }
         return;
     }
+    if (DO_L && lane == 0) R.link_done[wave] = 1;
     if (!valid) return;
-    if (DO_B) seg_store(R, Aref, my_ref, x);
-    if (DO_L) seg_store(R, Alink, UVC_LINK_M, x);
+    if (DO_B) { seg_store(R, Aref, my_ref, x); if (L5_BASE && l5_bq) BQS(R, UVC_LINK_M, x) = l5_bq; }
+    if (DO_L) seg_add_link<L5_LINK>(R, Alink, x);
 #ifdef UVC_FRAG_COARSE
     asm volatile("s_waitcnt vmcnt(0)" ::: "memory");
     COARSE_T(ct3)
@@ -3361,14 +3402,21 @@
 }
 
 struct AccForms { bool vcf, proton, split_windows, p2_plain, frag_plain, h16, fam, digest, duplex; int n_gen; };
+extern "C" int uvc_acc_split_windows(const RegionDev *R) {
+    const char *sp_env = getenv("UVCGPU_SPLIT");
+    const long long per_window = (long long)R->n_fast2 * (R->max_p2_span + 64) / (R->npos > 0 ? R->npos : 1);
+    return (sp_env ? (atoi(sp_env) != 0) : (R->nwin < 4 * 1024 && per_window >= 1024)) ? 1 : 0;
+}
+static bool p2_plain_form(const RegionDev *R, const UvcParams *P) {
+    return UVC_PLATFORM_IONTORRENT != P->inferred_sequencing_platform && !R->any_amplicon && !(P->primerlen > 0 && !(0x2 & P->primer_flag)) && (P->central_readlen >= P->microadjust_median_readlen_thres);
+}
+extern "C" int uvc_acc_p2_plain(const RegionDev *R, const UvcParams *P) { return p2_plain_form(R, P) ? 1 : 0; }
 static AccForms acc_forms(const RegionDev *R, const UvcParams *P, int n_dup) {
     AccForms F;
     F.vcf = (P->inferred_is_vcf_generated != 0);
     F.proton = (UVC_PLATFORM_IONTORRENT == P->inferred_sequencing_platform);
-    const char *sp_env = getenv("UVCGPU_SPLIT");
-    const long long per_window = (long long)R->n_fast2 * (R->max_p2_span + 64) / (R->npos > 0 ? R->npos : 1);
-    F.split_windows = sp_env ? (atoi(sp_env) != 0) : (R->nwin < 4 * 1024 && per_window >= 1024);
-    F.p2_plain = !F.proton && !R->any_amplicon && !(P->primerlen > 0 && !(0x2 & P->primer_flag)) && (P->central_readlen >= P->microadjust_median_readlen_thres);
+    F.split_windows = (uvc_acc_split_windows(R) != 0);
+    F.p2_plain = p2_plain_form(R, P);
     F.frag_plain = F.vcf && !F.proton && !(0x1 & P->fam_flag) && !(P->microadjust_padded_deletion_flag & 0x1);
     F.h16 = (R->max_frag_depth < 65536) && !R->frag32;
     F.fam = (R->n_generic_fs > 0);
@@ -3397,20 +3445,33 @@
     return ((long long)R->max_p2_span + PSCAN_TILE) * m / 10 + 2 < (1LL << 30);
 }
 template <bool DO_L, bool DO_B>
-static void launch_p2_fast(const char *kname, const AccForms &F, const RegionDev *R, const UvcParams *P, unsigned nwin, UvcProf *prof, hipStream_t s) {
-    if (F.split_windows && F.p2_plain) TIMED(prof, kname, hipLaunchKernelGGL((k_p2_fast_split<DO_L, DO_B, true>), dim3(R->nwin), dim3(256), 0, s, *R, *P));
-    else if (F.split_windows) TIMED(prof, kname, hipLaunchKernelGGL((k_p2_fast_split<DO_L, DO_B, false>), dim3(R->nwin), dim3(256), 0, s, *R, *P));
-    else if (F.p2_plain) TIMED(prof, kname, hipLaunchKernelGGL((k_p2_fast<DO_L, DO_B, true>), dim3(nwin), dim3(256), 0, s, *R, *P));
+static void launch_p2_fast(const char *kname, bool split, bool plain, const RegionDev *R, const UvcParams *P, UvcProf *prof, hipStream_t s) {
+    const unsigned nwin = nblk(R->npos, 256);
+    if (split && plain) TIMED(prof, kname, hipLaunchKernelGGL((k_p2_fast_split<DO_L, DO_B, true>), dim3(R->nwin), dim3(256), 0, s, *R, *P));
+    else if (split) TIMED(prof, kname, hipLaunchKernelGGL((k_p2_fast_split<DO_L, DO_B, false>), dim3(R->nwin), dim3(256), 0, s, *R, *P));
+    else if (plain) TIMED(prof, kname, hipLaunchKernelGGL((k_p2_fast<DO_L, DO_B, true>), dim3(nwin), dim3(256), 0, s, *R, *P));
     else TIMED(prof, kname, hipLaunchKernelGGL((k_p2_fast<DO_L, DO_B, false>), dim3(nwin), dim3(256), 0, s, *R, *P));
 }
+__global__ void __launch_bounds__(256) k_link_mark(RegionDev R, const int32_t *xs, int64_t n_xs) {
+    const int64_t t = (int64_t)blockIdx.x * blockDim.x + threadIdx.x;
+    if (xs) { if (t < n_xs) { const int x = xs[t]; if (x >= 0 && x < R.npos) R.link_need[x >> 6] = 1; } }
+    else if (t < R.npos && uvc_link_occ_marks(R.occ[t])) R.link_need[t >> 6] = 1;
+}
+extern "C" void uvc_launch_link_complete(const RegionDev *R, const UvcParams *P, int split, int scope, const int32_t *d_xs, int64_t n_xs, UvcProf *prof, hipStream_t s) {
+    if (!P->inferred_is_vcf_generated) { hipMemsetAsync(R->link_done, 1, (size_t)R->nwin, s); return; }
+    if (scope == UVC_LINK_ALL) hipMemsetAsync(R->link_need, 1, (size_t)R->nwin, s);
+    else if (scope == UVC_LINK_POSITIONS) { if (n_xs <= 0) return; hipLaunchKernelGGL(k_link_mark, dim3(nblk(n_xs, 256)), dim3(256), 0, s, *R, d_xs, n_xs); }
+    else hipLaunchKernelGGL(k_link_mark, dim3(nblk(R->npos, 256)), dim3(256), 0, s, *R, (const int32_t *)nullptr, (int64_t)0);
+    launch_p2_fast<true, false>("k_p2_fast_link", split != 0, p2_plain_form(R, P), R, P, prof, s);
+}
 
 extern "C" void uvc_launch_accumulate(const RegionDev *R, const UvcParams *P, int half_ratio_phred, const int32_t *dup_units, int n_dup, const int64_t *dup_off, int64_t n_dup_work,
-                                      const UvcAccStreams *st, UvcProf *prof) {
+                                      const UvcAccStreams *st, int link_eager, UvcProf *prof) {
     const hipStream_t s = st->s, side = st->side, side3 = st->side3;
     const hipEvent_t e_fork = st->e_fork, e_join = st->e_join, e_fork2 = st->e_fork2, e_join3 = st->e_join3, e_stat = st->e_stat, e_alleles = st->e_alleles;
     const unsigned nwin = nblk(R->npos, 256);
     const AccForms F = acc_forms(R, P, n_dup);
-    if (getenv("UVCGPU_TIMING")) print_forms(F);
+    if (getenv("UVCGPU_TIMING")) { print_forms(F); fprintf(stderr, "[uvcgpu accumulate] link %s\n", link_eager ? "eager" : "lazy"); }
     if (prof) prof->n = 0;
     hipStream_t s2 = (side ? side : s);
     hipStream_t s3 = ((side && side3) ? side3 : s2);
@@ -3442,11 +3503,11 @@
     if (UVC_PLATFORM_IONTORRENT != P->inferred_sequencing_platform)
         TIMED3(prof, "k_frag_sums", hipLaunchKernelGGL(k_frag_sums, dim3(nblk(R->npos, FSUM_TILE), 2), dim3(256), 0, s, *R, *P));
     if (P->inferred_is_vcf_generated) {
-        launch_p2_fast<false, true>("k_p2_fast_base", F, R, P, nwin, prof, s);
+        launch_p2_fast<false, true>("k_p2_fast_base", F.split_windows, F.p2_plain, R, P, prof, s);
         if (side) { hipEventRecord(e_fork2, s); hipStreamWaitEvent(s2, e_fork2, 0); }
         TIMED2(prof, "k_p2_mism", hipLaunchKernelGGL(k_p2_mism, dim3(2048), dim3(256), 0, s, *R, *P));
-        launch_p2_fast<true, false>("k_p2_fast_link", F, R, P, nwin, prof, s);
-    }
+    }
+    if (link_eager) uvc_launch_link_complete(R, P, F.split_windows, UVC_LINK_ALL, nullptr, 0, prof, s);
     if (side) {
         hipEventRecord(e_join, s2); hipStreamWaitEvent(s, e_join, 0);
         if (s3 != s2) { hipEventRecord(e_join3, s3); hipStreamWaitEvent(s, e_join3, 0); hipStreamWaitEvent(s2, e_join3, 0); }
@@ -3496,6 +3557,7 @@
     }
     if (P->inferred_is_vcf_generated) TIMED(prof, "k_p5b", hipLaunchKernelGGL(k_p5b, dim3(nblk(R->npos * 2, 256)), dim3(256), 0, s, *R, *P));
     if (side) hipStreamWaitEvent(s, e_fork2, 0);
+    if (!link_eager) uvc_launch_link_complete(R, P, F.split_windows, UVC_LINK_INDEL, nullptr, 0, prof, s);
 }
 
 __global__ void __launch_bounds__(256) k_math_probe_acc(int op, long long n, const double *in, int n_in, double *out, int n_out) {
diff --git a/uvc_amd/csrc/uvc_kernels_score.hip b/uvc_amd/csrc/uvc_kernels_score.hip
--- a/uvc_amd/csrc/uvc_kernels_score.hip
+++ b/uvc_amd/csrc/uvc_kernels_score.hip
@@ -369,6 +369,7 @@
     const int64_t x = refpos - R.beg;
     const int refidx = zpos - R.beg, refsize = (int)R.npos - 1;
     const int refsymbol = group_refsymbol(R, zpos, st), nsym = st_count(st);
+    if (st != UVC_BASE_SYMBOL && !R.link_done[x >> 6]) atomicExch(R.err, UVCGPU_EDEVICE);
     unsigned mask = type_mask(R, st, x, refsymbol);
     int bd[8], cd[8];
     const int totBDP = masked_bdepths(R, st, x, mask, bd);
diff --git a/uvc_amd/csrc/uvc_launch.h b/uvc_amd/csrc/uvc_launch.h
--- a/uvc_amd/csrc/uvc_launch.h
+++ b/uvc_amd/csrc/uvc_launch.h
@@ -1,6 +1,7 @@
 #ifndef UVC_LAUNCH_H
 #define UVC_LAUNCH_H
 #include "uvc_device.h"
+#include "uvc_link.h"
 
 struct RawReads {
     const int32_t *pos, *endpos, *mpos, *isize, *nm, *l_qseq, *n_cigar, *frag, *fs, *dflag, *kind, *fast_rank;
@@ -55,7 +56,10 @@
 void uvc_launch_zero_state(char *slab, const ZeroPlane *planes, int n_planes, uint8_t *dirty, int ndblk, int64_t npos, hipStream_t s);
 void uvc_launch_check_dirty(const RegionDev *R, unsigned long long *d_n_bad, hipStream_t s);
 void uvc_launch_accumulate(const RegionDev *R, const UvcParams *P, int half_ratio_phred, const int32_t *dup_units, int n_dup, const int64_t *dup_off, int64_t n_dup_work,
-                           const UvcAccStreams *st, UvcProf *prof);
+                           const UvcAccStreams *st, int link_eager, UvcProf *prof);
+int uvc_acc_split_windows(const RegionDev *R);
+int uvc_acc_p2_plain(const RegionDev *R, const UvcParams *P);
+void uvc_launch_link_complete(const RegionDev *R, const UvcParams *P, int split, int scope, const int32_t *d_xs, int64_t n_xs, UvcProf *prof, hipStream_t s);
 void uvc_launch_hap_cand(const RegionDev *R, const HapWork *H, int units, hipStream_t s);
 void uvc_launch_hap_events(const RegionDev *R, const UvcParams *P, const HapWork *H, int units, int n_cand, hipStream_t s);
 int uvc_launch_score(const UvcScoreIn *in, int32_t *d_fields, int64_t capacity, int32_t *d_fields_kept, hipStream_t s);
diff --git a/uvc_amd/csrc/uvc_link.h b/uvc_amd/csrc/uvc_link.h
--- /dev/null
+++ b/uvc_amd/csrc/uvc_link.h
@@ -0,0 +1,36 @@
+#ifndef UVC_LINK_H
+#define UVC_LINK_H
+#include <stddef.h>
+#include <stdint.h>
+#include "uvcgpu.h"
+
+#if defined(__HIPCC__)
+#define UVC_LINK_FN __host__ __device__ static inline
+#else
+#define UVC_LINK_FN static inline
+#endif
+
+enum { UVC_LINK_NONE = -1, UVC_LINK_INDEL = 0, UVC_LINK_POSITIONS = 1, UVC_LINK_ALL = 2 };
+
+UVC_LINK_FN size_t uvc_link_marks_off(size_t dirty_bytes) { return (dirty_bytes + 7) & ~(size_t)7; }
+UVC_LINK_FN size_t uvc_link_marks_stride(int64_t nwin) { return ((size_t)nwin + 3 + 7) & ~(size_t)7; }
+UVC_LINK_FN size_t uvc_link_marks_bytes(size_t dirty_bytes, int64_t nwin) { return uvc_link_marks_off(dirty_bytes) + 2 * uvc_link_marks_stride(nwin); }
+
+UVC_LINK_FN bool uvc_link_window_runs(uint8_t need, uint8_t done) { return need && !done; }
+UVC_LINK_FN bool uvc_link_occ_marks(uint32_t occ) { return ((occ >> UVC_LINK_M) & 0xFEu) != 0; }
+
+UVC_LINK_FN int uvc_link_score_scope(int all_out, int should_output_all, int tumor_vcf_is_provided, int64_t n_force_sites, int min_altdp_thres) {
+    return (all_out || should_output_all || tumor_vcf_is_provided || n_force_sites > 0 || min_altdp_thres <= 0) ? UVC_LINK_ALL : UVC_LINK_NONE;
+}
+UVC_LINK_FN int uvc_link_fetch_scope(int group) { return (group == UVC_F_SEG32 || group == UVC_F_SEG64 || group == UVC_F_VQ) ? UVC_LINK_ALL : UVC_LINK_NONE; }
+UVC_LINK_FN int uvc_link_columns_scope(void) { return UVC_LINK_POSITIONS; }
+UVC_LINK_FN int uvc_link_presence_scope(void) { return UVC_LINK_NONE; }
+
+struct UvcLinkState {
+    bool all_done = false;
+    void planes_zeroed() { all_done = false; }
+    void accumulated(bool eager) { all_done = eager; }
+    bool wants(bool has_planes, bool planes_released, int scope) const { return scope != UVC_LINK_NONE && has_planes && !planes_released && !all_done; }
+    void enqueued(int scope) { if (scope == UVC_LINK_ALL) all_done = true; }
+};
+#endif
```
